# LouisPwr/CarpeDeam

Measured on AMD Instinct MI355X. Metric: corrected bases/sec on 50M×100bp synthetic reads (dhigh), 1/2/4/8 GPU, higher is better.
Workload: dtype u8 (2-bit packed bases; int32 scores; software x87 f80 likelihood sums)

## Files before the change

carpedeam_amd/csrc/aggvote.h:

```cpp
#pragma once
#include "runsort.h"

namespace aggv {

struct Ent { uint32_t id, diag, cs; };
constexpr uint32_t PENDING = 0xFFFFFFFFu;

__global__ __launch_bounds__(1024) void k_seg_flags(const uint32_t *__restrict__ recRep, uint64_t nRec, uint32_t *__restrict__ flag) {
    const uint64_t j = (uint64_t) blockIdx.x * blockDim.x + threadIdx.x;
    if (j <= nRec) flag[j] = (j < nRec && (j == 0 || recRep[j - 1] != recRep[j])) ? 1u : 0u;
}
__global__ __launch_bounds__(1024) void k_seg_fill(const uint32_t *__restrict__ recRep, uint64_t nRec, uint32_t *__restrict__ segOfRec, uint32_t *__restrict__ segRep,
                                                   unsigned long long *__restrict__ segFirstRec, uint32_t *__restrict__ entCnt) {
    const uint64_t j = (uint64_t) blockIdx.x * blockDim.x + threadIdx.x;
    if (j > nRec) return;
    const uint32_t ex = segOfRec[j];
    if (j == nRec) { segFirstRec[ex] = nRec; return; }
    const bool start = j == 0 || recRep[j - 1] != recRep[j];
    const uint32_t g = start ? ex : ex - 1;
    segOfRec[j] = g;
    if (start) { segRep[g] = recRep[j]; segFirstRec[g] = j; entCnt[g] = PENDING; }
}

struct AggArgs {
    const uint64_t *keys; const uint64_t *recVal; const unsigned long long *dst; uint64_t nRec;
    const uint32_t *segOfRec, *segRep; const unsigned long long *segFirstRec; uint64_t nSeg;
    unsigned long long *entOff; uint32_t *entCnt; unsigned long long *perRep;
    Ent *ent; unsigned long long *cursor; unsigned long long cap; unsigned int *overflow;
    int repShift, diagBits; uint32_t idBits;
    uint32_t maxD;
    const uint64_t *sorted;
    const unsigned long long *list; const unsigned int *count;
    bucket::BigList hard;
    unsigned int nextClass = 0;
    int wideWord = 0;
};
constexpr int AG_H = 1024, AG_D = 512, AG_IDX = 9, AG_ORD = 11;
constexpr unsigned long long AG_CHUNK = 2048;
inline unsigned long long aggChunkSlack(unsigned long long units, unsigned long long segments, int cuCount) {
    const unsigned long long g = (unsigned long long) cuCount * 64;
    return (3 * std::min(units + 1, g) + std::min(segments + 1, g)) * AG_CHUNK;
}
static_assert((1 << AG_IDX) >= AG_D && (1 << AG_ORD) > runsort::U_T, "aggregation geometry");
__device__ __forceinline__ uint32_t aggHash(uint64_t k) { return (uint32_t) ((k * 0x9E3779B97F4A7C15ull) >> 40); }

#ifndef CDM_AGG_MINW
#define CDM_AGG_MINW 4
#endif
template <int NT, int ITEMS, typename W = uint64_t>
__global__ __launch_bounds__(NT, CDM_AGG_MINW) void k_unit_agg(AggArgs a) {
    using namespace runsort;
    __shared__ __align__(8) unsigned char sTab[AG_H * 16];
    unsigned long long *tKey = reinterpret_cast<unsigned long long *>(sTab);
    unsigned int *tCnt = reinterpret_cast<unsigned int *>(sTab + AG_H * 8), *tLast = reinterpret_cast<unsigned int *>(sTab + AG_H * 12);
    unsigned int *oFirst = reinterpret_cast<unsigned int *>(sTab), *oEnt = oFirst + (U_T + 2), *oHit = oEnt + (U_T + 2);
    static_assert(3 * (U_T + 2) * 4 <= AG_H * 16, "the directory fits the table's memory");
    __shared__ unsigned long long dKey[AG_D];
    __shared__ unsigned int dCnt[AG_D], dLast[AG_D];
    __shared__ uint16_t sPerm[AG_D];
    __shared__ uint64_t sGStart[NT];
    __shared__ uint32_t sGOff[NT], sGSeg[NT];
    __shared__ unsigned int sDistinct, sOver, sMaxOrd;
    __shared__ unsigned long long sBase, sChunkAt, sChunkEnd;
    const int tid = threadIdx.x, lane = tid & 63, wave = tid >> 6;
    const unsigned int nUnits = *a.count;
    if (tid == 0) { sChunkAt = 0; sChunkEnd = 0; }
    const int lowBits = a.repShift - 1;
    const uint64_t lowMask = (1ull << lowBits) - 1ull;
    for (unsigned int item = blockIdx.x; item < nUnits; item += gridDim.x) {
        const uint64_t base = a.list[3 * (size_t) item];
        const int m = (int) (a.list[3 * (size_t) item + 1] - base);
        const uint64_t rec0 = a.list[3 * (size_t) item + 2];
        const uint32_t g0 = a.segOfRec[rec0];
        for (int i = tid; i < AG_H; i += NT) { tKey[i] = ~0ull; tCnt[i] = 0u; tLast[i] = 0u; }
        if (tid == 0) { sDistinct = 0; sOver = 0; sMaxOrd = 0; }
        __syncthreads();
        const unsigned long long endG = base + (uint64_t) m;
        for (uint64_t c0 = rec0; c0 < a.nRec; c0 += NT) {
            const uint64_t j = c0 + tid;
            const unsigned long long d = j < a.nRec ? a.dst[j] : ~0ull;
            const bool valid = d < endG;
            sGOff[tid] = valid ? (uint32_t) (d - base) : (uint32_t) m;
            sGStart[tid] = valid ? (a.recVal[j] >> RUN_CNT_BITS) : 0ull;
            sGSeg[tid] = valid ? a.segOfRec[j] - g0 : 0u;
            const int nr = __syncthreads_count(valid);
            if (nr == 0) break;
            const int e0 = (int) sGOff[0], e1 = (nr == NT) ? (int) min((unsigned long long) m, (j0Next(a.dst, a.nRec, c0 + NT) - base)) : m;
            if (tid == 0) sMaxOrd = max(sMaxOrd, sGSeg[nr - 1]);
            for (int eb = e0; eb < e1; eb += NT * ITEMS) {
                uint64_t key[ITEMS]; uint32_t ordv[ITEMS];
#pragma unroll
                for (int k = 0; k < ITEMS; k++) {
                    const int e = eb + k * NT + tid;
                    if (e < e1) {
                        int r = 0;
#pragma unroll
                        for (int st = NT / 2; st > 0; st >>= 1) if (r + st < nr && (int) sGOff[r + st] <= e) r += st;
                        key[k] = a.keys[sGStart[r] + (uint64_t) (e - (int) sGOff[r])];
                        ordv[k] = sGSeg[r];
                    }
                }
#pragma unroll
                for (int k = 0; k < ITEMS; k++) {
                    const int e = eb + k * NT + tid;
                    if (e < e1) {
                        const uint64_t hk = ((uint64_t) ordv[k] << lowBits) | ((key[k] >> 1) & lowMask);
                        const unsigned int last = ((unsigned int) e << 1) | (unsigned int) (key[k] & 1ull);
                        uint32_t h = aggHash(hk) & (AG_H - 1);
                        int probe = 0;
                        for (; probe < AG_H; probe++) {
                            unsigned long long old = __hip_atomic_load(&tKey[h], __ATOMIC_RELAXED, __HIP_MEMORY_SCOPE_WORKGROUP);
                            if (old == ~0ull) {
                                old = atomicCAS(&tKey[h], ~0ull, (unsigned long long) hk);
                                if (old == ~0ull) { atomicAdd(&sDistinct, 1u); old = hk; }
                            }
                            if (old == hk) { atomicAdd(&tCnt[h], 1u); atomicMax(&tLast[h], last); break; }
                            h = (h + 1) & (AG_H - 1);
                        }
                        if (probe == AG_H) sOver = 1u;
                    }
                }
            }
            const bool stop = __syncthreads_or(sDistinct > a.maxD || sOver != 0u);
            if (stop || nr < NT) break;
        }
        __syncthreads();
        if (sDistinct > a.maxD || sOver) {
            if (tid == 0) a.hard.add(base, base + (uint64_t) m);
            __syncthreads();
            continue;
        }
        unsigned int c = 0;
        for (int i = tid; i < AG_H; i += NT) c += tKey[i] != ~0ull;
        unsigned int D;
        unsigned int pos = cdm_block_excl_sum<unsigned int>(c, D);
        for (int i = tid; i < AG_H; i += NT) if (tKey[i] != ~0ull) { dKey[pos] = tKey[i]; dCnt[pos] = tCnt[i]; dLast[pos] = tLast[i]; pos++; }
        __syncthreads();
        if (wave == 0) {
            bucket::sortGroup<W>((int) D, lane,
                [&](int i) { return ((W) dKey[i] << AG_IDX) | (W) i; },
                [&](auto &v) {
                    constexpr int R = sizeof(v) / sizeof(v[0]);
#pragma unroll
                    for (int r = 0; r < R; r++) { const int p = lane * R + r; if (p < (int) D) sPerm[p] = (uint16_t) ((uint32_t) v[r] & ((1u << AG_IDX) - 1u)); }
                });
        }
        const unsigned int nOrd = sMaxOrd + 1u;
        for (unsigned int o = tid; o < nOrd; o += NT) { oFirst[o] = 0xFFFFFFFFu; oEnt[o] = 0u; oHit[o] = 0u; }
        if (tid == 0) {
            if (sChunkAt + D > sChunkEnd) { const unsigned long long want = max(AG_CHUNK, (unsigned long long) D); sChunkAt = atomicAdd(a.cursor, want); sChunkEnd = sChunkAt + want; }
            const unsigned long long b = sChunkAt;
            sChunkAt += D;
            if (b + D > a.cap) { atomicExch(a.overflow, 1u); sBase = ~0ull; } else sBase = b;
        }
        __syncthreads();
        const uint64_t idMask = (1ull << a.idBits) - 1ull, diagMask = (1ull << a.diagBits) - 1ull;
        for (unsigned int p = tid; p < D; p += NT) {
            const uint64_t hk = dKey[sPerm[p]], prev = p ? dKey[sPerm[p - 1]] : ~0ull;
            const uint32_t o = (uint32_t) (hk >> lowBits);
            atomicMin(&oFirst[o], p);
            atomicAdd(&oEnt[o], 1u);
            if (p == 0 || (hk >> a.diagBits) != (prev >> a.diagBits)) {
                const uint32_t id = (uint32_t) ((hk >> a.diagBits) & idMask);
                if (id != a.segRep[g0 + o]) atomicAdd(&oHit[o], 1u);
            }
        }
        __syncthreads();
        const unsigned long long b = sBase;
        if (b != ~0ull) {
            for (unsigned int p = tid; p < D; p += NT) {
                const int i = sPerm[p]; const uint64_t hk = dKey[i];
                Ent e; e.id = (uint32_t) ((hk >> a.diagBits) & idMask); e.diag = (uint32_t) (hk & diagMask); e.cs = (dCnt[i] << 1) | (dLast[i] & 1u);
                a.ent[b + p] = e;
            }
            for (unsigned int o = tid; o < nOrd; o += NT) {
                a.entOff[g0 + o] = b + oFirst[o]; a.entCnt[g0 + o] = oEnt[o];
                a.perRep[a.segRep[g0 + o]] = oHit[o];
            }
        }
        __syncthreads();
    }
}

__global__ __launch_bounds__(1024) void k_pending_list(const uint32_t *__restrict__ entCnt, uint64_t nSeg, uint32_t *__restrict__ list, unsigned int *__restrict__ cnt) {
    const uint64_t g = (uint64_t) blockIdx.x * blockDim.x + threadIdx.x;
    const bool p = g < nSeg && entCnt[g] == PENDING;
    const uint32_t q = cdm_block_append(cnt, p);
    if (p) list[q] = (uint32_t) g;
}
__global__ __launch_bounds__(256) void k_rle_segment(AggArgs a, const uint32_t *__restrict__ list, const unsigned int *__restrict__ nList) {
    const unsigned int n = *nList;
    const int lane = threadIdx.x & 63;
    const uint64_t idMask = (1ull << a.idBits) - 1ull, diagMask = (1ull << a.diagBits) - 1ull;
    const uint64_t below = (1ull << lane) - 1ull;
    unsigned long long chunkAt = 0, chunkEnd = 0;
    for (unsigned int it = blockIdx.x * (blockDim.x >> 6) + (threadIdx.x >> 6); it < n; it += gridDim.x * (blockDim.x >> 6)) {
        const uint32_t g = list[it];
        const uint64_t s = a.dst[a.segFirstRec[g]], e = a.dst[a.segFirstRec[g + 1]];
        const uint32_t rep = a.segRep[g];
        unsigned int runs = 0, hits = 0;
        for (uint64_t i = s + lane; i < e; i += 64) {
            const uint64_t k = a.sorted[i], p = i > s ? a.sorted[i - 1] : ~0ull;
            if (i == s || (k >> 1) != (p >> 1)) runs++;
            if (i == s || (k >> (a.diagBits + 1)) != (p >> (a.diagBits + 1))) hits += ((uint32_t) ((k >> (a.diagBits + 1)) & idMask) != rep);
        }
        const unsigned int D = (unsigned int) cdm_wave_sum((int) runs), H = (unsigned int) cdm_wave_sum((int) hits);
        unsigned long long b = 0;
        if (lane == 0) {
            if (chunkAt + D > chunkEnd) { const unsigned long long want = max(AG_CHUNK, (unsigned long long) D); chunkAt = atomicAdd(a.cursor, want); chunkEnd = chunkAt + want; }
            b = chunkAt; chunkAt += D;
            if (b + D > a.cap) { atomicExch(a.overflow, 1u); b = ~0ull; }
            else { a.entOff[g] = b; a.entCnt[g] = D; a.perRep[rep] = H; }
        }
        b = (unsigned long long) __shfl((long long) b, 0, 64);
        if (b == ~0ull) continue;
        unsigned long long run = 0;
        for (uint64_t t0 = s; t0 < e; t0 += 64) {
            const uint64_t i = t0 + lane;
            bool start = false; uint64_t k = 0;
            if (i < e) { k = a.sorted[i]; start = i == s || (k >> 1) != (a.sorted[i - 1] >> 1); }
            const uint64_t m = __ballot(start);
            if (start) {
                const uint64_t later = lane < 63 ? (m >> (lane + 1)) : 0ull;
                uint64_t hi;
                if (later) hi = i + (uint64_t) __ffsll((unsigned long long) later);
                else {
                    uint64_t lo = min(t0 + 63, e - 1); hi = e;
                    while (hi - lo > 1) { const uint64_t mid = lo + ((hi - lo) >> 1); if ((a.sorted[mid] >> 1) == (k >> 1)) lo = mid; else hi = mid; }
                }
                Ent en; en.id = (uint32_t) ((k >> (a.diagBits + 1)) & idMask); en.diag = (uint32_t) ((k >> 1) & diagMask);
                en.cs = ((uint32_t) (hi - i) << 1) | (uint32_t) (a.sorted[hi - 1] & 1ull);
                a.ent[b + run + (unsigned long long) __popcll(m & below)] = en;
            }
            run += (unsigned long long) __popcll(m);
        }
    }
}

struct VoteEntArgs {
    const Ent *ent; const unsigned long long *entOff; const uint32_t *entCnt; const uint32_t *segRep; uint64_t nSeg;
    const uint64_t *hitOff;
    const uint32_t *stale;
    int diagBias;
    const uint32_t *cont = nullptr;
};
constexpr int HEAD_WORDS = 2048;
__global__ void k_head_entries(const Ent *__restrict__ ent, const unsigned long long *__restrict__ entOff, const uint32_t *__restrict__ entCnt, uint64_t nSeg, uint32_t *__restrict__ out) {
    if (nSeg == 0) { out[0] = 0; out[1] = 0; out[2] = 1; out[HEAD_WORDS + 3] = 0; return; }
    const uint32_t id = ent[entOff[0]].id;
    uint32_t words = 0; bool whole = true;
    for (uint64_t g = 0; g < nSeg && whole && words <= (uint32_t) HEAD_WORDS; g++) {
        const Ent *e = ent + entOff[g]; const uint32_t c = entCnt[g];
        for (uint32_t j = 0; j < c; j++) {
            if (e[j].id != id) { whole = false; break; }
            if (words + 2 <= (uint32_t) HEAD_WORDS) { out[3 + words] = e[j].diag | ((e[j].cs & 1u) ? 0u : 1u << 31); out[4 + words] = e[j].cs >> 1; words += 2; }
            else { words = (uint32_t) HEAD_WORDS + 1; whole = false; break; }
        }
    }
    out[0] = words; out[1] = id; out[2] = whole ? 1u : 0u;
    const uint64_t gl = nSeg - 1;
    out[HEAD_WORDS + 3] = ent[entOff[gl] + entCnt[gl] - 1].id;
}
struct Walk {
    uint32_t prevDiag = 0, diagCnt = 0, maxDiag = 0, diagonal = 0, top = 0; int bestRev = 0; bool any = false;
    __device__ __forceinline__ void add(uint32_t d, uint32_t c, int rev) {
        diagCnt = (any && prevDiag == d) ? diagCnt + c : c;
        if (diagCnt >= maxDiag) { diagonal = d; maxDiag = diagCnt; bestRev = rev; }
        prevDiag = d; top += c; any = true;
    }
};
template <typename HitT>
__global__ __launch_bounds__(256) void k_vote_entries(VoteEntArgs a, HitT *__restrict__ out) {
    const uint64_t g = (uint64_t) blockIdx.x * blockDim.x + threadIdx.x;
    if (g >= a.nSeg) return;
    const uint32_t rep = a.segRep[g], cnt = a.entCnt[g];
    const Ent *e = a.ent + a.entOff[g];
    uint64_t pos = a.hitOff[rep] + 1;
    uint32_t p = 0;
    while (p < cnt) {
        const uint32_t id = e[p].id;
        if (id == rep) { do p++; while (p < cnt && e[p].id == id); continue; }
        Walk w;
        do { const Ent x = e[p]; w.add(x.diag, x.cs >> 1, (x.cs & 1u) ? 0 : 1); p++; } while (p < cnt && e[p].id == id);
        if (p == cnt) {
            bool done = false;
            for (uint64_t g2 = g + 1; g2 < a.nSeg && !done; g2++) {
                const Ent *f = a.ent + a.entOff[g2]; const uint32_t c2 = a.entCnt[g2];
                uint32_t j = 0;
                for (; j < c2 && f[j].id == id; j++) w.add(f[j].diag, f[j].cs >> 1, (f[j].cs & 1u) ? 0 : 1);
                done = j < c2;
            }
            bool intoStale = !done;
            if (!done && a.cont) {
                if (id == a.cont[1]) for (uint32_t j = 0; j + 1 < a.cont[0]; j += 2) w.add(a.cont[3 + j] & 0x7FFFFFFFu, a.cont[4 + j], (int) (a.cont[3 + j] >> 31));
                intoStale = a.cont[2] != 0u;
            }
            if (intoStale && id == a.stale[1]) {
                const uint32_t m = a.stale[0];
                for (uint32_t j = 0; j < m; j++) w.add(a.stale[2 + j] + (uint32_t) a.diagBias, 1u, 0);
            }
        }
        HitT h;
        h.target = id; h.score = w.bestRev ? -(int) w.top : (int) w.top; h.diagonal = (int) (short) ((int) w.diagonal - a.diagBias);
        out[pos++] = h;
    }
}

}
```

carpedeam_amd/csrc/kmermatch.hip:

```cpp
#include <memory>
#include <cstring>

#include "aggvote.h"
#include "kmer_plan.h"
#include "kmer_tuple.h"
#include "kmer_extract.h"
#include "kmer_group.h"
#include "kmer_vote.h"

namespace {

using rx::DoubleBuf;
using namespace kplan;
static_assert(RADIX_BITS == rx::BITS && SLOT_REM_BITS == rx::SLOT_REM, "kmer_plan.h restates the radix sort's geometry");
inline uint64_t deviceBytes() { size_t fr = 0, tot = 0; if (hipMemGetInfo(&fr, &tot) == hipSuccess) return tot; (void) hipGetLastError(); return 0; }
inline Db planDb(const cdm_seqdb *db, int k, bool device = false) { Db d; d.n = db->n; d.maxLen = db->maxLen; d.residues = db->residues; d.k = k; if (device) d.deviceBytes = deviceBytes(); return d; }
inline int slotSplit(int k, int &lowBits) {
    lowBits = slotLowBits(k);
    if (const char *e = cdmGetenv("CDM_SLOT_LOWBITS")) {
        char *end = nullptr; const long v = strtol(e, &end, 10);
        if (end == e || *end || v < 0 || v > 64 || !slotLowBitsServed(k, (int) v)) {
            cdm_set_error("cdm_kmermatch: CDM_SLOT_LOWBITS=%s: k = %d takes 0 <= 2k - %d - n <= %d global bits behind the head digit", e, k, RADIX_BITS, 2 * RADIX_BITS); return CDM_ERR_INVALID;
        }
        lowBits = (int) v;
    }
    return CDM_OK;
}

struct KmerJobBase {
    virtual ~KmerJobBase() {}
    virtual int phaseA() = 0;
    virtual int staleTail(unsigned long long J) = 0;
    virtual int phaseB(cdm_hits **out) = 0;
    virtual int gatherByRep() = 0;
    virtual int sortFrom(const uint64_t *devKeys, uint64_t nKeys, uint32_t *head, uint64_t info[2]) = 0;
    virtual int voteWith(const uint32_t *cont, const uint32_t *staleIn, cdm_hits **out) = 0;
    virtual int splitBegin() = 0;
    virtual int splitFinish(const void *keys, const void *vals, uint64_t m, const void *hkeys, const void *hvals, uint64_t h, bool below) = 0;
    bool split = false;
    std::vector<unsigned long long> sendOff;
    const void *sendKeys = nullptr, *sendVals = nullptr, *sendHashKeys = nullptr, *sendHashVals = nullptr; unsigned long long sendHash = 0; int valBytes = 0;
    cdm_ctx *ctx = nullptr; const cdm_seqdb *db = nullptr; cdm_kmer_params parCopy; const cdm_kmer_params *par = nullptr;
    int part = 0, nparts = 1;
    int block = 0, nBlocks = 0;
    unsigned long long live = 0, nKept = 0, regionTwo = 0;
    bool anyBelow = false;
    uint64_t *gathered = nullptr;
    uint32_t staleHost[64 + 3] = {0};
};
template <typename LY>
struct KmerJob : KmerJobBase {
    typedef typename LY::V V;
    hipStream_t s = nullptr; uint32_t n = 0; int k = 0;
    uint32_t idBits = 0, diagBits = 0; int diagBias = 0; const char *sortEnv = nullptr; bool lsdOnly = false;
    bool wide = false;
    bool passes = false;
    uint64_t r2Slots = 0;
    uint32_t ordLo = 0, ordHi = 0;
    DevBuf<uint64_t> splitK; DevBuf<V> splitV;
    DevBuf<unsigned long long> counters;
    DevBuf<unsigned int> cls;
    DevBuf<uint32_t> listShort, listLong, listSingle, listHuge;
    DevBuf<unsigned long long> slots; DevBuf<uint64_t> slotOff; DevBuf<uint32_t> rankOf;
    uint64_t kmerSlots = 0; unsigned long long nTuples = 0;
    DoubleBuf<uint64_t> keys; DoubleBuf<V> vals;
    DevBuf<uint64_t> k0, k1; DevBuf<V> v0, v1;
    V *vA = nullptr, *vB = nullptr;
    DevBuf<unsigned long long> segBuf;
    TupleGeom geom; int lowBits = 0;
    DevBuf<unsigned long long> headHist; bool headCounted = false;
    DevBuf<uint32_t> stRep, ovRep; DevBuf<uint64_t> stVal, ovVal; DevBuf<uint8_t> stCnt; DevBuf<unsigned long long> recFlag; uint64_t stagedWaves = 0, stagedOwn = 0; unsigned long long ovCap = 0, nOvRec = 0;
    DevBuf<uint32_t> bigRecRep, bigRecRep1; DevBuf<uint64_t> bigRecVal, bigRecVal1; unsigned long long nBigRec = 0;
    bool ownPipeline = false;
    bool headRange = false; uint32_t headLo = 0, headHi = 0xFFFFFFFFu;
    GroupArgs<LY> ga; DevBuf<unsigned long long> statStripes; unsigned long long *startIo = nullptr; DevBuf<uint32_t> staleBuf;
    DevBuf<uint64_t> runsOut, runsTmp;
    DevBuf<uint64_t> recvA, recvB; DevBuf<uint32_t> contBuf;
    const uint64_t *sorted2M = nullptr; unsigned long long nGroupM = 0;
    bool haveEntries = false; uint64_t nSegM = 0;
    DevBuf<uint32_t> agSegOfRec, agSegRep, agEntCnt, agPending; DevBuf<unsigned long long> agSegFirstRec, agEntOff, agPerRep, agCursor; DevBuf<aggv::Ent> agEnt; DevBuf<unsigned int> agFlags;
    float msSort1 = 0;
    KmerJob(cdm_ctx *c, const cdm_seqdb *d, const cdm_kmer_params *p) { ctx = c; db = d; parCopy = *p; par = &parCopy; }
int init() {
    s = ctx->stream;
    n = (uint32_t) db->n;
    k = par->kmer_size;
    if (k < 4 || k > 31) { cdm_set_error("cdm_kmermatch: k must be in 4..31 (got %d)", k); return CDM_ERR_INVALID; }
    idBits = bitsFor(n); diagBits = bitsFor(2ull * db->maxLen + 2);
    wide = 2 * idBits + diagBits + 1 > 63 || cdmGetenv("CDM_FORCE_WIDE_KEY") != nullptr;
    if (wide && (int) (aggv::AG_ORD + idBits + diagBits) > 64) {
        cdm_set_error("cdm_kmermatch: %u sequences x max length %u: ids and diagonals beyond %d bits are not implemented", n, db->maxLen, 64 - aggv::AG_ORD); return CDM_ERR_UNSUPPORTED;
    }
    if (wide && nparts > 1 && !passes) { cdm_set_error("cdm_kmermatch_part: %u sequences x max length %u need the wide group key, which the exchange of the k-mer-range split does not carry yet", n, db->maxLen); return CDM_ERR_UNSUPPORTED; }
    diagBias = (int) db->maxLen + 1;
    sortEnv = cdmGetenv("CDM_KMER_SORT");
    lsdOnly = sortEnv && !strcmp(sortEnv, "lsd");
    if (!counters.alloc(8)) { cdm_set_error("cdm_kmermatch: out of device memory"); return CDM_ERR_HIP; }
    hipMemsetAsync(counters.p, 0, 8 * 8, s);
    geom.kbits = 2 * k; geom.lb = (int) bitsFor((uint64_t) db->maxLen + 1); geom.lenArr = db->len;
    if constexpr (LY::bySlot) {
        if (!slotLayoutFits(planDb(db, k)) || split || (nparts != 1 && !headRange) || passes || lsdOnly) { cdm_set_error("cdm_kmermatch: internal error: the slot layout was chosen for a run it does not serve"); return CDM_ERR_INVALID; }
        geom.uniL = db->maxLen; geom.uniK = k; geom.uniS = slotsPerSeq(db->maxLen, k); divMagic(geom.uniS, geom.uniMul, geom.uniSh); geom.headShift = 2 * k - std::min(rx::BITS, 2 * k);
    }
    return CDM_OK;
}
int phaseA() override {
    if (int rc = init()) return rc;
    constexpr uint32_t SHORT_CAP = 256, LONG_CAP = 4096;

    if (!cls.alloc(8) || !listShort.alloc(n) || !listLong.alloc(n) || !listSingle.alloc(n) || !listHuge.alloc(n)) { cdm_set_error("cdm_kmermatch: out of device memory"); return CDM_ERR_HIP; }
    if (!LY::bySlot && (!slots.alloc((size_t) n + 1) || !slotOff.alloc((size_t) n + 1) || !rankOf.alloc(n))) { cdm_set_error("cdm_kmermatch: out of device memory"); return CDM_ERR_HIP; }
    hipMemsetAsync(cls.p, 0, 8 * 4, s);
    uint64_t capacity = 0;
    if constexpr (LY::bySlot) capacity = (uint64_t) n * geom.uniS;
    else {
        DevBuf<uint32_t> lk0, lk1, lv0, lv1; DevBuf<unsigned long long> ordOff;
        if (!lk0.alloc(n) || !lk1.alloc(n) || !lv0.alloc(n) || !lv1.alloc(n) || !ordOff.alloc((size_t) n + 1)) { cdm_set_error("cdm_kmermatch: out of device memory"); return CDM_ERR_HIP; }
        hipLaunchKernelGGL(k_len_keys, dim3((n + 255) / 256), dim3(256), 0, s, db->len, n, db->maxLen, lk0.p, lv0.p);
        const unsigned lenBits = bitsFor((uint64_t) db->maxLen + 2);
        cdmscan::ScanTemp st;
        DoubleBuf<uint32_t> lk(lk0.p, lk1.p), lv(lv0.p, lv1.p);
        if (int rc = rx::sortPairs<uint32_t, uint32_t>(s, ctx->cuCount, lk, lv, (uint64_t) n, 0, (int) lenBits)) return rc;
        hipLaunchKernelGGL(k_slot_counts, dim3((n + 256) / 256), dim3(256), 0, s, db->len, lv.current(), n, k, slots.p);
        if (split) {
            const unsigned blk = nBlocks ? (unsigned) block : (unsigned) part, of = nBlocks ? (unsigned) nBlocks : (unsigned) nparts;
            DevBuf<uint32_t> cuts; uint32_t hc[2] = {0, 0};
            if (!cuts.alloc(2)) { cdm_set_error("cdm_kmermatch: out of device memory"); return CDM_ERR_HIP; }
            cdmscan::ScanTemp stCut;
            if (int rc = cdmscan::exclusiveScan<unsigned long long>(s, stCut, slots.p, ordOff.p, (size_t) n + 1)) return rc;
            hipLaunchKernelGGL(k_block_cuts, dim3(1), dim3(1), 0, s, (const unsigned long long *) ordOff.p, n, blk, of, cuts.p);
            hipMemcpyAsync(hc, cuts.p, 8, hipMemcpyDeviceToHost, s);
            if (hipStreamSynchronize(s) != hipSuccess) { cdm_set_error("cdm_kmermatch: slot layout failed"); return CDM_ERR_HIP; }
            ordLo = hc[0]; ordHi = hc[1];
            hipLaunchKernelGGL(k_slot_mask, dim3((n + 255) / 256), dim3(256), 0, s, slots.p, n, ordLo, ordHi);
        }
        if (int rc = cdmscan::exclusiveScan<unsigned long long>(s, st, slots.p, ordOff.p, (size_t) n + 1)) return rc;
        hipLaunchKernelGGL(k_slot_scatter, dim3((n + 256) / 256), dim3(256), 0, s, lv.current(), ordOff.p, n, slotOff.p, rankOf.p);
        hipMemcpyAsync(&capacity, ordOff.p + n, 8, hipMemcpyDeviceToHost, s);
        if (hipStreamSynchronize(s) != hipSuccess) { cdm_set_error("cdm_kmermatch: slot layout failed"); return CDM_ERR_HIP; }
    }
    kmerSlots = geom.kmerSlots = capacity;
    r2Slots = split ? (uint64_t) (ordHi - ordLo) : (uint64_t) n;
    capacity += r2Slots;
    nTuples = capacity;

    const uint64_t valSlots = LY::bySlot ? r2Slots : capacity;
    if (!k0.alloc(capacity) || !k1.alloc(capacity) || !v0.alloc(valSlots) || !v1.alloc(valSlots)) {
        cdm_set_error("cdm_kmermatch: out of device memory for %llu k-mer tuples (%.1f GB)", (unsigned long long) capacity, (capacity * 16.0 + valSlots * 2.0 * sizeof(V)) / 1e9); return CDM_ERR_HIP;
    }
    vA = LY::bySlot ? v0.p - kmerSlots : v0.p; vB = LY::bySlot ? v1.p - kmerSlots : v1.p;
    ExtractArgs<LY> ea; ea.geom = geom; ea.uniS = geom.uniS;
    ea.woff = db->woff; ea.len = db->len; ea.codes = db->codes; ea.nmask = db->nmask; ea.hasN = db->hasN;
    ea.k = k; ea.kmersPerSeq = par->kmers_per_seq; ea.scale = par->kmers_per_seq_scale; ea.seed = par->hash_shift; ea.ignoreMultiKmer = par->ignore_multi_kmer;
    ea.keys = k0.p; ea.vals = vA; ea.slotOff = slotOff.p; ea.slowShort = listShort.p; ea.slowLong = listLong.p; ea.slowHuge = listHuge.p; ea.slowCnt = cls.p; ea.n = n;
    ea.hugeSp = nullptr; ea.hugeSel = nullptr; ea.hugeCap = 0;
    ea.list = nullptr; ea.nList = 0; ea.hashBase = kmerSlots; ea.rankOf = rankOf.p;
    if constexpr (LY::bySlot) {
        const char *e = cdmGetenv("CDM_SLOT_HIST");
        if (headRange || !(e && !strcmp(e, "kernel"))) {
            if (!headHist.alloc(HEAD_BINS)) { cdm_set_error("cdm_kmermatch: out of device memory"); return CDM_ERR_HIP; }
            hipMemsetAsync(headHist.p, 0, HEAD_BINS * 8, s);
            ea.headHist = headHist.p; ea.headShift = geom.headShift; headCounted = true;
        }
    }
    {
        const unsigned __int128 space = (unsigned __int128) 1 << (2 * k);
        ea.kLo = (uint64_t) (space * (unsigned) part / (unsigned) nparts);
        ea.kHi = (part == nparts - 1) ? ~0ull : (uint64_t) (space * (unsigned) (part + 1) / (unsigned) nparts);
        ea.lastPart = (part == nparts - 1) ? 1 : 0; ea.belowFlag = cls.p + 5;
        if (split) { ea.kLo = 0; ea.kHi = ~0ull; ea.lastPart = 1; ea.ordLo = ordLo; ea.ordHi = ordHi; }
        if (headRange) { ea.kLo = 0; ea.kHi = ~0ull; }
    }
    hipEventRecord(ctx->ev0, s);
    bool uniformKernel = false;
    if constexpr (LY::bySlot) {
        const char *e = cdmGetenv("CDM_EXTRACT");
        const uint32_t L = db->maxLen, W = (L + 15) / 16, nPos = L - (uint32_t) k + 1u;
        const size_t cap = (size_t) (float) ((float) (par->kmers_per_seq - 1) + (par->kmers_per_seq_scale * (float) L));
        if (!(e && !strcmp(e, "pair")) && k <= 30 && ea.kLo == 0 && ea.kHi == ~0ull && ea.ordHi == 0 && ea.lastPart && nPos <= cap && nPos <= (uint32_t) PAIR_POS &&
            db->nCount == 0 && !db->raw && (uint64_t) n * W < (1ull << 32)) {
            unsigned int bad = 1;
            hipLaunchKernelGGL(k_uniform_check, dim3((n + 255) / 256), dim3(256), 0, s, (const uint32_t *) db->len, (const uint32_t *) db->woff, (const uint8_t *) db->hasN, n, L, W, cls.p + 6);
            hipMemcpyAsync(&bad, cls.p + 6, 4, hipMemcpyDeviceToHost, s);
            if (hipStreamSynchronize(s) != hipSuccess) { cdm_set_error("cdm_kmermatch: looking at the sequence lengths failed"); return CDM_ERR_HIP; }
            uniformKernel = bad == 0;
        }
        if (uniformKernel) {
            const uint32_t batches = ((n + 1) / 2 + UNI_BATCH - 1) / UNI_BATCH;
            uint32_t blocks = std::min<uint32_t>((batches + FAST_WAVES - 1) / FAST_WAVES, ctx->cuCount * UNI_MINW);
            if (const char *eb = cdmGetenv("CDM_EXTRACT_BLOCKS")) blocks = std::max(1u, std::min<uint32_t>(blocks, (uint32_t) atoi(eb)));
            hipLaunchKernelGGL(k_extract_uniform<LY>, dim3(blocks), dim3(64 * FAST_WAVES), 0, s, ea, L, W);
        }
    }
    ea.single = listSingle.p; ea.listCount = nullptr;
    if (!uniformKernel) {
        hipLaunchKernelGGL(k_seq_hash<LY>, dim3((n + 255) / 256), dim3(256), 0, s, ea);
        if (k <= 30) {
            hipLaunchKernelGGL(k_extract_pair<LY>, dim3(std::min<uint32_t>(((n + 1) / 2 + FAST_WAVES - 1) / FAST_WAVES, ctx->cuCount * 16)), dim3(64 * FAST_WAVES), 0, s, ea);
            ea.list = listSingle.p; ea.listCount = cls.p + 2;
        }
        hipLaunchKernelGGL(k_extract_fast<LY>, dim3(std::min<uint32_t>((n + FAST_WAVES - 1) / FAST_WAVES, ctx->cuCount * 16)), dim3(64 * FAST_WAVES), 0, s, ea);
        ea.listCount = nullptr;
    }
    unsigned int hcls[4] = {0, 0, 0, 0};
    hipMemcpyAsync(hcls, cls.p, 16, hipMemcpyDeviceToHost, s);
    { hipError_t e = hipStreamSynchronize(s); if (e != hipSuccess) { cdm_set_error("cdm_kmermatch: extraction failed: %s", hipGetErrorString(e)); return CDM_ERR_HIP; } }
    auto general = [&](void (*kern)(ExtractArgs<LY>), const uint32_t *list, uint32_t cnt, uint32_t blocks, uint32_t nt) { ea.list = list; ea.nList = cnt; hipLaunchKernelGGL(kern, dim3(blocks), dim3(nt), 0, s, ea); };
    if (hcls[0]) general(k_extract<LY, SHORT_CAP, 64>, listShort.p, hcls[0], std::min<uint32_t>(hcls[0], ctx->cuCount * 32), 64);
    if (hcls[1]) general(k_extract<LY, LONG_CAP, 256>, listLong.p, hcls[1], std::min<uint32_t>(hcls[1], ctx->cuCount * 2), 256);
    DevBuf<SeqPos> hugeSp; DevBuf<uint8_t> hugeSel;
    if (hcls[3]) {
        uint32_t cap = LONG_CAP; while (cap < db->maxLen) cap <<= 1;
        const uint32_t blocks = std::min<uint32_t>(hcls[3], (uint32_t) ctx->cuCount * 4);
        if (!hugeSp.alloc((size_t) blocks * cap) || !hugeSel.alloc((size_t) blocks * cap)) { cdm_set_error("cdm_kmermatch: out of device memory"); return CDM_ERR_HIP; }
        ea.hugeSp = hugeSp.p; ea.hugeSel = hugeSel.p; ea.hugeCap = cap;
        general(k_extract<LY, 0, 256>, listHuge.p, hcls[3], blocks, 256);
    }
    hipEventRecord(ctx->ev1, s);
    unsigned int belowHost = 0;
    hipMemcpyAsync(&belowHost, cls.p + 5, 4, hipMemcpyDeviceToHost, s);
    { hipError_t e = hipStreamSynchronize(s); if (e != hipSuccess) { cdm_set_error("cdm_kmermatch: extraction (general path) failed: %s", hipGetErrorString(e)); return CDM_ERR_HIP; } }
    anyBelow = belowHost != 0;
    hipEventElapsedTime(&ctx->lastMs[3], ctx->ev0, ctx->ev1);
    if (cdmGetenv("CDM_BUCKET_STATS")) fprintf(stderr, "kmermatch extraction (%s): %u sequences through k_extract for a repeated k-mer or a bottom-m selection, %u + %u longer ones\n", uniformKernel ? "uniform kernel" : "pair + fast kernels", hcls[0], hcls[1], hcls[3]);
    if (split) return splitPartition();
    if constexpr (LY::bySlot) if (headRange) {
        unsigned long long hh[HEAD_BINS];
        if (hipMemcpy(hh, headHist.p, sizeof(hh), hipMemcpyDeviceToHost) != hipSuccess) { cdm_set_error("cdm_kmermatch: reading the head histogram failed"); return CDM_ERR_HIP; }
        std::vector<uint32_t> cut = equalShareCuts(hh, HEAD_BINS, nparts);
        cut.resize((size_t) nparts + 1, (uint32_t) HEAD_BINS);
        headLo = cut[part]; headHi = cut[part + 1];
        anyBelow = false; for (uint32_t d = 0; d < headLo; d++) anyBelow = anyBelow || hh[d] != 0;
    }
    return sortAndGroup();
}
int splitPartition() {
    DevBuf<unsigned long long> cnt, bounds;
    if (!cnt.alloc(2) || !bounds.alloc((size_t) CDM_KPART_SLICES + 2)) { cdm_set_error("cdm_kmermatch: out of device memory"); return CDM_ERR_HIP; }
    unsigned long long m = 0, h = 0;
    const int shift = 2 * k - 8;
    DoubleBuf<uint64_t> ordK(k0.p, k1.p); DoubleBuf<V> ordV(v0.p, v1.p);
    if (kmerSlots) {
        if (int rc = rx::sortPairs<uint64_t, V>(s, ctx->cuCount, ordK, ordV, (uint64_t) kmerSlots, shift, 2 * k + 1)) return rc;
        hipLaunchKernelGGL(k_live_count, dim3(1), dim3(1), 0, s, (const uint64_t *) ordK.current(), (uint64_t) kmerSlots, 2 * k, cnt.p);
        hipMemcpyAsync(&m, cnt.p, 8, hipMemcpyDeviceToHost, s);
    }
    uint64_t *rK = ordK.current(); V *rV = ordV.current();
    if (r2Slots) {
        if (int rc = rx::compactPairs<uint64_t, V>(s, k0.p + kmerSlots, v0.p + kmerSlots, (uint64_t) r2Slots, k1.p + kmerSlots, v1.p + kmerSlots, cnt.p + 1)) return rc;
        hipMemcpyAsync(&h, cnt.p + 1, 8, hipMemcpyDeviceToHost, s);
    }
    if (hipStreamSynchronize(s) != hipSuccess) { cdm_set_error("cdm_kmermatch: ordering the tuples by k-mer slice failed: %s", hipGetErrorString(hipGetLastError())); return CDM_ERR_HIP; }
    sendOff.assign((size_t) CDM_KPART_SLICES + 1, 0);
    if (m) {
        hipLaunchKernelGGL(k_slice_bounds, dim3(2), dim3(256), 0, s, (const uint64_t *) rK, (uint64_t) m, shift, (uint32_t) CDM_KPART_SLICES, bounds.p);
        hipMemcpyAsync(sendOff.data(), bounds.p, ((size_t) CDM_KPART_SLICES + 1) * 8, hipMemcpyDeviceToHost, s);
        if (hipStreamSynchronize(s) != hipSuccess) { cdm_set_error("cdm_kmermatch: ordering the tuples by k-mer slice failed: %s", hipGetErrorString(hipGetLastError())); return CDM_ERR_HIP; }
    }
    sendKeys = rK; sendVals = rV; valBytes = (int) sizeof(V);
    sendHashKeys = k1.p + kmerSlots; sendHashVals = v1.p + kmerSlots; sendHash = h;
    return CDM_OK;
}
int splitBegin() override {
    split = true;
    if (nparts != CDM_KPART_SLICES) { cdm_set_error("cdm_kmermatch: internal error: the split by reads orders its tuples by %d slices", CDM_KPART_SLICES); return CDM_ERR_INVALID; }
    return phaseA();
}
int takeOver(uint64_t m, uint64_t h, bool below) { vA = v0.p; vB = v1.p; kmerSlots = m; r2Slots = h; nTuples = m + h; geom.kmerSlots = m; anyBelow = below; return sortAndGroup(); }
void freeExtraction() { slots.free(); slotOff.free(); rankOf.free(); listShort.free(); listLong.free(); listSingle.free(); listHuge.free(); }
int splitFinish(const void *keysIn, const void *valsIn, uint64_t m, const void *hkeys, const void *hvals, uint64_t h, bool below) override {
    freeExtraction();
    splitK.free(); splitV.free(); k0.free(); k1.free(); v0.free(); v1.free();
    DevBuf<uint64_t> nk0, nk1; DevBuf<V> nv0, nv1;
    const uint64_t tot = m + h;
    if (!nk0.alloc(tot) || !nk1.alloc(tot) || !nv0.alloc(tot) || !nv1.alloc(tot)) { cdm_set_error("cdm_kmermatch: out of device memory for %llu received k-mer tuples", (unsigned long long) tot); return CDM_ERR_HIP; }
    if (m) { hipMemcpyAsync(nk0.p, keysIn, m * 8, hipMemcpyDeviceToDevice, s); hipMemcpyAsync(nv0.p, valsIn, m * sizeof(V), hipMemcpyDeviceToDevice, s); }
    if (h) { hipMemcpyAsync(nk0.p + m, hkeys, h * 8, hipMemcpyDeviceToDevice, s); hipMemcpyAsync(nv0.p + m, hvals, h * sizeof(V), hipMemcpyDeviceToDevice, s); }
    if (hipStreamSynchronize(s) != hipSuccess) { cdm_set_error("cdm_kmermatch: taking over the received tuples failed"); return CDM_ERR_HIP; }
    k0.p = nk0.release(); k1.p = nk1.release(); v0.p = nv0.release(); v1.p = nv1.release();
    return takeOver(m, h, below);
}
int keepOnlyOutgoing() {
    DevBuf<uint64_t> hk; DevBuf<V> hv;
    const unsigned long long m = sendOff.empty() ? 0 : sendOff.back();
    if (!hk.alloc(sendHash) || !hv.alloc(sendHash) || !splitK.alloc(m) || !splitV.alloc(m)) { cdm_set_error("cdm_kmermatch: out of device memory"); return CDM_ERR_HIP; }
    if (m) { hipMemcpyAsync(splitK.p, sendKeys, m * 8, hipMemcpyDeviceToDevice, s); hipMemcpyAsync(splitV.p, sendVals, m * sizeof(V), hipMemcpyDeviceToDevice, s); }
    if (sendHash) { hipMemcpyAsync(hk.p, sendHashKeys, sendHash * 8, hipMemcpyDeviceToDevice, s); hipMemcpyAsync(hv.p, sendHashVals, sendHash * sizeof(V), hipMemcpyDeviceToDevice, s); }
    if (hipStreamSynchronize(s) != hipSuccess) { cdm_set_error("cdm_kmermatch: keeping a block's tuples failed"); return CDM_ERR_HIP; }
    k0.free(); k1.free(); v0.free(); v1.free();
    sendKeys = splitK.p; sendVals = splitV.p;
    freeExtraction(); cls.free(); counters.free();
    sendHashKeys = keptHashK.p = hk.release(); sendHashVals = keptHashV.p = hv.release();
    return CDM_OK;
}
DevBuf<uint64_t> keptHashK; DevBuf<V> keptHashV;
int rangeFinishOwned(DevBuf<uint64_t> &keysBuf, DevBuf<V> &valsBuf, uint64_t m, uint64_t h, bool below) {
    passes = true; split = true;
    if (int rc = init()) return rc;
    const uint64_t tot = m + h;
    if (!k1.alloc(tot) || !v1.alloc(tot)) { cdm_set_error("cdm_kmermatch: out of device memory for a pass over %llu k-mer tuples", (unsigned long long) tot); return CDM_ERR_HIP; }
    k0.p = keysBuf.release(); v0.p = valsBuf.release();
    return takeOver(m, h, below);
}
int sortAndGroup() {
    keys = DoubleBuf<uint64_t>(k0.p, k1.p); vals = DoubleBuf<V>(vA, vB);
    lowBits = lsdOnly ? 0 : std::max(0, 2 * k + 1 - 27);
    if constexpr (LY::bySlot) if (int rc = slotSplit(k, lowBits)) return rc;
    hipEventRecord(ctx->ev0, s);
    if (int rc = sortRegionOne()) return rc;
    hipEventRecord(ctx->ev1, s);
    hipEventRecord(ctx->ev2, s);
    if (int rc = sortRegionTwo()) return rc;
    hipEventRecord(ctx->ev3, s);
    ga.geom = geom;
    ga.keys = keys.current(); ga.vals = vals.current(); ga.n = nTuples; ga.onlyExtendable = par->include_only_extendable; ga.covMode = par->cov_mode;
    ga.covThr = par->cov_thr; ga.idBits = idBits; ga.diagBits = diagBits; ga.diagBias = diagBias; ga.first = 0; ga.wide = wide ? 1 : 0;
    ga.firstRunIdx = (anyBelow || (split && kmerSlots == 0)) ? ~0ull : 0ull;
    if (!statStripes.alloc(STAT_STRIPES)) { cdm_set_error("cdm_kmermatch: out of device memory"); return CDM_ERR_HIP; }
    hipMemsetAsync(statStripes.p, 0, STAT_STRIPES * 8, s);
    ga.stat = statStripes.p;
    startIo = (unsigned long long *) keys.alternate();
    if (!LY::bySlot) live = 0;
    nKept = 0;
    if (!staleBuf.alloc(STALE_MAX + 3)) { cdm_set_error("cdm_kmermatch: out of device memory"); return CDM_ERR_HIP; }
    hipMemsetAsync(staleBuf.p, 0, (STALE_MAX + 3) * 4, s);
    if (kmerSlots && !LY::bySlot) {
        hipLaunchKernelGGL(k_live_count, dim3(1), dim3(1), 0, s, ga.keys, (uint64_t) kmerSlots, 2 * k, counters.p + 3);
        hipMemcpyAsync(&live, counters.p + 3, 8, hipMemcpyDeviceToHost, s);
        if (hipStreamSynchronize(s) != hipSuccess) { cdm_set_error("cdm_kmermatch: grouping failed"); return CDM_ERR_HIP; }
    }
    if (lowBits == 0) { if (scanGroups(ga, startIo) != CDM_OK) return groupingFailed(); }
    else if (int rc = groupBuckets()) return rc;
    return countKept();
}
int groupingFailed() { cdm_set_error("cdm_kmermatch: grouping failed: %s", hipGetErrorString(hipGetLastError())); return CDM_ERR_HIP; }
int sortRegionOne() {
    const int sortTop = lowBits ? 2 * k + 1 : 2 * k;
    if constexpr (LY::bySlot) {
        if (!segBuf.alloc(rx::BINS + 1)) { cdm_set_error("cdm_kmermatch: out of device memory"); return CDM_ERR_HIP; }
        uint64_t *res = nullptr; unsigned long long liveSlots = 0;
        if (int rc = rx::sortSlotKeys(s, ctx->cuCount, k0.p, k1.p, (uint64_t) kmerSlots, 2 * k, lowBits, headCounted ? headHist.p : nullptr, segBuf.p, liveSlots, res, &ctx->lastMs[13], &ctx->lastMs[14],
                                      headRange ? headLo : 0u, headRange ? std::min<uint32_t>(headHi, (uint32_t) rx::BINS) : (uint32_t) rx::BINS)) return rc;
        keys = DoubleBuf<uint64_t>(res, res == k0.p ? k1.p : k0.p); vals = res == k0.p ? DoubleBuf<V>(vA, vB) : DoubleBuf<V>(vB, vA);
        ctx->lastMs[15] = (float) (((double) kmerSlots * 8.0 + (double) liveSlots * 8.0 + (double) (ctx->lastMs[14] - 1.f) * (double) liveSlots * 16.0) / 1e9);
        live = liveSlots; geom.seg = segBuf.p;
        return CDM_OK;
    }
    uint64_t sorted = kmerSlots;
    const bool range = nparts > 1 && kmerSlots && !lsdOnly && !split;
    DevBuf<unsigned long long> cnt;
    if (range) {
        if (!cnt.alloc(1)) { cdm_set_error("cdm_kmermatch: out of device memory"); return CDM_ERR_HIP; }
        if (int rc = rx::compactPairs<uint64_t, V>(s, k0.p, vA, (uint64_t) kmerSlots, k1.p, vB, cnt.p)) return rc;
        unsigned long long m = 0;
        hipMemcpyAsync(&m, cnt.p, 8, hipMemcpyDeviceToHost, s);
        if (hipStreamSynchronize(s) != hipSuccess) { cdm_set_error("cdm_kmermatch: compaction failed"); return CDM_ERR_HIP; }
        keys = DoubleBuf<uint64_t>(k1.p, k0.p); vals = DoubleBuf<V>(vB, vA); sorted = m;
    }
    if (int rc = rx::sortPairs<uint64_t, V>(s, ctx->cuCount, keys, vals, sorted, lowBits, sortTop, &ctx->lastMs[13])) return rc;
    ctx->lastMs[14] = (float) ((sortTop - lowBits + rx::BITS - 1) / rx::BITS);
    ctx->lastMs[15] = (float) ((double) ctx->lastMs[14] * (double) sorted * 2.0 * (8.0 + sizeof(V)) / 1e9);
    if (range) hipMemsetAsync(keys.current() + sorted, 0xFF, (size_t) (kmerSlots - sorted) * 8, s);
    return CDM_OK;
}
int sortRegionTwo() {
    DoubleBuf<uint64_t> rk(k0.p + kmerSlots, k1.p + kmerSlots); DoubleBuf<V> rv(vA + kmerSlots, vB + kmerSlots);
    if (int rc = rx::sortPairs<uint64_t, V>(s, ctx->cuCount, rk, rv, (uint64_t) r2Slots, 0, 63)) return rc;
    uint64_t *kOut = keys.current() + kmerSlots; V *vOut = vals.current() + kmerSlots;
    if (rk.current() != kOut && r2Slots) { hipMemcpyAsync(kOut, rk.current(), (size_t) r2Slots * 8, hipMemcpyDeviceToDevice, s); hipMemcpyAsync(vOut, rv.current(), (size_t) r2Slots * sizeof(V), hipMemcpyDeviceToDevice, s); }
    return CDM_OK;
}
int scanGroups(GroupArgs<LY> g, unsigned long long *io) {
    const size_t cnt = (size_t) (g.n - g.first);
    if (cnt == 0) return CDM_OK;
    cdmscan::ScanTemp t;
    if (int rc = cdmscan::inclusiveMaxScanFn(s, t, StartFrom<LY>{StartIndex<LY>{g.keys, g.geom, (unsigned long long) g.first}}, io + g.first, cnt)) return rc;
    if (cnt > CDM_MAX_LAUNCH_THREADS - 256) { cdm_set_error("cdm_kmermatch: %zu tuples in one grouping launch (CDM_KMER_SORT=lsd takes fewer than 2^32)", cnt); return CDM_ERR_UNSUPPORTED; }
    hipLaunchKernelGGL(k_groups<LY>, CDM_GRID((cnt + 255) / 256, 256), dim3(256), 0, s, g, io);
    return hipStreamSynchronize(s) == hipSuccess ? CDM_OK : CDM_ERR_HIP;
}
template <typename W>
bool launchFused(int own, uint32_t maxBucket, DevBuf<unsigned long long> &bigList, DevBuf<unsigned int> &bigCnt, DevBuf<BlockHead> &heads) {
    BucketGroupArgs<LY, W> ba;
    static_cast<GroupParams &>(ba) = ga; ba.n = live;
    ba.keys = ga.keys; ba.vals = ga.vals; ba.geom = geom; ba.out = startIo; ba.lowBits = lowBits; ba.own = own; ba.maxBucket = maxBucket;
    ba.big.list = bigList.p; ba.big.cnt = bigCnt.p;
    const uint64_t perBlock = (uint64_t) own * bucket::BK_WAVES;
    stagedWaves = 0;
    if (LY::bySlot && (ownPipeline || headRange) && live && !cdmGetenv("CDM_RUN_RECORDS") && !cdmGetenv("CDM_RUN_CAP")) {
        const uint64_t waves = (live + (uint64_t) own - 1) / (uint64_t) own;
        ovCap = live / 256 + 4096;
        if (stRep.alloc(waves * REC_CAP) && stVal.alloc(waves * REC_CAP) && stCnt.alloc(waves + 1) && recFlag.alloc(2) && ovRep.alloc(ovCap) && ovVal.alloc(ovCap)) {
            hipMemsetAsync(stCnt.p, 0, waves + 1, s); hipMemsetAsync(recFlag.p, 0, 8, s);
            ba.recRep = stRep.p; ba.recVal = stVal.p; ba.recCnt = stCnt.p; stagedWaves = waves; stagedOwn = (uint64_t) own; nBigRec = 0;
            ba.ovRep = ovRep.p; ba.ovVal = ovVal.p; ba.ovCursor = recFlag.p; ba.ovCap = ovCap;
            if (const char *e = cdmGetenv("CDM_REC_LIMIT")) { const long v = atol(e); if (v >= 0 && v <= REC_CAP) ba.recLimit = (uint32_t) v; }
        } else { dropStages(); (void) hipGetLastError(); }
    }
    if constexpr (LY::bySlot) {
        const uint64_t blocks = (live + perBlock - 1) / perBlock;
        if (!heads.alloc(blocks)) { cdm_set_error("cdm_kmermatch: out of device memory"); return false; }
        if (blocks) hipLaunchKernelGGL(k_block_heads, CDM_GRID((blocks + 255) / 256, 256), dim3(256), 0, s, geom, (uint64_t) live, perBlock, blocks, heads.p);
        ba.blockHead = heads.p;
    }
    if (live) hipLaunchKernelGGL((k_bucket_groups<LY, W>), dim3((unsigned) ((live + perBlock - 1) / perBlock)), dim3(bucket::BK_NT), cdm_lds_pad("CDM_LDS_PAD_GROUPS"), s, ba);
    return true;
}
void dropStages() { stagedWaves = 0; stRep.free(); stVal.free(); stCnt.free(); ovRep.free(); ovVal.free(); }
int groupBuckets() {
    int own; uint32_t maxBucket; bucket::capacities(own, maxBucket);
    own = std::min(own, GkGeom<LY>::OWN); maxBucket = std::min<uint32_t>(maxBucket, (uint32_t) GkGeom<LY>::MAXB);
    DevBuf<unsigned long long> bigList; DevBuf<unsigned int> bigCnt;
    if (!bigList.alloc(bucket::bigListSlots(kmerSlots, maxBucket)) || !bigCnt.alloc(1)) { cdm_set_error("cdm_kmermatch: out of device memory"); return CDM_ERR_HIP; }
    hipMemsetAsync(bigCnt.p, 0, 4, s);
    if (kmerSlots) hipMemsetAsync(startIo + live, 0xFF, (size_t) (kmerSlots - live) * 8, s);
    DevBuf<BlockHead> heads;
    if (!(lowBits <= GROUP_WORD32_LOWBITS ? launchFused<uint32_t>(own, maxBucket, bigList, bigCnt, heads) : launchFused<uint64_t>(own, maxBucket, bigList, bigCnt, heads))) return CDM_ERR_HIP;
    unsigned int nBig = 0; unsigned long long recOver = 0;
    hipMemcpyAsync(&nBig, bigCnt.p, 4, hipMemcpyDeviceToHost, s);
    if (stagedWaves) hipMemcpyAsync(&recOver, recFlag.p, 8, hipMemcpyDeviceToHost, s);
    GroupArgs<LY> g2 = ga; g2.first = kmerSlots;
    int rc = scanGroups(g2, startIo);
    nOvRec = recOver;
    if (stagedWaves && recOver > ovCap) dropStages();
    if (rc == CDM_OK && nBig) rc = groupBigBuckets(bigList, nBig);
    return rc == CDM_OK ? CDM_OK : groupingFailed();
}
template <bool GATHER> void bigBucketPairs(unsigned int grid, const unsigned long long *ranges, unsigned int nBig, uint64_t *dk, V *dv) {
    if constexpr (LY::bySlot) hipLaunchKernelGGL(k_big_slot_pairs<GATHER>, dim3(grid), dim3(256), 0, s, ranges, nBig, const_cast<uint64_t *>(ga.keys), geom, dk, dv);
    else {
        hipLaunchKernelGGL((bucket::k_big_copy<uint64_t, GATHER>), dim3(grid), dim3(256), 0, s, ranges, nBig, const_cast<uint64_t *>(ga.keys), dk);
        hipLaunchKernelGGL((bucket::k_big_copy<V, GATHER>), dim3(grid), dim3(256), 0, s, ranges, nBig, const_cast<V *>(ga.vals), dv);
    }
}
int groupBigBuckets(DevBuf<unsigned long long> &bigList, unsigned int nBig) {
    DevBuf<unsigned long long> ranges; uint64_t total = 0; unsigned long long firstStart = ~0ull;
    int rc = bucket::loadBigList(s, bigList.p, nBig, ranges, total, &firstStart);
    if (cdmGetenv("CDM_BUCKET_STATS")) fprintf(stderr, "kmermatch sort 1: %llu slots, low bits %d: %u big buckets, %llu tuples\n", (unsigned long long) kmerSlots, lowBits, nBig, (unsigned long long) total);
    DevBuf<uint64_t> dk0, dk1; DevBuf<V> dv0, dv1; DevBuf<unsigned long long> ds;
    if (rc == CDM_OK && (!dk0.alloc(total) || !dk1.alloc(total) || !dv0.alloc(total) || !dv1.alloc(total) || !ds.alloc(total))) rc = CDM_ERR_HIP;
    if (rc != CDM_OK) return rc;
    const unsigned int grid = bucket::bigCopyGrid(nBig);
    bigBucketPairs<true>(grid, ranges.p, nBig, dk0.p, dv0.p);
    DoubleBuf<uint64_t> dk(dk0.p, dk1.p); DoubleBuf<V> dv(dv0.p, dv1.p);
    if (int rc2 = rx::sortPairs<uint64_t, V>(s, ctx->cuCount, dk, dv, (uint64_t) total, 0, 2 * k)) return rc2;
    bigBucketPairs<false>(grid, ranges.p, nBig, dk.current(), dv.current());
    GroupArgs<LY> gd = ga; gd.keys = dk.current(); gd.vals = dv.current(); gd.n = total; gd.first = 0;
    gd.geom.kmerSlots = ~0ull;
    gd.firstRunIdx = (firstStart == 0 && !anyBelow) ? 0ull : ~0ull;
    if (int rc2 = scanGroups(gd, ds.p)) return rc2;
    hipLaunchKernelGGL((bucket::k_big_copy<unsigned long long, false>), dim3(grid), dim3(256), 0, s, (const unsigned long long *) ranges.p, nBig, startIo, ds.p);
    if (hipStreamSynchronize(s) != hipSuccess) return CDM_ERR_HIP;
    if (stagedWaves) {
        DevBuf<unsigned long long> gapped;
        if (!gapped.alloc(total + nBig)) return CDM_ERR_HIP;
        hipLaunchKernelGGL(k_big_gap_copy, dim3(grid), dim3(256), 0, s, (const unsigned long long *) ranges.p, nBig, (const unsigned long long *) ds.p, gapped.p);
        runsort::RunArgs ra = runArgs((const uint64_t *) gapped.p, total + nBig, 0, 0);
        rc = runsort::makeRunRecords(s, ra, bigRecRep, bigRecRep1, bigRecVal, bigRecVal1, nBigRec);
        if (rc == CDM_OK && nBigRec) hipLaunchKernelGGL(k_big_rec_starts, CDM_GRID((nBigRec + 255) / 256, 256), dim3(256), 0, s, (const unsigned long long *) ranges.p, nBig, bigRecVal.p, (uint64_t) nBigRec);
        if (rc == CDM_OK && hipStreamSynchronize(s) != hipSuccess) rc = CDM_ERR_HIP;
        bigRecRep1.free(); bigRecVal1.free();
    }
    return rc;
}
int countKept() {
    hipLaunchKernelGGL(k_reduce_stats, dim3(1), dim3(256), 0, s, (const unsigned long long *) statStripes.p, counters.p + 4);
    hipMemcpyAsync(&nKept, counters.p + 4, 8, hipMemcpyDeviceToHost, s);
    { hipError_t e = hipStreamSynchronize(s); if (e != hipSuccess) { cdm_set_error("cdm_kmermatch: grouping failed: %s", hipGetErrorString(e)); return CDM_ERR_HIP; } }
    hipEventElapsedTime(&msSort1, ctx->ev0, ctx->ev1);
    regionTwo = 0;
    if (nparts > 1 && part == nparts - 1 && r2Slots) {
        hipLaunchKernelGGL(k_count_hash_tuples, dim3(1), dim3(1), 0, s, (const uint64_t *) ga.keys + kmerSlots, (uint64_t) r2Slots, counters.p + 6);
        hipMemcpyAsync(&regionTwo, counters.p + 6, 8, hipMemcpyDeviceToHost, s);
        if (hipStreamSynchronize(s) != hipSuccess) { cdm_set_error("cdm_kmermatch: grouping failed"); return CDM_ERR_HIP; }
    }
    return CDM_OK;
}
runsort::RunArgs runArgs(const uint64_t *gk, unsigned long long nIn, unsigned long long skipLo, unsigned long long skipHi) const {
    runsort::RunArgs ra; ra.keys = gk; ra.n = nIn; ra.skipLo = skipLo; ra.skipHi = skipHi; ra.repShift = (int) (idBits + diagBits + 1);
    ra.wide = wide ? 1 : 0; ra.idShift = (int) diagBits + 1; ra.idMask = (1ull << idBits) - 1ull;
    return ra;
}
int staleTail(unsigned long long J) override {
    memset(staleHost, 0, sizeof(staleHost));
    hipMemsetAsync(staleBuf.p, 0, (STALE_MAX + 3) * 4, s);
    const unsigned long long realTuples = live + regionTwo;
    if (nparts > 1 && J >= realTuples) { staleHost[STALE_MAX + 4] = 1; return hipStreamSynchronize(s) == hipSuccess ? CDM_OK : CDM_ERR_HIP; }
    StaleArgs<LY> sa;
    sa.keys = ga.keys; sa.vals = ga.vals; sa.geom = geom; sa.live = live; sa.kmerSlots = kmerSlots; sa.nTuples = nTuples; sa.J = J;
    sa.lowBits = lowBits; sa.sorted = (lowBits == 0); sa.out = staleBuf.p;
    hipLaunchKernelGGL(k_stale_tail<LY>, dim3(1), dim3(256), 0, s, sa);
    hipMemcpyAsync(staleHost, staleBuf.p, (STALE_MAX + 3) * 4, hipMemcpyDeviceToHost, s);
    if (hipStreamSynchronize(s) != hipSuccess) { cdm_set_error("cdm_kmermatch: grouping failed"); return CDM_ERR_HIP; }
    if (staleHost[0] >= (uint32_t) STALE_MAX) {
        cdm_set_error("cdm_kmermatch: the reference's last per-target scan could run over %d or more left-over tuples of one sequence; not reproduced on the device", STALE_MAX);
        return CDM_ERR_UNSUPPORTED;
    }
    staleHost[STALE_MAX + 4] = (J + staleHost[0] >= realTuples) ? 1u : 0u;
    return CDM_OK;
}
int phaseB(cdm_hits **out) override {
    if (int rc = sort2((const uint64_t *) startIo, nTuples, live, kmerSlots, keys.current(), (uint64_t *) startIo, true)) return rc;
    return vote(nullptr, true, out);
}
int sort2(const uint64_t *keysIn, unsigned long long nIn, unsigned long long skipLo, unsigned long long skipHi, uint64_t *bufA, uint64_t *bufB, bool ownBuffers) {

    if (ownBuffers) { v0.free(); v1.free(); }
    const int top2 = (int) ((wide ? idBits : 2 * idBits) + diagBits + 1);
    const char *sort2Env = cdmGetenv("CDM_KMER_SORT2");
    const bool sort2Check = sort2Env && !strcmp(sort2Env, "check");
    const bool sort2Runs = !lsdOnly && (!sort2Env || !strcmp(sort2Env, "runs") || sort2Check);
    if (wide && (!sort2Runs || sort2Check || !ownBuffers)) { cdm_set_error("cdm_kmermatch: the wide group key runs on the default pipeline only (run records + aggregated entries)"); return CDM_ERR_UNSUPPORTED; }
    if (sort2Env && strcmp(sort2Env, "runs") && strcmp(sort2Env, "radix") && !sort2Check) { cdm_set_error("cdm_kmermatch: CDM_KMER_SORT2 must be runs, radix or check"); return CDM_ERR_INVALID; }
    unsigned long long nGroup = 0;
    const uint64_t *sorted2 = nullptr;
    hipEventRecord(ctx->ev0, s);
    if (sort2Runs) {
        using namespace runsort;
        const uint64_t *gk = keysIn;
        uint64_t *sortedOut = bufA;
        if (sort2Check) {
            if (!runsOut.alloc(nIn)) { cdm_set_error("cdm_kmermatch: out of device memory (sort 2 check)"); return CDM_ERR_HIP; }
            sortedOut = runsOut.p;
        }
        const RunArgs ra = runArgs(gk, nIn, skipLo, skipHi);
        const bool fromStage = stagedWaves && ownBuffers && keysIn == (const uint64_t *) startIo;
        RepRecords R;
        if (int rc = recordsByRep(ra, fromStage, true, R, nGroup)) return rc;
        const unsigned long long nRec = R.nRec; const DoubleBuf<uint32_t> &rk = R.rep; const DoubleBuf<uint64_t> &rv = R.val; DevBuf<unsigned long long> &dst = R.dst;
        if (nRec) {
            if (hipStreamSynchronize(s) != hipSuccess) { cdm_set_error("cdm_kmermatch: sort 2 (records) failed: %s", hipGetErrorString(hipGetLastError())); return CDM_ERR_HIP; }
            const char *voteEnv = cdmGetenv("CDM_KMER_VOTE");
            const bool wordFits = aggv::AG_ORD + idBits + diagBits + aggv::AG_IDX <= 64 && !(wide && cdmGetenv("CDM_FORCE_WIDE_WORD"));
            const char *distVote = cdmGetenv("CDM_DIST_VOTE");
            bool aggregated = wide || ((ownBuffers || !(distVote && !strcmp(distVote, "tuples"))) && !sort2Check && !(voteEnv && !strcmp(voteEnv, "tuples")) && wordFits);
            if ((wide || fromStage) && ownBuffers && nGroup != nKept) { cdm_set_error("cdm_kmermatch: internal error: %llu group tuples counted, %llu in the run records", nKept, nGroup); return CDM_ERR_HIP; }
            if (aggregated) {
                const unsigned long long slack = aggv::aggChunkSlack(nGroup / runsort::U_T, nRec, ctx->cuCount);
                unsigned long long capEnt = nGroup / 6 + (4ull << 20) + slack;
                if (const char *e = cdmGetenv("CDM_AGG_CAP")) capEnt = strtoull(e, nullptr, 10);
                int rc = aggregate(sortedOut, nGroup, rk.current(), (const uint64_t *) rv.current(), dst.p, nRec, gk, top2, capEnt, !wordFits);
                while (rc == CDM_ERR_UNSUPPORTED && wide && capEnt < nGroup + 1 + slack) {
                    capEnt = std::min<unsigned long long>(nGroup + 1 + slack, std::max<unsigned long long>(capEnt * 3, 1024));
                    rc = aggregate(sortedOut, nGroup, rk.current(), (const uint64_t *) rv.current(), dst.p, nRec, gk, top2, capEnt, !wordFits);
                }
                if (rc == CDM_ERR_UNSUPPORTED && !wide) aggregated = false;
                else if (rc) return rc;
            }
            haveEntries = aggregated;
            if (!aggregated && segmentedSortKeys(s, ctx->cuCount, sortedOut, sortedOut, nGroup, (int) (idBits + diagBits + 1), (int) (diagBits + 1), top2, rk.current(), dst.p, nRec, gk,
                                  (const uint64_t *) rv.current()) != CDM_OK) {
                cdm_set_error("cdm_kmermatch: segmented sort 2 failed: %s", hipGetErrorString(hipGetLastError())); return CDM_ERR_HIP;
            }
        }
        sorted2 = sortedOut;
    }
    if (!sort2Runs || sort2Check) {
        const int shiftHi2 = lsdOnly ? 1 : std::max(1, top2 + 1 - 32);
        bool g2First = true;
        if (int rc = rx::sortKeys<uint64_t>(s, ctx->cuCount, const_cast<uint64_t *>(keysIn), bufA, (uint64_t) nIn, shiftHi2, top2 + 1, g2First)) return rc;
        DoubleBuf<uint64_t> g(g2First ? const_cast<uint64_t *>(keysIn) : bufA, g2First ? bufA : const_cast<uint64_t *>(keysIn));
        unsigned long long nGroupR = 0;
        if (nIn) {
            hipLaunchKernelGGL(k_live_count, dim3(1), dim3(1), 0, s, (const uint64_t *) g.current(), (uint64_t) nIn, top2, counters.p + 2);
            hipMemcpyAsync(&nGroupR, counters.p + 2, 8, hipMemcpyDeviceToHost, s);
            if (hipStreamSynchronize(s) != hipSuccess) { cdm_set_error("cdm_kmermatch: radix sort 2 failed"); return CDM_ERR_HIP; }
        }
        const uint64_t *sortedR = g.current();
        if (shiftHi2 > 1) {
            if (bucket::bucketSortKeys(s, g.current(), g.alternate(), nGroupR, shiftHi2, 1, top2) != CDM_OK) { cdm_set_error("cdm_kmermatch: bucket sort 2 failed: %s", hipGetErrorString(hipGetLastError())); return CDM_ERR_HIP; }
            sortedR = g.alternate();
        }
        if (sort2Check) {
            if (nGroupR != nGroup) { cdm_set_error("cdm_kmermatch: sort 2 check: %llu kept tuples by runs, %llu by radix", nGroup, nGroupR); return CDM_ERR_HIP; }
            hipMemsetAsync(counters.p + 5, 0xFF, 8, s);
            if (nGroup) hipLaunchKernelGGL(k_first_diff, dim3((unsigned) std::min<uint64_t>((nGroup + 255) / 256, 65535)), dim3(256), 0, s, sorted2, sortedR, (uint64_t) nGroup, counters.p + 5);
            unsigned long long firstDiff = ~0ull, pair[2] = {0, 0};
            hipMemcpyAsync(&firstDiff, counters.p + 5, 8, hipMemcpyDeviceToHost, s);
            if (hipStreamSynchronize(s) != hipSuccess) { cdm_set_error("cdm_kmermatch: sort 2 check failed"); return CDM_ERR_HIP; }
            if (firstDiff != ~0ull) {
                hipMemcpy(&pair[0], sorted2 + firstDiff, 8, hipMemcpyDeviceToHost); hipMemcpy(&pair[1], sortedR + firstDiff, 8, hipMemcpyDeviceToHost);
                cdm_set_error("cdm_kmermatch: sort 2 check: first difference at %llu of %llu: runs %016llx radix %016llx (idBits %u diagBits %u)", firstDiff, nGroup, pair[0], pair[1], idBits, diagBits);
                return CDM_ERR_HIP;
            }
        }
        nGroup = nGroupR; sorted2 = sortedR;
    }
    hipEventRecord(ctx->ev1, s);
    sorted2M = sorted2; nGroupM = nGroup;
    return CDM_OK;
}
struct RepRecords {
    cdmscan::ScanTemp st; DevBuf<uint32_t> r0, r1; DevBuf<uint64_t> v0, v1; DevBuf<unsigned long long> dst; unsigned long long nRec = 0;
    DoubleBuf<uint32_t> rep; DoubleBuf<uint64_t> val;
};
int recordsByRep(const runsort::RunArgs &ra, bool staged, bool dstIfNone, RepRecords &R, unsigned long long &total) {
    if (staged) { if (int rc = stagedRunRecords(ra, R.r0, R.r1, R.v0, R.v1, R.nRec)) return rc; }
    else if (int rc = runsort::makeRunRecords(s, ra, R.r0, R.r1, R.v0, R.v1, R.nRec)) return rc;
    if (R.nRec == 0 && !dstIfNone) return CDM_OK;
    if (!R.dst.alloc(R.nRec + 1)) { cdm_set_error("cdm_kmermatch: out of device memory (%llu run records)", R.nRec); return CDM_ERR_HIP; }
    if (R.nRec == 0) return CDM_OK;
    R.rep = DoubleBuf<uint32_t>(R.r0.p, R.r1.p); R.val = DoubleBuf<uint64_t>(R.v0.p, R.v1.p);
    if (int rc = rx::sortPairs<uint32_t, uint64_t>(s, ctx->cuCount, R.rep, R.val, (uint64_t) R.nRec, 0, (int) idBits)) return rc;
    hipMemsetAsync(R.val.current() + R.nRec, 0, 8, s);
    if (int rc = cdmscan::exclusiveScanFn<unsigned long long, runsort::RunLen>(s, R.st, runsort::RunLen{R.val.current()}, R.dst.p, (size_t) R.nRec + 1)) return rc;
    hipMemcpyAsync(&total, R.dst.p + R.nRec, 8, hipMemcpyDeviceToHost, s);
    return CDM_OK;
}
int stagedRunRecords(const runsort::RunArgs &whole, DevBuf<uint32_t> &rr0, DevBuf<uint32_t> &rr1, DevBuf<uint64_t> &rv0, DevBuf<uint64_t> &rv1, unsigned long long &nRec) {
    DevBuf<unsigned long long> off; cdmscan::ScanTemp st;
    if (!off.alloc(stagedWaves + 1)) { cdm_set_error("cdm_kmermatch: out of device memory (run records)"); return CDM_ERR_HIP; }
    if (int rc = cdmscan::exclusiveScanFn<unsigned long long, RecCount>(s, st, RecCount{stCnt.p}, off.p, (size_t) stagedWaves + 1)) return rc;
    unsigned long long n1 = 0, n2 = 0;
    hipMemcpyAsync(&n1, off.p + stagedWaves, 8, hipMemcpyDeviceToHost, s);
    DevBuf<uint32_t> q0, q1; DevBuf<uint64_t> w0, w1;
    runsort::RunArgs r2 = whole; r2.keys = whole.keys + kmerSlots; r2.n = whole.n - kmerSlots; r2.skipLo = r2.skipHi = 0; r2.base = kmerSlots;
    if (r2.n) { if (int rc = runsort::makeRunRecords(s, r2, q0, q1, w0, w1, n2)) return rc; }
    if (hipStreamSynchronize(s) != hipSuccess) { cdm_set_error("cdm_kmermatch: run records failed: %s", hipGetErrorString(hipGetLastError())); return CDM_ERR_HIP; }
    unsigned long long nb = nBigRec;
    if (nOvRec) {
        DevBuf<uint64_t> x0, x1; DevBuf<uint32_t> y0, y1;
        const unsigned long long tot = nBigRec + nOvRec;
        if (!x0.alloc(tot) || !x1.alloc(tot) || !y0.alloc(tot) || !y1.alloc(tot)) { cdm_set_error("cdm_kmermatch: out of device memory (run records)"); return CDM_ERR_HIP; }
        if (nBigRec) { hipMemcpyAsync(x0.p, bigRecVal.p, nBigRec * 8, hipMemcpyDeviceToDevice, s); hipMemcpyAsync(y0.p, bigRecRep.p, nBigRec * 4, hipMemcpyDeviceToDevice, s); }
        hipMemcpyAsync(x0.p + nBigRec, ovVal.p, nOvRec * 8, hipMemcpyDeviceToDevice, s); hipMemcpyAsync(y0.p + nBigRec, ovRep.p, nOvRec * 4, hipMemcpyDeviceToDevice, s);
        DoubleBuf<uint64_t> x(x0.p, x1.p); DoubleBuf<uint32_t> y(y0.p, y1.p);
        if (int rc = rx::sortPairs<uint64_t, uint32_t>(s, ctx->cuCount, x, y, (uint64_t) tot, runsort::RUN_CNT_BITS, 64)) return rc;
        bigRecVal.free(); bigRecRep.free();
        bigRecVal.p = x.current() == x0.p ? x0.release() : x1.release(); bigRecRep.p = y.current() == y0.p ? y0.release() : y1.release();
        nb = tot;
    }
    nRec = n1 + nb + n2;
    if (!rr0.alloc(nRec) || !rr1.alloc(nRec) || !rv0.alloc(nRec + 1) || !rv1.alloc(nRec + 1)) { cdm_set_error("cdm_kmermatch: out of device memory (%llu run records)", nRec); return CDM_ERR_HIP; }
    if (n1) hipLaunchKernelGGL(k_rec_compact, CDM_GRID((stagedWaves + REC_WAVES - 1) / REC_WAVES, 256), dim3(256), 0, s, (const uint32_t *) stRep.p, (const uint64_t *) stVal.p, (const unsigned long long *) off.p, (uint64_t) stagedWaves,
                               (uint64_t) stagedOwn, (const uint64_t *) bigRecVal.p, (uint64_t) nb, rr0.p, rv0.p);
    if (nb) hipLaunchKernelGGL(k_rec_place_big, CDM_GRID((nb + 255) / 256, 256), dim3(256), 0, s, (const uint32_t *) bigRecRep.p, (const uint64_t *) bigRecVal.p, (uint64_t) nb, (const uint64_t *) stVal.p, (const uint8_t *) stCnt.p,
                               (const unsigned long long *) off.p, (uint64_t) stagedOwn, rr0.p, rv0.p);
    if (n2) { hipMemcpyAsync(rr0.p + n1 + nb, q0.p, n2 * 4, hipMemcpyDeviceToDevice, s); hipMemcpyAsync(rv0.p + n1 + nb, w0.p, n2 * 8, hipMemcpyDeviceToDevice, s); }
    if (hipStreamSynchronize(s) != hipSuccess) { cdm_set_error("cdm_kmermatch: run records (packing) failed: %s", hipGetErrorString(hipGetLastError())); return CDM_ERR_HIP; }
    if (cdmGetenv("CDM_BUCKET_STATS")) fprintf(stderr, "run records: %llu staged by the grouping kernel, %llu beyond its waves' stages, %llu of its big buckets, %llu of the whole-sequence hash region\n", n1, nOvRec, nBigRec, n2);
    stRep.free(); stVal.free(); stCnt.free(); bigRecRep.free(); bigRecVal.free(); ovRep.free(); ovVal.free(); stagedWaves = 0; nBigRec = 0; nOvRec = 0;
    return CDM_OK;
}
int voteEntries(cdm_hits **out, const uint32_t *contDev = nullptr) {
    DevBuf<unsigned long long> perRepScan;
    if (!perRepScan.alloc((size_t) n + 1)) { cdm_set_error("cdm_kmermatch: out of device memory (vote)"); return CDM_ERR_HIP; }
    cdmscan::ScanTemp st4a;
    if (int rc = cdmscan::exclusiveScan<unsigned long long>(s, st4a, agPerRep.p, perRepScan.p, (size_t) n + 1)) return rc;
    if (int rc = placeHits(perRepScan.p, true, out, [&](cdm_hits *res) {
        aggv::VoteEntArgs va; va.ent = agEnt.p; va.entOff = agEntOff.p; va.entCnt = agEntCnt.p; va.segRep = agSegRep.p; va.nSeg = nSegM; va.hitOff = res->off; va.stale = staleBuf.p; va.diagBias = diagBias; va.cont = contDev;
        if (nSegM) hipLaunchKernelGGL(aggv::k_vote_entries<HitRec>, dim3((unsigned) ((nSegM + 255) / 256)), dim3(256), 0, s, va, res->rec);
    })) return rc;
    agEnt.free(); agEntOff.free(); agEntCnt.free(); agSegRep.free(); agSegOfRec.free(); agSegFirstRec.free(); agPerRep.free(); agPending.free();
    return CDM_OK;
}
template <typename Place>
int placeHits(const unsigned long long *perRepScan, bool sort1R2, cdm_hits **out, Place place) {
    cdm_hits *res = new cdm_hits(); res->n = n;
    if (cdmMalloc(&res->off, ((size_t) n + 1) * 8) != hipSuccess) { delete res; cdm_set_error("cdm_kmermatch: out of device memory"); return CDM_ERR_HIP; }
    hipLaunchKernelGGL(k_offsets, dim3((n + 256) / 256), dim3(256), 0, s, perRepScan, n, res->off);
    uint64_t total = 0;
    hipMemcpyAsync(&total, res->off + n, 8, hipMemcpyDeviceToHost, s);
    { hipError_t e = hipStreamSynchronize(s); if (e != hipSuccess) { cdm_hits_free(res); cdm_set_error("cdm_kmermatch: vote failed: %s", hipGetErrorString(e)); return CDM_ERR_HIP; } }
    res->count = total;
    if (cdmMalloc(&res->rec, (total + 1) * sizeof(HitRec)) != hipSuccess) { cdm_hits_free(res); cdm_set_error("cdm_kmermatch: out of device memory"); return CDM_ERR_HIP; }
    hipLaunchKernelGGL(k_self, dim3((n + 255) / 256), dim3(256), 0, s, res->off, n, res->rec);
    place(res);
    { hipError_t e = hipStreamSynchronize(s); if (e != hipSuccess) { cdm_hits_free(res); cdm_set_error("cdm_kmermatch: placing hits failed: %s", hipGetErrorString(e)); return CDM_ERR_HIP; } }
    float msSort2 = 0; hipEventElapsedTime(&msSort2, ctx->ev0, ctx->ev1);
    ctx->lastMs[2] = msSort1 + msSort2;
    ctx->lastMs[5] = msSort1;
    ctx->lastMs[6] = msSort2;
    if (sort1R2) hipEventElapsedTime(&ctx->lastMs[7], ctx->ev2, ctx->ev3);
    *out = res;
    return CDM_OK;
}
static void aggUnitHook(hipStream_t st, unsigned int grid, const unsigned long long *list, const unsigned int *count, bucket::BigList hard, void *user) {
    aggv::AggArgs *u = reinterpret_cast<aggv::AggArgs *>(user);
    aggv::AggArgs a = *u;
    a.list = list; a.count = count; a.hard = hard;
    const int cls = (int) (u->nextClass++ % runsort::U_CLASSES);
    const unsigned int pad = cdm_lds_pad("CDM_LDS_PAD_AGG");
    if (u->wideWord) {
        if (cls == 0) hipLaunchKernelGGL((aggv::k_unit_agg<256, runsort::U_CLASS_CAP[0] / 256, bucket::u128>), dim3(grid), dim3(256), pad, st, a);
        else if (cls == 1) hipLaunchKernelGGL((aggv::k_unit_agg<256, runsort::U_CLASS_CAP[1] / 256, bucket::u128>), dim3(grid), dim3(256), pad, st, a);
        else hipLaunchKernelGGL((aggv::k_unit_agg<256, runsort::U_CLASS_CAP[2] / 256, bucket::u128>), dim3(grid), dim3(256), pad, st, a);
        return;
    }
    if (cls == 0) hipLaunchKernelGGL((aggv::k_unit_agg<256, runsort::U_CLASS_CAP[0] / 256>), dim3(grid), dim3(256), pad, st, a);
    else if (cls == 1) hipLaunchKernelGGL((aggv::k_unit_agg<256, runsort::U_CLASS_CAP[1] / 256>), dim3(grid), dim3(256), pad, st, a);
    else hipLaunchKernelGGL((aggv::k_unit_agg<256, runsort::U_CLASS_CAP[2] / 256>), dim3(grid), dim3(256), pad, st, a);
}
int aggregate(uint64_t *sortedOut, unsigned long long nGroup, const uint32_t *recRep, const uint64_t *recVal, const unsigned long long *dst, unsigned long long nRec,
              const uint64_t *gk, int top2, unsigned long long capEnt, bool wideWord) {
    using namespace aggv;
    cdmscan::ScanTemp st;
    agEnt.free(); agSegOfRec.free(); agPerRep.free(); agCursor.free(); agFlags.free(); agSegRep.free(); agSegFirstRec.free(); agEntOff.free(); agEntCnt.free(); agPending.free();
    if (!agSegOfRec.alloc(nRec + 2) || !agPerRep.alloc((size_t) n + 1) || !agCursor.alloc(2) || !agFlags.alloc(4)) { cdm_set_error("cdm_kmermatch: out of device memory (aggregation)"); return CDM_ERR_HIP; }
    hipLaunchKernelGGL(k_seg_flags, CDM_GRID((nRec + 1024) / 1024, 1024), dim3(1024), 0, s, recRep, (uint64_t) nRec, agSegOfRec.p);
    if (int rc = cdmscan::exclusiveScan<uint32_t>(s, st, agSegOfRec.p, agSegOfRec.p, (size_t) nRec + 1)) return rc;
    uint32_t nSeg = 0;
    hipMemcpyAsync(&nSeg, agSegOfRec.p + nRec, 4, hipMemcpyDeviceToHost, s);
    if (hipStreamSynchronize(s) != hipSuccess) { cdm_set_error("cdm_kmermatch: aggregation (segments) failed: %s", hipGetErrorString(hipGetLastError())); return CDM_ERR_HIP; }
    if (!agSegRep.alloc(nSeg + 1) || !agSegFirstRec.alloc((size_t) nSeg + 2) || !agEntOff.alloc((size_t) nSeg + 1) || !agEntCnt.alloc((size_t) nSeg + 1) || !agPending.alloc((size_t) nSeg + 1) ||
        !agEnt.alloc(capEnt + 1)) {
        agEnt.free(); cdm_set_error("cdm_kmermatch: out of device memory (aggregation)"); return CDM_ERR_HIP;
    }
    hipLaunchKernelGGL(k_seg_fill, CDM_GRID((nRec + 1024) / 1024, 1024), dim3(1024), 0, s, recRep, (uint64_t) nRec, agSegOfRec.p, agSegRep.p, agSegFirstRec.p, agEntCnt.p);
    hipMemsetAsync(agPerRep.p, 0, ((size_t) n + 1) * 8, s);
    hipMemsetAsync(agCursor.p, 0, 16, s); hipMemsetAsync(agFlags.p, 0, 16, s);
    AggArgs a;
    a.keys = gk; a.recVal = recVal; a.dst = dst; a.nRec = nRec; a.segOfRec = agSegOfRec.p; a.segRep = agSegRep.p; a.segFirstRec = agSegFirstRec.p; a.nSeg = nSeg;
    a.entOff = agEntOff.p; a.entCnt = agEntCnt.p; a.perRep = agPerRep.p; a.ent = agEnt.p; a.cursor = agCursor.p; a.cap = capEnt; a.overflow = agFlags.p;
    a.maxD = AG_D;
    if (const char *e = cdmGetenv("CDM_AGG_D")) { const long v = atol(e); if (v >= 1 && v <= AG_D) a.maxD = (uint32_t) v; }
    a.repShift = (int) (idBits + diagBits + 1); a.diagBits = (int) diagBits; a.idBits = idBits; a.sorted = sortedOut; a.list = nullptr; a.count = nullptr; a.hard.list = nullptr; a.hard.cnt = nullptr;
    a.wideWord = wideWord ? 1 : 0;
    if (runsort::segmentedSortKeys(s, ctx->cuCount, sortedOut, sortedOut, nGroup, (int) (idBits + diagBits + 1), (int) (diagBits + 1), top2, recRep, dst, nRec, gk, recVal, aggUnitHook, &a, wide, agSegOfRec.p, (int) bitsFor((uint64_t) nSeg + 1), agSegFirstRec.p, (uint64_t) nSeg) != CDM_OK) {
        cdm_set_error("cdm_kmermatch: segmented sort 2 failed: %s", hipGetErrorString(hipGetLastError())); return CDM_ERR_HIP;
    }
    hipLaunchKernelGGL(k_pending_list, dim3((unsigned) (((uint64_t) nSeg + 1023) / 1024)), dim3(1024), 0, s, (const uint32_t *) agEntCnt.p, (uint64_t) nSeg, agPending.p, agFlags.p + 1);
    unsigned int fl[4] = {0, 0, 0, 0};
    hipMemcpyAsync(fl, agFlags.p, 16, hipMemcpyDeviceToHost, s);
    if (hipStreamSynchronize(s) != hipSuccess) { cdm_set_error("cdm_kmermatch: aggregation failed: %s", hipGetErrorString(hipGetLastError())); return CDM_ERR_HIP; }
    if (fl[1] && cdmGetenv("CDM_RLE_STATS")) {
        std::vector<uint32_t> pl(fl[1]); std::vector<unsigned long long> fr((size_t) nSeg + 1), dd((size_t) nRec + 1);
        hipMemcpy(pl.data(), agPending.p, (size_t) fl[1] * 4, hipMemcpyDeviceToHost); hipMemcpy(fr.data(), agSegFirstRec.p, ((size_t) nSeg + 1) * 8, hipMemcpyDeviceToHost);
        hipMemcpy(dd.data(), dst, ((size_t) nRec + 1) * 8, hipMemcpyDeviceToHost);
        unsigned long long tot = 0, mx = 0, over4k = 0, over64k = 0, inBig = 0;
        for (uint32_t g : pl) { const unsigned long long m = dd[fr[g + 1]] - dd[fr[g]]; tot += m; mx = std::max(mx, m); if (m > 4096) { over4k++; inBig += m; } if (m > 65536) over64k++; }
        fprintf(stderr, "rle segments: %u of %llu, %llu tuples (longest %llu; %llu beyond 4096 tuples holding %llu, %llu beyond 65536)\n", fl[1], (unsigned long long) nSeg, tot, mx, over4k, inBig, over64k);
    }
    if (fl[1] && !fl[0]) {
        hipLaunchKernelGGL(k_rle_segment, dim3(std::min<unsigned int>((fl[1] + 3) / 4, (unsigned int) ctx->cuCount * 16)), dim3(256), 0, s, a, (const uint32_t *) agPending.p, (const unsigned int *) (agFlags.p + 1));
        hipMemcpyAsync(fl, agFlags.p, 16, hipMemcpyDeviceToHost, s);
        if (hipStreamSynchronize(s) != hipSuccess) { cdm_set_error("cdm_kmermatch: aggregation (segments of the tuple sorters) failed: %s", hipGetErrorString(hipGetLastError())); return CDM_ERR_HIP; }
    }
    unsigned long long used = 0;
    hipMemcpy(&used, agCursor.p, 8, hipMemcpyDeviceToHost);
    if (cdmGetenv("CDM_BUCKET_STATS")) fprintf(stderr, "aggregate: %llu group tuples, %u segments, %llu entries (room for %llu), %u segments through the tuple sorters%s\n", nGroup, nSeg, used, capEnt, fl[1],
                                            fl[0] ? "; entry buffer overflow" : "");
    if (fl[0]) { agEnt.free(); return CDM_ERR_UNSUPPORTED; }
    nSegM = nSeg;
    return CDM_OK;
}
int vote(const uint32_t *contDev, bool ownBuffers, cdm_hits **out) {
    if (haveEntries) return voteEntries(out, contDev);
    const uint64_t *sorted2 = sorted2M; const unsigned long long nGroup = nGroupM;
    DevBuf<unsigned long long> perRep, perRepScan, vTileCnt, vTileOff;
    const uint64_t vTiles = (nGroup + CP_TILE - 1) / CP_TILE;
    if (!perRep.alloc((size_t) n + 1) || !perRepScan.alloc((size_t) n + 1) || !vTileCnt.alloc(vTiles + 1) || !vTileOff.alloc(vTiles + 1)) {
        cdm_set_error("cdm_kmermatch: out of device memory (vote)"); return CDM_ERR_HIP;
    }
    hipMemsetAsync(perRep.p, 0, ((size_t) n + 1) * 8, s);
    hipMemsetAsync(vTileCnt.p, 0, (vTiles + 1) * 8, s);
    VoteArgs va;
    if (ownBuffers && nGroup != nKept) { cdm_set_error("cdm_kmermatch: internal error: %llu group tuples counted, %llu sorted", nKept, nGroup); return CDM_ERR_HIP; }
    va.stale = staleBuf.p; va.cont = contDev;
    va.keys = sorted2; va.n = nGroup; va.idBits = idBits; va.diagBits = diagBits; va.diagBias = diagBias; va.perRep = perRep.p;
    if (nGroup) hipLaunchKernelGGL(k_seg_count, dim3((unsigned) vTiles), dim3(256), 0, s, va, vTileCnt.p);
    cdmscan::ScanTemp st4a, st4b;
    if (int rc = cdmscan::exclusiveScan<unsigned long long>(s, st4a, perRep.p, perRepScan.p, (size_t) n + 1)) return rc;
    if (int rc = cdmscan::exclusiveScan<unsigned long long>(s, st4b, vTileCnt.p, vTileOff.p, (size_t) vTiles + 1)) return rc;
    return placeHits(perRepScan.p, ownBuffers, out, [&](cdm_hits *res) {
        if (nGroup) hipLaunchKernelGGL(k_seg_place, dim3((unsigned) vTiles), dim3(256), cdm_lds_pad("CDM_LDS_PAD_VOTE"), s, va, vTileOff.p, perRepScan.p, res->off, res->rec);
    });
}
int gatherByRep() override {
    using namespace runsort;
    v0.free(); v1.free();
    RunArgs ra; ra.keys = (const uint64_t *) startIo; ra.n = nTuples; ra.skipLo = live; ra.skipHi = kmerSlots; ra.repShift = (int) (idBits + diagBits + 1);
    unsigned long long nOut = 0;
    RepRecords R;
    if (int rc = recordsByRep(ra, stagedWaves != 0, false, R, nOut)) return rc;
    gathered = keys.current();
    if (R.nRec == 0) return CDM_OK;
    hipLaunchKernelGGL(k_run_gather, CDM_GRID((R.nRec + 255) / 256, 256), dim3(256), 0, s, (const uint64_t *) startIo, (const uint64_t *) R.val.current(), (const unsigned long long *) R.dst.p, (uint64_t) R.nRec, gathered);
    if (hipStreamSynchronize(s) != hipSuccess) { cdm_set_error("cdm_kmermatch: gather by representative failed: %s", hipGetErrorString(hipGetLastError())); return CDM_ERR_HIP; }
    if (nOut != nKept) { cdm_set_error("cdm_kmermatch: internal error: %llu group tuples counted, %llu gathered", nKept, nOut); return CDM_ERR_HIP; }
    return CDM_OK;
}
int sortFrom(const uint64_t *devKeys, uint64_t nKeys, uint32_t *head, uint64_t info[2]) override {
    k0.free(); k1.free(); v0.free(); v1.free();
    if (!recvA.alloc(nKeys) || !recvB.alloc(nKeys) || !contBuf.alloc(CONT_CAP + 4)) { cdm_set_error("cdm_kmermatch: out of device memory for %llu received group tuples", (unsigned long long) nKeys); return CDM_ERR_HIP; }
    if (nKeys) hipMemcpyAsync(recvB.p, devKeys, nKeys * 8, hipMemcpyDeviceToDevice, s);
    if (int rc = sort2(recvB.p, nKeys, 0, 0, recvA.p, recvB.p, false)) return rc;
    if (haveEntries) {
        static_assert(aggv::HEAD_WORDS == CONT_CAP, "the words of a head");
        uint32_t lastId = 0;
        hipLaunchKernelGGL(aggv::k_head_entries, dim3(1), dim3(1), 0, s, (const aggv::Ent *) agEnt.p, (const unsigned long long *) agEntOff.p, (const uint32_t *) agEntCnt.p, (uint64_t) nSegM, contBuf.p);
        hipMemcpyAsync(head, contBuf.p, (CONT_CAP + 3) * 4, hipMemcpyDeviceToHost, s);
        hipMemcpyAsync(&lastId, contBuf.p + CONT_CAP + 3, 4, hipMemcpyDeviceToHost, s);
        if (hipStreamSynchronize(s) != hipSuccess) { cdm_set_error("cdm_kmermatch: second half (aggregation) failed: %s", hipGetErrorString(hipGetLastError())); return CDM_ERR_HIP; }
        info[0] = nGroupM; info[1] = lastId;
        return CDM_OK;
    }
    hipLaunchKernelGGL(k_head_segment, dim3(1), dim3(1), 0, s, sorted2M, (uint64_t) nGroupM, idBits, diagBits, contBuf.p);
    uint64_t last = 0;
    hipMemcpyAsync(head, contBuf.p, (CONT_CAP + 3) * 4, hipMemcpyDeviceToHost, s);
    if (nGroupM) hipMemcpyAsync(&last, sorted2M + nGroupM - 1, 8, hipMemcpyDeviceToHost, s);
    if (hipStreamSynchronize(s) != hipSuccess) { cdm_set_error("cdm_kmermatch: second half (sort) failed: %s", hipGetErrorString(hipGetLastError())); return CDM_ERR_HIP; }
    info[0] = nGroupM; info[1] = (last >> (diagBits + 1)) & ((1ull << idBits) - 1ull);
    return CDM_OK;
}
int voteWith(const uint32_t *cont, const uint32_t *staleIn, cdm_hits **out) override {
    if (hipMemcpyAsync(staleBuf.p, staleIn, (STALE_MAX + 3) * 4, hipMemcpyHostToDevice, s) != hipSuccess) { cdm_set_error("cdm_kmermatch: stale list upload failed"); return CDM_ERR_HIP; }
    if (cont) {
        if (cont[0] > (uint32_t) CONT_CAP) { cdm_set_error("cdm_kmermatch: the scan of this rank's last target runs over more than %d tuples of the next ranks; not reproduced", CONT_CAP); return CDM_ERR_UNSUPPORTED; }
        if (hipMemcpyAsync(contBuf.p, cont, (3 + (size_t) cont[0]) * 4, hipMemcpyHostToDevice, s) != hipSuccess) { cdm_set_error("cdm_kmermatch: continuation list upload failed"); return CDM_ERR_HIP; }
    }
    return vote(cont ? contBuf.p : nullptr, false, out);
}
};

template <typename LY>
int kmermatchPassesT(cdm_ctx *ctx, const cdm_seqdb *db, const cdm_kmer_params *par, int P, int B, cdm_hits **out, const KmerRanks *ranks = nullptr) {
    typedef typename LY::V V;
    hipStream_t s = ctx->stream;
    const int W = ranks ? ranks->world : 1, R = ranks ? ranks->rank : 0;
    if (W > 1) P = std::min(255, (std::max(P, 1) + W - 1) / W * W);
    if (P < 1 || P > 255 || B < 1) { cdm_set_error("cdm_kmermatch: %d passes over %d blocks", P, B); return CDM_ERR_INVALID; }
    const bool stats = cdmGetenv("CDM_BUCKET_STATS") != nullptr;
    struct NoHeadroom { float was; NoHeadroom() : was(cdmPoolHeadroomSwap(1.0f)) {} ~NoHeadroom() { cdmPoolHeadroomSwap(was); } } noHeadroom;
    constexpr int F = CDM_KPART_SLICES;
    std::vector<std::vector<unsigned long long>> cnt((size_t) B, std::vector<unsigned long long>((size_t) F + 1, 0));
    auto extractBlock = [&](KmerJob<LY> &ex, int b) -> int { ex.part = 0; ex.nparts = F; ex.block = b; ex.nBlocks = B; ex.passes = true; return ex.splitBegin(); };
    std::vector<unsigned long long> fine((size_t) F, 0);
    auto poolLine = [&](const char *what, int i) { if (stats) { uint64_t st[8]; cdm_pool_stats(st); fprintf(stderr, "kmermatch passes (%d x %d): %s %d: %.1f GB mapped, %.1f GB in use\n", P, B, what, i, st[6] / 1e9, st[7] / 1e9); } };
    poolLine("start", 0);
    std::vector<std::unique_ptr<KmerJob<LY>>> kept((size_t) B);
    bool keepAll = true; unsigned long long keptBytes = 0, keepBudget = 0;
    { size_t fr = 0, tot = 0; if (hipMemGetInfo(&fr, &tot) == hipSuccess) keepBudget = (unsigned long long) (0.40 * (double) tot); else (void) hipGetLastError(); }
    if (const char *e = cdmGetenv("CDM_KMER_KEEP")) keepBudget = strtoull(e, nullptr, 10);
    for (int b = 0; b < B; b++) {
        std::unique_ptr<KmerJob<LY>> ex(new KmerJob<LY>(ctx, db, par));
        if (int rc = extractBlock(*ex, b)) return rc;
        for (int f = 0; f < F; f++) { cnt[b][f] = ex->sendOff[f + 1] - ex->sendOff[f]; fine[f] += cnt[b][f]; }
        cnt[b][F] = ex->sendHash;
        if (keepAll) {
            const unsigned long long bytes = (ex->sendOff[F] + ex->sendHash) * (8ull + sizeof(V));
            if (keptBytes + bytes > keepBudget) { keepAll = false; for (auto &q : kept) q.reset(); }
            else { if (int rc = ex->keepOnlyOutgoing()) return rc; keptBytes += bytes; kept[b] = std::move(ex); }
        }
        poolLine("counted block", b);
    }
    const std::vector<uint32_t> cut = equalShareCuts(fine.data(), F, P);
    P = (int) cut.size() - 1;
    auto runRange = [&](int r, KmerJob<LY> &job) -> int {
        const int f0 = (int) cut[r], f1 = (int) cut[r + 1];
        unsigned long long m = 0, h = 0; bool below = false;
        std::vector<unsigned long long> mine((size_t) B, 0);
        for (int b = 0; b < B; b++) {
            for (int f = f0; f < f1; f++) mine[b] += cnt[b][f];
            m += mine[b]; if (r == P - 1) h += cnt[b][F];
            for (int f = 0; f < f0; f++) below = below || cnt[b][f] != 0;
        }
        DevBuf<uint64_t> rk; DevBuf<V> rv;
        if (!rk.alloc(m + h) || !rv.alloc(m + h)) { cdm_set_error("cdm_kmermatch: out of device memory for a pass over %llu k-mer tuples", m + h); return CDM_ERR_HIP; }
        unsigned long long at = 0, hat = m;
        for (int b = 0; b < B; b++) {
            if (mine[b] == 0 && !(r == P - 1 && cnt[b][F])) continue;
            std::unique_ptr<KmerJob<LY>> again;
            if (!keepAll) { again.reset(new KmerJob<LY>(ctx, db, par)); if (int rc = extractBlock(*again, b)) return rc; }
            KmerJob<LY> &ex = keepAll ? *kept[b] : *again;
            if ((unsigned long long) (ex.sendOff[f1] - ex.sendOff[f0]) != mine[b] || ex.sendHash != cnt[b][F]) { cdm_set_error("cdm_kmermatch: internal error: a block's tuple counts changed between two extractions"); return CDM_ERR_HIP; }
            if (mine[b]) {
                hipMemcpyAsync(rk.p + at, (const uint64_t *) ex.sendKeys + ex.sendOff[f0], mine[b] * 8, hipMemcpyDeviceToDevice, s);
                hipMemcpyAsync(rv.p + at, (const V *) ex.sendVals + ex.sendOff[f0], mine[b] * sizeof(V), hipMemcpyDeviceToDevice, s);
                at += mine[b];
            }
            if (r == P - 1 && cnt[b][F]) {
                hipMemcpyAsync(rk.p + hat, ex.sendHashKeys, cnt[b][F] * 8, hipMemcpyDeviceToDevice, s);
                hipMemcpyAsync(rv.p + hat, ex.sendHashVals, cnt[b][F] * sizeof(V), hipMemcpyDeviceToDevice, s);
                hat += cnt[b][F];
            }
            if (hipStreamSynchronize(s) != hipSuccess) { cdm_set_error("cdm_kmermatch: gathering a pass's tuples failed: %s", hipGetErrorString(hipGetLastError())); return CDM_ERR_HIP; }
        }
        job.part = r; job.nparts = P;
        return job.rangeFinishOwned(rk, rv, m, h, below);
    };
    DevBuf<uint64_t> G; unsigned long long gCap = 0, gCount = 0, J = 0;
    std::vector<unsigned long long> realOf((size_t) P, 0);
    DevBuf<unsigned long long> cntDev;
    if (!cntDev.alloc(1)) { cdm_set_error("cdm_kmermatch: out of device memory"); return CDM_ERR_HIP; }
    auto ownerOf = [&](int r) { return (int) ((long long) r * W / P); };
    std::vector<unsigned long long> keptOf((size_t) P, 0);
    for (int r = 0; r < P; r++) {
        if (ownerOf(r) != R) continue;
        KmerJob<LY> job(ctx, db, par);
        if (int rc = runRange(r, job)) return rc;
        realOf[r] = job.live + job.regionTwo; J += job.nKept; keptOf[r] = job.nKept;
        const unsigned long long nt = job.nTuples;
        if (stats) fprintf(stderr, "kmermatch pass %d of %d: %llu tuples, %llu kept\n", r + 1, P, nt, job.nKept);
        if (nt == 0) continue;
        if (gCount + nt > gCap) {
            const unsigned long long want = std::max(gCount + nt, gCap * 2);
            DevBuf<uint64_t> bigger;
            if (!bigger.alloc(want)) { cdm_set_error("cdm_kmermatch: out of device memory for %llu group keys", want); return CDM_ERR_HIP; }
            if (gCount) hipMemcpyAsync(bigger.p, G.p, gCount * 8, hipMemcpyDeviceToDevice, s);
            if (hipStreamSynchronize(s) != hipSuccess) { cdm_set_error("cdm_kmermatch: growing the group key array failed"); return CDM_ERR_HIP; }
            G.free(); G.p = bigger.release(); gCap = want;
        }
        DevBuf<uint8_t> d0, d1;
        if (!d0.alloc(nt) || !d1.alloc(nt)) { cdm_set_error("cdm_kmermatch: out of device memory"); return CDM_ERR_HIP; }
        if (int rc = rx::compactPairs<uint64_t, uint8_t>(s, (const uint64_t *) job.startIo, d0.p, (uint64_t) nt, G.p + gCount, d1.p, cntDev.p)) return rc;
        unsigned long long got = 0;
        hipMemcpyAsync(&got, cntDev.p, 8, hipMemcpyDeviceToHost, s);
        if (hipStreamSynchronize(s) != hipSuccess) { cdm_set_error("cdm_kmermatch: collecting a pass's group keys failed"); return CDM_ERR_HIP; }
        gCount += got;
    }
    if (W > 1) {
        std::vector<unsigned long long> mine(2 * (size_t) P + 1), all((2 * (size_t) P + 1) * W);
        for (int r = 0; r < P; r++) { mine[2 * r] = realOf[r]; mine[2 * r + 1] = keptOf[r]; }
        mine[2 * (size_t) P] = gCount;
        if (int rc = ranks->gatherHost(ranks->user, mine.data(), all.data(), mine.size() * 8)) return rc;
        J = 0;
        std::vector<uint64_t> recvOff((size_t) W + 1, 0);
        for (int p = 0; p < W; p++) {
            const unsigned long long *a = all.data() + (size_t) p * mine.size();
            for (int r = 0; r < P; r++) if (ownerOf(r) == p) { realOf[r] = a[2 * r]; J += a[2 * r + 1]; }
            recvOff[p + 1] = recvOff[p] + a[2 * (size_t) P] * 8;
        }
        const unsigned long long total = recvOff[W] / 8;
        DevBuf<uint64_t> whole;
        if (!whole.alloc(total)) { cdm_set_error("cdm_kmermatch: out of device memory for %llu group keys of all ranks", total); return CDM_ERR_HIP; }
        if (!G.p && !G.alloc(0)) { cdm_set_error("cdm_kmermatch: out of device memory"); return CDM_ERR_HIP; }
        if (int rc = ranks->gatherDev(ranks->user, G.p, gCount * 8, whole.p, recvOff.data(), s)) return rc;
        if (hipStreamSynchronize(s) != hipSuccess) { cdm_set_error("cdm_kmermatch: gathering the ranks' group keys failed: %s", hipGetErrorString(hipGetLastError())); return CDM_ERR_HIP; }
        G.free(); G.p = whole.release(); gCount = total; gCap = total;
    }
    uint32_t stale[CDM_STALE_MAX + 5]; memset(stale, 0, sizeof(stale));
    if (J) {
        int holder = -1; unsigned long long jLocal = 0, base = 0;
        for (int r = 0; r < P; r++) { if (J < base + realOf[r]) { holder = r; jLocal = J - base; break; } base += realOf[r]; }
        uint32_t got = 0; bool have = false; uint32_t target = 0;
        for (int r = holder; holder >= 0 && r < P; r++) {
            KmerJob<LY> job(ctx, db, par);
            if (int rc = runRange(r, job)) return rc;
            if (int rc = job.staleTail(r == holder ? jLocal : 0)) return rc;
            const uint32_t *l = job.staleHost;
            if (l[0]) {
                if (!have) { target = l[1]; have = true; } else if (l[1] != target) break;
                for (uint32_t j = 0; j < l[0] && got < (uint32_t) CDM_STALE_MAX; j++) stale[2 + got++] = l[2 + j];
            }
            if (!l[CDM_STALE_MAX + 4]) break;
        }
        if (got >= (uint32_t) CDM_STALE_MAX) { cdm_set_error("cdm_kmermatch: the reference's last per-target scan would run over %d or more left-over tuples; not reproduced", CDM_STALE_MAX); return CDM_ERR_UNSUPPORTED; }
        stale[0] = got; stale[1] = have ? target : 0;
    }
    for (auto &q : kept) q.reset();
    KmerJob<LY> fin(ctx, db, par);
    fin.passes = true;
    if (int rc = fin.init()) return rc;
    if (!fin.staleBuf.alloc(STALE_MAX + 3) || !fin.k0.alloc(gCount)) { cdm_set_error("cdm_kmermatch: out of device memory"); return CDM_ERR_HIP; }
    if (hipMemcpyAsync(fin.staleBuf.p, stale, (STALE_MAX + 3) * 4, hipMemcpyHostToDevice, s) != hipSuccess || hipStreamSynchronize(s) != hipSuccess) { cdm_set_error("cdm_kmermatch: stale list upload failed"); return CDM_ERR_HIP; }
    if (!G.p && !G.alloc(0)) { cdm_set_error("cdm_kmermatch: out of device memory"); return CDM_ERR_HIP; }
    fin.startIo = (unsigned long long *) G.p; fin.live = gCount; fin.kmerSlots = gCount; fin.nTuples = gCount; fin.nKept = J;
    fin.keys = DoubleBuf<uint64_t>(fin.k0.p, G.p);
    if (int rc = fin.sort2(G.p, gCount, gCount, gCount, fin.k0.p, G.p, true)) return rc;
    return fin.vote(nullptr, true, out);
}
template <typename LY>
int kmermatchT(cdm_ctx *ctx, const cdm_seqdb *db, const cdm_kmer_params *par, cdm_hits **out, const KmerRanks *ranks, const Db &d) {
    PassPlan pl = passPlan(d, sizeof(typename LY::V));
    if (const char *e = cdmGetenv("CDM_KMER_PASSES")) { pl.P = atoi(e); const char *c = strchr(e, ','); pl.B = c ? atoi(c + 1) : pl.P; }
    const int P = pl.P, B = pl.B;
    if (ranks && ranks->world > 1) return kmermatchPassesT<LY>(ctx, db, par, std::max(P, ranks->world), std::max(B, 1), out, ranks);
    if (P > 1 || B > 1) return kmermatchPassesT<LY>(ctx, db, par, std::max(P, 1), std::max(B, 1), out);
    KmerJob<LY> job(ctx, db, par);
    job.ownPipeline = true;
    if (int rc = job.phaseA()) return rc;
    if (job.nKept) if (int rc = job.staleTail(job.nKept)) return rc;
    return job.phaseB(out);
}

Switches layoutSwitches() {
    Switches sw;
    if (const char *e = cdmGetenv("CDM_KMER_LAYOUT")) sw.layout = !strcmp(e, "wide") ? LayoutSwitch::Wide : !strcmp(e, "packed") ? LayoutSwitch::Packed : !strcmp(e, "slot") ? LayoutSwitch::Slot : LayoutSwitch::Other;
    sw.forceHuge = cdmGetenv("CDM_FORCE_HUGE_LAYOUT"); sw.forceWideKey = cdmGetenv("CDM_FORCE_WIDE_KEY"); sw.kmerSort = cdmGetenv("CDM_KMER_SORT"); sw.kmerPasses = cdmGetenv("CDM_KMER_PASSES");
    return sw;
}
template <typename F> auto withLayout(Layout l, F f) -> decltype(f(LayoutHuge())) {
    return l == Layout::Slot ? f(LayoutSlot()) : l == Layout::Packed ? f(LayoutPacked()) : l == Layout::Wide ? f(LayoutWide()) : l == Layout::Long ? f(LayoutLong()) : f(LayoutHuge());
}

}

struct cdm_kpart { KmerJobBase *job = nullptr; uint64_t nSeq = 0; uint32_t repShift = 0; bool gatheredDone = false; };
int cdm_kmermatch_part_takes_slots(const cdm_seqdb *db, const cdm_kmer_params *par) {
    return chooseLayout(Entry::Part, planDb(db, par->kmer_size, true), layoutSwitches()) == Layout::Slot ? 1 : 0;
}
template <typename Start>
static int openPart(const char *entry, Entry e, cdm_ctx *ctx, const cdm_seqdb *db, const cdm_kmer_params *par, cdm_kpart **out, Start start) {
    if (cdmGetenv("CDM_KMER_SORT") || cdmGetenv("CDM_KMER_SORT2")) { cdm_set_error("%s: the A/B switches CDM_KMER_SORT / CDM_KMER_SORT2 apply to the single-device path only", entry); return CDM_ERR_INVALID; }
    CDM_HIP(hipSetDevice(ctx->device));
    const Db d = planDb(db, par->kmer_size, e == Entry::Part);
    const Layout l = chooseLayout(e, d, layoutSwitches());
    if (l == Layout::TooLong) { cdm_set_error("%s: sequences of %u letters or more are not implemented", entry, MAX_SEQ_LETTERS); return CDM_ERR_UNSUPPORTED; }
    cdm_kpart *h = new cdm_kpart();
    h->job = withLayout(l, [&](auto ly) -> KmerJobBase * { auto *j = new KmerJob<decltype(ly)>(ctx, db, par); j->headRange = decltype(ly)::bySlot; return j; });
    h->nSeq = db->n; h->repShift = repShiftOf(d);
    const int rc = start(*h->job);
    if (rc != CDM_OK) { cdm_kpart_free(h); return rc; }
    *out = h;
    return CDM_OK;
}
extern "C" int cdm_kmermatch_part(cdm_ctx *ctx, const cdm_seqdb *db, const cdm_kmer_params *par, int part, int nparts, cdm_kpart **out) {
    if (!ctx || !db || !par || !out || nparts < 1 || part < 0 || part >= nparts) { cdm_set_error("cdm_kmermatch_part: invalid argument"); return CDM_ERR_INVALID; }
    return openPart("cdm_kmermatch_part", Entry::Part, ctx, db, par, out, [&](KmerJobBase &j) { j.part = part; j.nparts = nparts; return j.phaseA(); });
}
extern "C" int cdm_kmermatch_split_begin(cdm_ctx *ctx, const cdm_seqdb *db, const cdm_kmer_params *par, int rank, int nranks, cdm_kpart **out) {
    if (!ctx || !db || !par || !out || nranks < 1 || rank < 0 || rank >= nranks) { cdm_set_error("cdm_kmermatch_split_begin: invalid argument"); return CDM_ERR_INVALID; }
    return openPart("cdm_kmermatch_split_begin", Entry::SplitBegin, ctx, db, par, out, [&](KmerJobBase &j) { j.part = 0; j.nparts = CDM_KPART_SLICES; j.block = rank; j.nBlocks = nranks; return j.splitBegin(); });
}
extern "C" int cdm_kpart_outgoing(const cdm_kpart *h, uint64_t *offsets, const void **keys, const void **vals, int *valBytes, const void **hashKeys, const void **hashVals, uint64_t *nHash) {
    if (!h || !h->job->split || !offsets || !keys || !vals || !valBytes || !hashKeys || !hashVals || !nHash) { cdm_set_error("cdm_kpart_outgoing: invalid argument"); return CDM_ERR_INVALID; }
    for (int p = 0; p <= CDM_KPART_SLICES; p++) offsets[p] = h->job->sendOff[p];
    *keys = h->job->sendKeys; *vals = h->job->sendVals; *valBytes = h->job->valBytes;
    *hashKeys = h->job->sendHashKeys; *hashVals = h->job->sendHashVals; *nHash = h->job->sendHash;
    return CDM_OK;
}
int cdm_kmermatch_needs_wide_key(const cdm_seqdb *db) {
    return needsWideKey(planDb(db, 0), cdmGetenv("CDM_FORCE_WIDE_KEY") != nullptr) ? 1 : 0;
}
extern "C" int cdm_kpart_set_range(cdm_kpart *h, int rank, int nranks) {
    if (!h || !h->job->split || nranks < 1 || rank < 0 || rank >= nranks) { cdm_set_error("cdm_kpart_set_range: invalid argument"); return CDM_ERR_INVALID; }
    h->job->block = rank; h->job->nBlocks = nranks;
    return CDM_OK;
}
extern "C" int cdm_kmermatch_split_finish(cdm_ctx *ctx, cdm_kpart *h, const void *keys, const void *vals, uint64_t m, const void *hashKeys, const void *hashVals, uint64_t nHash, int below) {
    if (!ctx || !h || !h->job->split || (m && (!keys || !vals)) || (nHash && (!hashKeys || !hashVals))) { cdm_set_error("cdm_kmermatch_split_finish: invalid argument"); return CDM_ERR_INVALID; }
    h->job->part = h->job->block; h->job->nparts = h->job->nBlocks;
    if (nHash && h->job->part != h->job->nparts - 1) { cdm_set_error("cdm_kmermatch_split_finish: the whole-sequence hash tuples belong to the last rank"); return CDM_ERR_INVALID; }
    CDM_HIP(hipSetDevice(ctx->device));
    return h->job->splitFinish(keys, vals, m, hashKeys, hashVals, nHash, below != 0);
}
extern "C" void cdm_kpart_free(cdm_kpart *h) { if (!h) return; delete h->job; delete h; }
extern "C" int cdm_kpart_info(const cdm_kpart *h, uint64_t info[4]) {
    info[0] = h->job->live + h->job->regionTwo; info[1] = h->job->nKept; info[2] = h->job->anyBelow ? 1 : 0; info[3] = h->nSeq;
    return CDM_OK;
}
extern "C" int cdm_kpart_stale(cdm_ctx *ctx, cdm_kpart *h, uint64_t J, uint32_t out[67]) {
    CDM_HIP(hipSetDevice(ctx->device));
    const int rc = h->job->staleTail(J);
    if (rc != CDM_OK) return rc;
    memcpy(out, h->job->staleHost, 67 * sizeof(uint32_t));
    return CDM_OK;
}
extern "C" int cdm_kpart_gather_at(cdm_ctx *ctx, cdm_kpart *h, int nb, const uint64_t *bounds, uint64_t *offsets, const void **devKeys) {
    if (nb < 1 || !bounds || !offsets || !devKeys) { cdm_set_error("cdm_kpart_gather_at: invalid argument"); return CDM_ERR_INVALID; }
    CDM_HIP(hipSetDevice(ctx->device));
    if (!h->gatheredDone) { const int rc = h->job->gatherByRep(); if (rc != CDM_OK) return rc; h->gatheredDone = true; }
    DevBuf<uint64_t> dBound; DevBuf<unsigned long long> dOut;
    if (!dBound.alloc(nb) || !dOut.alloc(nb)) { cdm_set_error("cdm_kpart_gather_at: out of device memory"); return CDM_ERR_HIP; }
    CDM_HIP(hipMemcpyAsync(dBound.p, bounds, (size_t) nb * 8, hipMemcpyHostToDevice, ctx->stream));
    hipLaunchKernelGGL(k_rep_bounds, dim3((nb + 63) / 64), dim3(64), 0, ctx->stream, (const uint64_t *) h->job->gathered, (uint64_t) h->job->nKept, (int) h->repShift, (const uint64_t *) dBound.p, nb, dOut.p);
    std::vector<unsigned long long> o((size_t) nb);
    CDM_HIP(hipMemcpyAsync(o.data(), dOut.p, (size_t) nb * 8, hipMemcpyDeviceToHost, ctx->stream));
    CDM_HIP(hipStreamSynchronize(ctx->stream));
    for (int t = 0; t < nb; t++) offsets[t] = o[t];
    *devKeys = h->job->gathered;
    return CDM_OK;
}
extern "C" int cdm_kpart_gather(cdm_ctx *ctx, cdm_kpart *h, int nranks, uint64_t *offsets, const void **devKeys) {
    if (nranks < 1 || !offsets || !devKeys) { cdm_set_error("cdm_kpart_gather: invalid argument"); return CDM_ERR_INVALID; }
    std::vector<uint64_t> bound((size_t) nranks + 1);
    for (int r = 0; r <= nranks; r++) bound[r] = (uint64_t) ((unsigned __int128) h->nSeq * (unsigned) r / (unsigned) nranks);
    if (int rc = cdm_kpart_gather_at(ctx, h, nranks + 1, bound.data(), offsets, devKeys)) return rc;
    offsets[nranks] = h->job->nKept;
    return CDM_OK;
}
extern "C" int cdm_kpart_sort(cdm_ctx *ctx, cdm_kpart *h, const void *devKeys, uint64_t nKeys, uint32_t *head, uint64_t info[2]) {
    if (!head || !info || (nKeys && !devKeys)) { cdm_set_error("cdm_kpart_sort: invalid argument"); return CDM_ERR_INVALID; }
    CDM_HIP(hipSetDevice(ctx->device));
    return h->job->sortFrom((const uint64_t *) devKeys, nKeys, head, info);
}
extern "C" int cdm_kpart_vote(cdm_ctx *ctx, cdm_kpart *h, const uint32_t *cont, const uint32_t *stale, cdm_hits **out) {
    if (!out || !stale) { cdm_set_error("cdm_kpart_vote: invalid argument"); return CDM_ERR_INVALID; }
    CDM_HIP(hipSetDevice(ctx->device));
    return h->job->voteWith(cont, stale, out);
}
extern "C" int cdm_kpart_cont_cap(void) { return CONT_CAP; }
extern "C" int cdm_kmer_slot_split(int k, int *low_bits) {
    if (!low_bits) { cdm_set_error("cdm_kmer_slot_split: invalid argument"); return CDM_ERR_INVALID; }
    Db d; d.n = 1; d.maxLen = 64; d.residues = 64; d.k = k;
    if (!slotLayoutFits(d)) { cdm_set_error("cdm_kmer_slot_split: the slot layout takes 14 <= k <= 20 (got %d)", k); return CDM_ERR_INVALID; }
    return slotSplit(k, *low_bits);
}
extern "C" int cdm_dev_copy(cdm_ctx *ctx, void *dst, const void *src, uint64_t bytes) {
    CDM_HIP(hipSetDevice(ctx->device));
    if (bytes) CDM_HIP(hipMemcpyAsync(dst, src, bytes, hipMemcpyDeviceToDevice, ctx->stream));
    CDM_HIP(hipStreamSynchronize(ctx->stream));
    return CDM_OK;
}

int cdm_kmermatch_impl(cdm_ctx *ctx, const cdm_seqdb *db, const cdm_kmer_params *par, cdm_hits **out) { return cdm_kmermatch_ranks_impl(ctx, db, par, nullptr, out); }
int cdm_kmermatch_ranks_impl(cdm_ctx *ctx, const cdm_seqdb *db, const cdm_kmer_params *par, const KmerRanks *ranks, cdm_hits **out) {
    const Db d = planDb(db, par->kmer_size, true);
    const Layout l = chooseLayout(Entry::Single, d, layoutSwitches(), ranks != nullptr);
    switch (l) {
        case Layout::PackedUnfit: cdm_set_error("cdm_kmermatch: CDM_KMER_LAYOUT=packed needs 2k + 1 + 2 x length bits <= 63 (k %d, max length %u)", d.k, db->maxLen); return CDM_ERR_INVALID;
        case Layout::BadSwitch: cdm_set_error("cdm_kmermatch: CDM_KMER_LAYOUT must be wide, packed or slot"); return CDM_ERR_INVALID;
        case Layout::SlotUnfit: cdm_set_error("cdm_kmermatch: CDM_KMER_LAYOUT=slot needs sequences of one length (at least k letters), fewer than 2^32 k-mer slots and 14 <= k <= 20"); return CDM_ERR_INVALID;
        case Layout::TooLong: cdm_set_error("cdm_kmermatch: sequences of %u letters or more are not implemented", MAX_SEQ_LETTERS); return CDM_ERR_UNSUPPORTED;
        default: break;
    }
    return withLayout(l, [&](auto ly) { return kmermatchT<decltype(ly)>(ctx, db, par, out, ranks, d); });
}
```

carpedeam_amd/csrc/runsort.h:

```cpp
#pragma once
#include "bucket.h"
#include "devutil.h"

namespace runsort {

#ifndef CDM_RUN_ITEMS
#define CDM_RUN_ITEMS 16
#endif
constexpr int RUN_ITEMS = CDM_RUN_ITEMS, RUN_NT = 256, RUN_TILE = RUN_NT * RUN_ITEMS;
static_assert(RUN_ITEMS == 8 || RUN_ITEMS == 16, "the boundary bits of a thread are one byte or one 16-bit word");
template <int N> struct RunBitsOf { typedef uint16_t T; };
template <> struct RunBitsOf<8> { typedef uint8_t T; };
typedef RunBitsOf<RUN_ITEMS>::T RunBits;
constexpr int RUN_CNT_BITS = 13;

constexpr uint64_t GK_START = 1ull << 62, GK_DROPPED = 1ull << 63;
__host__ __device__ __forceinline__ bool gkKept(uint64_t k) { return (k >> 63) == 0ull; }
struct RunArgs {
    const uint64_t *keys;
    uint64_t n;
    uint64_t skipLo, skipHi;
    uint64_t base = 0;
    int repShift;
    int wide = 0, idShift = 0; uint64_t idMask = 0;
};
__device__ __forceinline__ int runPad(int i) { return i + (i >> 4); }
constexpr int RUN_LDS = RUN_TILE + RUN_TILE / 16 + 1;

constexpr uint32_t RUN_NONE = 0xFFFFFFFFu;
__device__ __forceinline__ void runRepsWide(const RunArgs &a, uint64_t base, bool skip, uint32_t *sRep) {
    __shared__ unsigned long long sKept[RUN_TILE / 64];
    __shared__ uint32_t sWaveLast[RUN_NT / 64], sCarry;
    __shared__ int sNeed;
    const int lane = threadIdx.x & 63, wave = threadIdx.x >> 6;
    if (threadIdx.x == 0) { sNeed = 0; sCarry = RUN_NONE; }
#pragma unroll
    for (int j = 0; j < RUN_ITEMS; j++) {
        const int li = threadIdx.x + RUN_NT * j; const uint64_t i = base + (uint64_t) li;
        const uint64_t k = (!skip && i < a.n && !(i >= a.skipLo && i < a.skipHi)) ? a.keys[i] : ~0ull;
        const bool start = k != ~0ull && (k & GK_START) != 0ull;
        sRep[runPad(li)] = start ? (uint32_t) ((k >> a.idShift) & a.idMask) : RUN_NONE;
        const unsigned long long kb = __ballot(gkKept(k));
        if (lane == 0) sKept[(RUN_NT * j + 64 * wave) >> 6] = kb;
    }
    __syncthreads();
    uint32_t mine = RUN_NONE;
#pragma unroll
    for (int j = 0; j < RUN_ITEMS; j++) { const uint32_t r = sRep[runPad(threadIdx.x * RUN_ITEMS + j)]; if (r != RUN_NONE) mine = r; }
    uint32_t incl = mine;
#pragma unroll
    for (int d = 1; d < 64; d <<= 1) { const uint32_t o = (uint32_t) __shfl_up((int) incl, d, 64); if (lane >= d && incl == RUN_NONE) incl = o; }
    if (lane == 63) sWaveLast[wave] = incl;
    uint32_t carry = (uint32_t) __shfl_up((int) incl, 1, 64);
    if (lane == 0) carry = RUN_NONE;
    __syncthreads();
    for (int w = wave - 1; w >= 0 && carry == RUN_NONE; w--) carry = sWaveLast[w];
    uint32_t cur = carry; bool need = false;
    const unsigned int keptBits = (unsigned int) ((sKept[(threadIdx.x * RUN_ITEMS) >> 6] >> ((threadIdx.x * RUN_ITEMS) & 63)) & ((1u << RUN_ITEMS) - 1u));
    uint32_t out[RUN_ITEMS];
#pragma unroll
    for (int j = 0; j < RUN_ITEMS; j++) {
        const uint32_t r = sRep[runPad(threadIdx.x * RUN_ITEMS + j)];
        if (r != RUN_NONE) cur = r;
        const bool kept = (keptBits >> j) & 1u;
        out[j] = kept ? cur : RUN_NONE;
        need |= kept && cur == RUN_NONE;
    }
    if (need) sNeed = 1;
    __syncthreads();
    if (sNeed) {
        if (wave == 0) {
            uint64_t hi = base;
            uint32_t found = RUN_NONE;
            while (hi > 0) {
                const uint64_t i = hi - 1 - (uint64_t) lane;
                const uint64_t k = (hi > (uint64_t) lane) ? a.keys[i] : ~0ull;
                const unsigned long long sm = __ballot(k != ~0ull && (k & GK_START) != 0ull);
                if (sm) { const int l = __ffsll(sm) - 1; found = (uint32_t) ((bucket::readLane64(k, l) >> a.idShift) & a.idMask); break; }
                hi = hi > 64 ? hi - 64 : 0;
            }
            if (lane == 0) sCarry = found;
        }
        __syncthreads();
        const uint32_t c = sCarry;
#pragma unroll
        for (int j = 0; j < RUN_ITEMS; j++) if (((keptBits >> j) & 1u) && out[j] == RUN_NONE) out[j] = c;
    }
    __syncthreads();
#pragma unroll
    for (int j = 0; j < RUN_ITEMS; j++) sRep[runPad(threadIdx.x * RUN_ITEMS + j)] = out[j];
}
__device__ __forceinline__ void runFlags(const RunArgs &a, uint64_t base, uint32_t *sRep, unsigned int &startBits, unsigned int &boundBits) {
    const bool skip = base >= a.skipLo && base + RUN_TILE <= a.skipHi;
    if (a.wide) runRepsWide(a, base, skip, sRep);
    else {
#pragma unroll
    for (int j = 0; j < RUN_ITEMS; j++) {
        const int li = threadIdx.x + RUN_NT * j; const uint64_t i = base + (uint64_t) li;
        const uint64_t k = (!skip && i < a.n && !(i >= a.skipLo && i < a.skipHi)) ? a.keys[i] : ~0ull;
        sRep[runPad(li)] = k != ~0ull ? (uint32_t) (k >> a.repShift) : RUN_NONE;
    }
    }
    __syncthreads();
    startBits = 0; boundBits = 0;
    uint32_t prev = (threadIdx.x == 0) ? RUN_NONE : sRep[runPad(threadIdx.x * RUN_ITEMS - 1)];
#pragma unroll
    for (int j = 0; j < RUN_ITEMS; j++) {
        const uint32_t r = sRep[runPad(threadIdx.x * RUN_ITEMS + j)];
        const bool kept = r != RUN_NONE;
        const bool start = kept && r != prev;
        if (start) startBits |= 1u << j;
        if (start || !kept) boundBits |= 1u << j;
        prev = r;
    }
}
__global__ __launch_bounds__(RUN_NT) void k_run_count(RunArgs a, unsigned long long *__restrict__ tileCnt) {
    __shared__ uint32_t sKeys[RUN_LDS];
    unsigned int sb, bb;
    runFlags(a, (uint64_t) blockIdx.x * RUN_TILE, sKeys, sb, bb);
    const unsigned int tot = cdm_block_sum<unsigned int>((unsigned int) __popc(sb));
    if (threadIdx.x == 0) tileCnt[blockIdx.x] = tot;
}
__global__ __launch_bounds__(RUN_NT) void k_run_write(RunArgs a, const unsigned long long *__restrict__ tileOff, uint32_t *__restrict__ recRep, uint64_t *__restrict__ recVal) {
    __shared__ uint32_t sKeys[RUN_LDS];
    __shared__ __align__(8) RunBits sBound[RUN_NT + 32 / sizeof(RunBits)];
    const uint64_t base = (uint64_t) blockIdx.x * RUN_TILE;
    unsigned int sb, bb;
    runFlags(a, base, sKeys, sb, bb);
    sBound[threadIdx.x] = (RunBits) bb;
    if (threadIdx.x < 32 / sizeof(RunBits)) sBound[RUN_NT + threadIdx.x] = 0;
    unsigned int tot;
    unsigned long long rank = tileOff[blockIdx.x] + cdm_block_excl_sum<unsigned int>((unsigned int) __popc(sb), tot);
    const unsigned long long *words = reinterpret_cast<const unsigned long long *>(sBound);
#pragma unroll 1
    while (sb) {
        const int j = __ffs(sb) - 1;
        sb &= sb - 1;
        const int li = threadIdx.x * RUN_ITEMS + j;
        int e = RUN_TILE;
        for (int w = (li + 1) >> 6; w < RUN_TILE / 64; w++) {
            unsigned long long m = words[w];
            if (w == ((li + 1) >> 6)) m &= ~0ull << ((li + 1) & 63);
            if (m) { e = w * 64 + __ffsll(m) - 1; break; }
        }
        recRep[rank] = sKeys[runPad(li)];
        recVal[rank] = ((a.base + base + (uint64_t) li) << RUN_CNT_BITS) | (uint64_t) (e - li);
        rank++;
    }
}
constexpr unsigned long long RS_AGG = 1ull << 62, RS_PREFIX = 2ull << 62, RS_MASK = (1ull << 62) - 1ull;
struct RunScan { unsigned long long *status; unsigned int *ticket; unsigned long long *total; unsigned int *overflow; unsigned long long cap; unsigned long long tiles; };
__global__ __launch_bounds__(RUN_NT) void k_run_records(RunArgs a, RunScan sc, uint32_t *__restrict__ recRep, uint64_t *__restrict__ recVal) {
    __shared__ uint32_t sKeys[RUN_LDS];
    __shared__ __align__(8) RunBits sBound[RUN_NT + 32 / sizeof(RunBits)];
    __shared__ unsigned int sTile;
    __shared__ unsigned long long sPrefix;
    if (threadIdx.x == 0) sTile = atomicAdd(sc.ticket, 1u);
    __syncthreads();
    const unsigned long long tile = sTile;
    const uint64_t base = (uint64_t) tile * RUN_TILE;
    unsigned int sb, bb;
    runFlags(a, base, sKeys, sb, bb);
    sBound[threadIdx.x] = (RunBits) bb;
    if (threadIdx.x < 32 / sizeof(RunBits)) sBound[RUN_NT + threadIdx.x] = 0;
    unsigned int tot;
    const unsigned int ex = cdm_block_excl_sum<unsigned int>((unsigned int) __popc(sb), tot);
    if (threadIdx.x < 64) {
        const int lane = threadIdx.x;
        unsigned long long excl = 0;
        if (tile == 0) { if (lane == 0) __hip_atomic_store(&sc.status[0], RS_PREFIX | (unsigned long long) tot, __ATOMIC_RELAXED, __HIP_MEMORY_SCOPE_AGENT); }
        else {
            if (lane == 0) __hip_atomic_store(&sc.status[tile], RS_AGG | (unsigned long long) tot, __ATOMIC_RELAXED, __HIP_MEMORY_SCOPE_AGENT);
            long long t0 = (long long) tile - 1;
            while (true) {
                const long long t = t0 - lane;
                unsigned long long v = RS_PREFIX;
                if (t >= 0) do { v = __hip_atomic_load(&sc.status[t], __ATOMIC_RELAXED, __HIP_MEMORY_SCOPE_AGENT); } while ((v >> 62) == 0ull);
                const unsigned long long pm = __ballot((v >> 62) == 2ull);
                const int first = pm ? __ffsll(pm) - 1 : 63;
                const unsigned long long part = cdm_wave_incl_sum<unsigned long long>(lane <= first ? (v & RS_MASK) : 0ull);
                excl += (unsigned long long) __shfl((long long) part, 63, 64);
                if (pm) break;
                t0 -= 64;
            }
            if (lane == 0) __hip_atomic_store(&sc.status[tile], RS_PREFIX | (excl + tot), __ATOMIC_RELAXED, __HIP_MEMORY_SCOPE_AGENT);
        }
        if (lane == 0) {
            sPrefix = excl;
            if (tile + 1 == sc.tiles) *sc.total = excl + tot;
            if (excl + tot > sc.cap) *sc.overflow = 1u;
        }
    }
    __syncthreads();
    unsigned long long rank = sPrefix + ex;
    if (sPrefix + tot > sc.cap) return;
    const unsigned long long *words = reinterpret_cast<const unsigned long long *>(sBound);
#pragma unroll 1
    while (sb) {
        const int j = __ffs(sb) - 1;
        sb &= sb - 1;
        const int li = threadIdx.x * RUN_ITEMS + j;
        int e = RUN_TILE;
        for (int w = (li + 1) >> 6; w < RUN_TILE / 64; w++) {
            unsigned long long m = words[w];
            if (w == ((li + 1) >> 6)) m &= ~0ull << ((li + 1) & 63);
            if (m) { e = w * 64 + __ffsll(m) - 1; break; }
        }
        recRep[rank] = sKeys[runPad(li)];
        recVal[rank] = ((a.base + base + (uint64_t) li) << RUN_CNT_BITS) | (uint64_t) (e - li);
        rank++;
    }
}
struct RunLen { const uint64_t *recVal; __device__ __forceinline__ unsigned long long operator()(size_t j) const { return recVal[j] & ((1ull << RUN_CNT_BITS) - 1ull); } };

template <typename Put>
__device__ __forceinline__ unsigned int waveGatherRecords(const uint64_t *__restrict__ keys, const uint64_t *__restrict__ recVal, const unsigned long long *__restrict__ dst,
                                                          uint64_t nRec, uint64_t j0, unsigned long long end, int lane, uint32_t *sOff, uint64_t *sStart, const Put &put) {
    const uint64_t j = j0 + lane;
    const bool valid = j < nRec && dst[j] < end;
    const uint64_t rv = valid ? recVal[j] : 0ull;
    const unsigned int cnt = (unsigned int) (rv & ((1ull << RUN_CNT_BITS) - 1ull));
    const unsigned int incl = cdm_wave_incl_sum<unsigned int>(cnt);
    sOff[lane] = incl - cnt; sStart[lane] = rv >> RUN_CNT_BITS;
    const unsigned int total = (unsigned int) __shfl((int) incl, 63, 64);
    bucket::waveLdsSync();
    for (unsigned int e = lane; e < total; e += 64) {
        int r = 0;
#pragma unroll
        for (int s = 32; s > 0; s >>= 1) if (sOff[r + s] <= e) r += s;
        put(e, keys[sStart[r] + (e - sOff[r])]);
    }
    bucket::waveLdsSync();
    return total;
}
__global__ __launch_bounds__(256) void k_run_gather(const uint64_t *__restrict__ keys, const uint64_t *__restrict__ recVal, const unsigned long long *__restrict__ dst,
                                                    uint64_t nRec, uint64_t *__restrict__ out) {
    __shared__ uint32_t sOffAll[4][64];
    __shared__ uint64_t sStartAll[4][64];
    const int lane = threadIdx.x & 63, wave = threadIdx.x >> 6;
    const uint64_t j0 = ((uint64_t) blockIdx.x * 4 + wave) * 64;
    if (j0 >= nRec) return;
    const unsigned long long d0 = dst[j0];
    waveGatherRecords(keys, recVal, dst, nRec, j0, ~0ull, lane, sOffAll[wave], sStartAll[wave], [&](unsigned int e, uint64_t t) { out[d0 + e] = t; });
}
__global__ __launch_bounds__(256) void k_gather_ranges(const unsigned long long *__restrict__ list, const unsigned int *__restrict__ count, const uint64_t *__restrict__ keys,
                                                       const uint64_t *__restrict__ recVal, const unsigned long long *__restrict__ dst, uint64_t nRec, uint64_t *__restrict__ out) {
    __shared__ uint32_t sOffAll[4][64];
    __shared__ uint64_t sStartAll[4][64];
    const int lane = threadIdx.x & 63, wave = threadIdx.x >> 6;
    const unsigned int n = *count;
    for (unsigned int item = blockIdx.x; item < n; item += gridDim.x) {
        const unsigned long long s = list[2 * (size_t) item], e = list[2 * (size_t) item + 1];
        uint64_t lo = 0, hi = nRec;
        while (lo < hi) { const uint64_t mid = lo + ((hi - lo) >> 1); if (dst[mid] < s) lo = mid + 1; else hi = mid; }
        for (uint64_t j0 = lo + 64ull * wave; j0 < nRec; j0 += 256) {
            const unsigned long long d0 = dst[j0];
            if (d0 >= e) break;
            waveGatherRecords(keys, recVal, dst, nRec, j0, e, lane, sOffAll[wave], sStartAll[wave], [&](unsigned int x, uint64_t t) { out[d0 + x] = t; });
        }
    }
}

constexpr int U_T = 1024;
constexpr int SEG_CLASSES = 4;
struct SegListArgs {
    const uint32_t *recRep; const unsigned long long *dst; uint64_t nRec;
    uint32_t maxWave;
    const unsigned long long *uEnd; uint64_t units;
    uint32_t cap[SEG_CLASSES - 1];
    unsigned long long *list[SEG_CLASSES]; unsigned int *cnt;
    const unsigned long long *segFirstRec = nullptr; uint64_t nSeg = 0;
};
__global__ __launch_bounds__(1024) void k_seg_list(SegListArgs a) {
    const uint64_t j = (uint64_t) blockIdx.x * blockDim.x + threadIdx.x;
    int cls = -1; unsigned long long s = 0, e = 0;
    if (j < a.nRec) {
        const uint32_t rep = a.recRep[j];
        if (j == 0 || a.recRep[j - 1] != rep) {
            uint64_t lo = j, step = 1;
            while (lo + step < a.nRec && a.recRep[lo + step] == rep) { lo += step; step <<= 1; }
            uint64_t hi = min(lo + step, a.nRec);
            while (hi - lo > 1) { const uint64_t mid = lo + ((hi - lo) >> 1); if (a.recRep[mid] == rep) lo = mid; else hi = mid; }
            s = a.dst[j]; e = a.dst[hi];
            const unsigned long long n = e - s;
            const bool inUnit = a.uEnd && s / U_T < a.units && e <= a.uEnd[s / U_T];
            if (n > a.maxWave && !inUnit) cls = n <= a.cap[0] ? 0 : n <= a.cap[1] ? 1 : n <= a.cap[2] ? 2 : 3;
        }
    }
    if (!__syncthreads_or(cls >= 0)) return;
#pragma unroll
    for (int c = 0; c < SEG_CLASSES; c++) {
        const uint32_t q = cdm_block_append(a.cnt + c, cls == c);
        if (cls == c) { a.list[c][2 * (size_t) q] = s; a.list[c][2 * (size_t) q + 1] = e; }
    }
}

__global__ __launch_bounds__(1024) void k_seg_list_segments(SegListArgs a) {
    const uint64_t g = (uint64_t) blockIdx.x * blockDim.x + threadIdx.x;
    int cls = -1; unsigned long long s = 0, e = 0;
    if (g < a.nSeg) {
        s = a.dst[a.segFirstRec[g]]; e = a.dst[a.segFirstRec[g + 1]];
        const unsigned long long n = e - s;
        const bool inUnit = a.uEnd && s / U_T < a.units && e <= a.uEnd[s / U_T];
        if (n > a.maxWave && !inUnit) cls = n <= a.cap[0] ? 0 : n <= a.cap[1] ? 1 : n <= a.cap[2] ? 2 : 3;
    }
    if (!__syncthreads_or(cls >= 0)) return;
#pragma unroll
    for (int c = 0; c < SEG_CLASSES; c++) {
        const uint32_t q = cdm_block_append(a.cnt + c, cls == c);
        if (cls == c) { a.list[c][2 * (size_t) q] = s; a.list[c][2 * (size_t) q + 1] = e; }
    }
}

#ifndef CDM_U_NT
#define CDM_U_NT 512
#endif
#ifndef CDM_U_NT0
#define CDM_U_NT0 256
#define CDM_U_NT1 256
#endif
constexpr int U_MAXSEG = 2048, U_CAP = U_T + U_MAXSEG, U_NB = 256, U_IDXB = 12, U_ORDB = 11;
constexpr int U_CLASSES = 3;
constexpr int U_CLASS_CAP[U_CLASSES] = {1536, 2048, U_CAP};
constexpr int U_CLASS_NT[U_CLASSES] = {CDM_U_NT0, CDM_U_NT1, CDM_U_NT};
static_assert(U_CAP <= (1 << U_IDXB) && U_T <= (1 << U_ORDB), "unit sorter geometry");

struct UnitBoundArgs {
    const uint32_t *recRep; const unsigned long long *dst; uint64_t nRec;
    uint32_t maxSeg; uint64_t units;
    unsigned long long *uStart, *uEnd, *uRec;
    const uint32_t *segOfRec = nullptr; const unsigned long long *segFirstRec = nullptr;
};
__global__ __launch_bounds__(1024) void k_unit_bounds(UnitBoundArgs a) {
    const uint64_t r = (uint64_t) blockIdx.x * blockDim.x + threadIdx.x;
    if (r >= a.nRec) return;
    const unsigned long long d0 = a.dst[r], d1 = a.dst[r + 1];
    const uint64_t uLo = d0 / U_T + 1, uHi = (r == a.nRec - 1) ? a.units : d1 / U_T;
    if (r == 0) { a.uStart[0] = 0; a.uRec[0] = 0; }
    if (uLo > uHi) return;
    uint64_t hi, first;
    if (a.segFirstRec) { const uint32_t g = a.segOfRec[r]; first = a.segFirstRec[g]; hi = a.segFirstRec[g + 1]; }
    else {
        const uint32_t rep = a.recRep[r];
        uint64_t lo = r, step = 1;
        while (lo + step < a.nRec && a.recRep[lo + step] == rep) { lo += step; step <<= 1; }
        hi = min(lo + step, a.nRec);
        while (hi - lo > 1) { const uint64_t mid = lo + ((hi - lo) >> 1); if (a.recRep[mid] == rep) lo = mid; else hi = mid; }
        first = r; uint64_t out = ~0ull, st = 1;
        while (first >= st) { if (a.recRep[first - st] == rep) { first -= st; st <<= 1; } else { out = first - st; break; } }
        while (first - out > 1) { const uint64_t mid = out + ((first - out) >> 1); if (a.recRep[mid] == rep) first = mid; else out = mid; }
    }
    const unsigned long long e = a.dst[hi];
    const unsigned long long sSeg = a.dst[first];
    for (uint64_t u = uLo; u <= uHi; u++) {
        if (u <= a.units) { a.uStart[u] = e; a.uRec[u] = hi; }
        const bool mine = sSeg >= (u - 1) * (unsigned long long) U_T;
        if (u >= 1 && u - 1 < a.units) a.uEnd[u - 1] = (mine && e - sSeg > a.maxSeg) ? sSeg : e;
    }
}
struct UnitClassArgs {
    const unsigned long long *uStart, *uEnd, *uRec; uint64_t units, n;
    uint32_t cap[U_CLASSES];
    unsigned long long *list[U_CLASSES]; unsigned int *cnt;
};
__global__ __launch_bounds__(1024) void k_unit_classes(UnitClassArgs a) {
    const uint64_t u = (uint64_t) blockIdx.x * blockDim.x + threadIdx.x;
    int cls = -1; unsigned long long s = 0, e = 0, r0 = 0;
    if (u < a.units) {
        s = a.uStart[u]; e = a.uEnd[u]; r0 = a.uRec[u];
        const unsigned long long m = e > s ? e - s : 0;
        if (m) cls = m <= a.cap[0] ? 0 : m <= a.cap[1] ? 1 : 2;
    }
#pragma unroll
    for (int c = 0; c < U_CLASSES; c++) {
        const uint32_t q = cdm_block_append(a.cnt + c, cls == c);
        if (cls == c) { a.list[c][3 * (size_t) q] = s; a.list[c][3 * (size_t) q + 1] = e; a.list[c][3 * (size_t) q + 2] = r0; }
    }
}

struct UnitArgs {
    const uint64_t *keys; const uint64_t *recVal; const unsigned long long *dst; uint64_t nRec;
    uint64_t *out; uint64_t n;
    int repShift;
    int hiShift;
    uint32_t maxSub;
    const unsigned long long *list; const unsigned int *count;
    bucket::BigList hard;
};
__device__ __forceinline__ unsigned long long j0Next(const unsigned long long *__restrict__ dst, uint64_t nRec, uint64_t j) { return dst[min(j, nRec)]; }
#ifndef CDM_U_MINW
#define CDM_U_MINW 5
#endif
template <int CAP, int U_NT>
__global__ __launch_bounds__(U_NT, CDM_U_MINW) void k_unit_sort(UnitArgs a) {
    constexpr int ROUNDS = (CAP + U_NT - 1) / U_NT, U_WAVES = U_NT / 64;
    static_assert(U_NB <= U_NT && U_NB % U_WAVES == 0 && CAP % U_NT == 0, "unit sorter geometry");
    __shared__ uint64_t sKeys[CAP];
    constexpr int SHARE_BYTES = (CAP * 2 > U_NT * 12) ? CAP * 2 : U_NT * 12;
    __shared__ __align__(8) unsigned char sShare[SHARE_BYTES];
    uint16_t *sPerm = reinterpret_cast<uint16_t *>(sShare);
    uint64_t *sGStart = reinterpret_cast<uint64_t *>(sShare);
    uint32_t *sGOff = reinterpret_cast<uint32_t *>(sShare + U_NT * 8);
    __shared__ unsigned long long sBits[ROUNDS * U_NT / 64];
    __shared__ unsigned int sPre[ROUNDS * U_NT / 64];
    __shared__ unsigned int sCnt[U_NB];
    __shared__ unsigned int sOff[U_NB + 1];
    __shared__ uint32_t sRep[U_T + 2];
    const int tid = threadIdx.x, lane = tid & 63, wave = tid >> 6;
    const unsigned int nUnits = *a.count;
    for (unsigned int item = blockIdx.x; item < nUnits; item += gridDim.x) {
        const uint64_t base = a.list[3 * (size_t) item];
        const int m = (int) (a.list[3 * (size_t) item + 1] - base);
        const uint64_t rec0 = a.list[3 * (size_t) item + 2];
        {
            if (tid < U_NB) sCnt[tid] = 0;
            const unsigned long long endG = base + (uint64_t) m;
            for (uint64_t c0 = rec0; c0 < a.nRec; c0 += U_NT) {
                const uint64_t j = c0 + tid;
                const unsigned long long d = j < a.nRec ? a.dst[j] : ~0ull;
                const bool valid = d < endG;
                sGOff[tid] = valid ? (uint32_t) (d - base) : (uint32_t) m;
                sGStart[tid] = valid ? (a.recVal[j] >> RUN_CNT_BITS) : 0ull;
                const int nr = __syncthreads_count(valid);
                if (nr == 0) break;
                const int e0 = (int) sGOff[0], e1 = (nr == U_NT) ? (int) min((unsigned long long) m, (j0Next(a.dst, a.nRec, c0 + U_NT) - base)) : m;
                for (int e = e0 + tid; e < e1; e += U_NT) {
                    int r = 0;
#pragma unroll
                    for (int st = U_NT / 2; st > 0; st >>= 1) if (r + st < nr && (int) sGOff[r + st] <= e) r += st;
                    sKeys[e] = a.keys[sGStart[r] + (uint64_t) (e - (int) sGOff[r])];
                }
                __syncthreads();
                if (nr < U_NT) break;
            }
            __syncthreads();
#pragma unroll
            for (int r = 0; r < ROUNDS; r++) {
                const int i = r * U_NT + tid;
                const uint64_t k = i < m ? sKeys[i] : ~0ull, p = (i && i < m) ? sKeys[i - 1] : 0ull;
                const unsigned long long bm = __ballot(i < m && (i == 0 || (k >> a.repShift) != (p >> a.repShift)));
                if (lane == 0) sBits[i >> 6] = bm;
            }
            __syncthreads();
        }
        if (wave == 0) {
            unsigned int run = 0;
#pragma unroll
            for (int w0 = 0; w0 < ROUNDS * U_NT / 64; w0 += 64) {
                const unsigned int c = (w0 + lane < ROUNDS * U_NT / 64) ? (unsigned int) __popcll(sBits[w0 + lane]) : 0u;
                const unsigned int incl = cdm_wave_incl_sum<unsigned int>(c);
                if (w0 + lane < ROUNDS * U_NT / 64) sPre[w0 + lane] = run + incl - c;
                run += __shfl(incl, 63, 64);
            }
        }
        __syncthreads();
        const int idBits = a.repShift - a.hiShift;
        const unsigned int nSeg = sPre[(m - 1) >> 6] + (unsigned int) __popcll(sBits[(m - 1) >> 6] & ((2ull << ((m - 1) & 63)) - 1ull));
        const uint64_t range = ((uint64_t) nSeg << idBits) - 1ull;
        const int bl = range ? 64 - __clzll((long long) range) : 0, sh = max(0, bl - 8) + a.hiShift;
        const uint64_t lowRep = (1ull << a.repShift) - 1ull;
        for (int i = tid; i < m; i += U_NT) {
            const unsigned long long w = sBits[i >> 6];
            const unsigned int o = sPre[i >> 6] + (unsigned int) __popcll(w & ((2ull << (i & 63)) - 1ull)) - 1u;
            const uint64_t k = sKeys[i];
            if ((w >> (i & 63)) & 1ull) sRep[o] = (uint32_t) (k >> a.repShift);
            const uint64_t t = ((uint64_t) o << a.repShift) | (k & lowRep);
            sKeys[i] = t;
            atomicAdd(&sCnt[(unsigned int) (t >> sh)], 1u);
        }
        __syncthreads();
        const unsigned int c = tid < U_NB ? sCnt[tid] : 0u;
        unsigned int tot;
        const unsigned int ex = cdm_block_excl_sum<unsigned int>(c, tot);
        if (tid < U_NB) sOff[tid] = ex;
        if (tid == 0) sOff[U_NB] = tot;
        const bool hard = __syncthreads_or(c > a.maxSub);
        if (hard) { if (tid == 0) a.hard.add(base, base + (uint64_t) m); continue; }
        if (tid < U_NB) sCnt[tid] = ex;
        __syncthreads();
        for (int i = tid; i < m; i += U_NT) sPerm[atomicAdd(&sCnt[(unsigned int) (sKeys[i] >> sh)], 1u)] = (uint16_t) i;
        __syncthreads();
        constexpr int PER = U_NB / U_WAVES;
        auto sortRange = [&](int g0, int gm) {
            bucket::sortGroup<uint64_t>(gm, lane,
                [&](int i) { const int e = sPerm[g0 + i]; return ((sKeys[e] >> 1) << U_IDXB) | (uint64_t) e; },
                [&](auto &v) {
                    constexpr int R = sizeof(v) / sizeof(v[0]);
#pragma unroll
                    for (int r = 0; r < R; r++) {
                        const int p = lane * R + r;
                        if (p < gm) { const uint64_t t = sKeys[(int) (v[r] & ((1u << U_IDXB) - 1u))]; a.out[base + (uint64_t) (g0 + p)] = ((uint64_t) sRep[t >> a.repShift] << a.repShift) | (t & lowRep); }
                    }
                });
        };
        int b = wave * PER;
        const int bLast = b + PER;
        const int w0 = (int) sOff[b], wm = (int) sOff[bLast] - w0;
        if (wm <= bucket::BK_MAXB) { if (wm > 0) sortRange(w0, wm); }
        else while (b < bLast) {
            const int g0 = (int) sOff[b];
            int bE = b + 1;
            while (bE < bLast && (int) sOff[bE + 1] - g0 <= bucket::BK_GROUP) bE++;
            const int gm = (int) sOff[bE] - g0;
            if (gm > 0) sortRange(g0, gm);
            b = bE;
        }
        __syncthreads();
    }
}

__global__ __launch_bounds__(256) void k_gather_ranges_dense(const unsigned long long *__restrict__ ranges, unsigned int cnt, const uint64_t *__restrict__ keys,
                                                             const uint64_t *__restrict__ recVal, const unsigned long long *__restrict__ dst, uint64_t nRec,
                                                             const uint32_t *__restrict__ segOfRec, uint64_t keyMask, uint64_t *__restrict__ dense, uint32_t *__restrict__ ord) {
    __shared__ uint32_t sOffAll[4][64];
    __shared__ uint64_t sStartAll[4][64];
    const int lane = threadIdx.x & 63, wave = threadIdx.x >> 6;
    uint32_t *sOff = sOffAll[wave]; uint64_t *sStart = sStartAll[wave];
    for (unsigned int item = blockIdx.x; item < cnt; item += gridDim.x) {
        const unsigned long long s = ranges[3 * (size_t) item], e = ranges[3 * (size_t) item + 1], o = ranges[3 * (size_t) item + 2];
        uint64_t lo = 0, hi = nRec;
        while (lo < hi) { const uint64_t mid = lo + ((hi - lo) >> 1); if (dst[mid] < s) lo = mid + 1; else hi = mid; }
        for (uint64_t j0 = lo + 64ull * wave; j0 < nRec; j0 += 256) {
            const unsigned long long d0 = dst[j0];
            if (d0 >= e) break;
            const uint64_t j = j0 + lane;
            const bool valid = j < nRec && dst[j] < e;
            const uint64_t rv = valid ? recVal[j] : 0ull;
            const unsigned int len = (unsigned int) (rv & ((1ull << RUN_CNT_BITS) - 1ull));
            const unsigned int incl = cdm_wave_incl_sum<unsigned int>(len);
            sOff[lane] = incl - len; sStart[lane] = rv >> RUN_CNT_BITS;
            const unsigned int total = (unsigned int) __shfl((int) incl, 63, 64);
            bucket::waveLdsSync();
            for (unsigned int x = lane; x < total; x += 64) {
                int r = 0;
#pragma unroll
                for (int st = 32; st > 0; st >>= 1) if (sOff[r + st] <= x) r += st;
                const unsigned long long at = o + (d0 - s) + x;
                dense[at] = keys[sStart[r] + (x - sOff[r])] & keyMask;
                ord[at] = segOfRec[j0 + (uint64_t) r];
            }
            bucket::waveLdsSync();
        }
    }
}
typedef void (*UnitHook)(hipStream_t s, unsigned int grid, const unsigned long long *list, const unsigned int *count, bucket::BigList hard, void *user);
inline int segmentedSortKeys(hipStream_t s, int cuCount, uint64_t *in, uint64_t *out, uint64_t n, int shiftHi, int hiShift, int top,
                             const uint32_t *recRep, const unsigned long long *dst, uint64_t nRec, const uint64_t *srcKeys, const uint64_t *recVal,
                             UnitHook unitHook = nullptr, void *hookUser = nullptr, bool wide = false, const uint32_t *segOfRec = nullptr, int segBits = 0,
                             const unsigned long long *segFirstRec = nullptr, uint64_t nSeg = 0) {
    using namespace bucket;
    if (n == 0) return CDM_OK;
    if (wide && (!unitHook || !segOfRec)) { cdm_set_error("segmented sort: keys without the representative need the aggregating unit kernel and its segment table"); return CDM_ERR_UNSUPPORTED; }
    uint32_t maxSeg = U_MAXSEG, blockCap = wide ? 0 : 4096;
    if (const char *e = cdmGetenv("CDM_UNIT_CAP")) { const long m = atol(e); if (m >= 1 && m <= U_MAXSEG) maxSeg = (uint32_t) m; }
    if (const char *e = cdmGetenv("CDM_BLOCK_CAP")) { const long m = atol(e); if (m >= 0 && m <= 4096) blockCap = (uint32_t) m; }
    uint32_t maxSub = BK_MAXB;
    if (const char *e = cdmGetenv("CDM_UNIT_SUB")) { const long m = atol(e); if (m >= 1 && m <= BK_MAXB) maxSub = (uint32_t) m; }
    if (shiftHi - 1 + BLK_IDX > 64) blockCap = 0;
    if (!unitHook && U_ORDB + shiftHi - 1 + U_IDXB > 64) maxSeg = 0;
    const uint64_t units = (n + U_T - 1) / U_T;
    const size_t listCap = (size_t) (n / ((uint64_t) maxSeg + 1) + 2);
    DevBuf<unsigned long long> lists[SEG_CLASSES], hardList, uStart, uEnd, uRec, uList[U_CLASSES]; DevBuf<unsigned int> cnt;
    constexpr int NCNT = SEG_CLASSES + 1 + U_CLASSES;
    if (!cnt.alloc(NCNT) || !hardList.alloc(2 * (size_t) (units + 1)) || !uStart.alloc(units + 2) || !uEnd.alloc(units + 1) || !uRec.alloc(units + 2)) return CDM_ERR_HIP;
    for (int c = 0; c < U_CLASSES; c++) if (!uList[c].alloc(3 * (size_t) (units + 1))) return CDM_ERR_HIP;
    for (int c = 2; c < SEG_CLASSES; c++) if (!lists[c].alloc(2 * (listCap + (c == 3 ? (size_t) units + 1 : 0)))) return CDM_ERR_HIP;
    hipMemsetAsync(cnt.p, 0, NCNT * 4, s);
    if (maxSeg) {
        hipMemsetAsync(uStart.p, 0, (units + 2) * 8, s); hipMemsetAsync(uEnd.p, 0, (units + 1) * 8, s); hipMemsetAsync(uRec.p, 0, (units + 2) * 8, s);
        UnitBoundArgs ub; ub.recRep = recRep; ub.dst = dst; ub.nRec = nRec; ub.maxSeg = maxSeg; ub.units = units; ub.uStart = uStart.p; ub.uEnd = uEnd.p; ub.uRec = uRec.p;
        if (segOfRec && segFirstRec) { ub.segOfRec = segOfRec; ub.segFirstRec = segFirstRec; }
        hipLaunchKernelGGL(k_unit_bounds, CDM_GRID((nRec + 1023) / 1024, 1024), dim3(1024), 0, s, ub);
        UnitClassArgs uc; uc.uStart = uStart.p; uc.uEnd = uEnd.p; uc.uRec = uRec.p; uc.units = units; uc.n = n;
        for (int c = 0; c < U_CLASSES; c++) { uc.cap[c] = (uint32_t) U_CLASS_CAP[c]; uc.list[c] = uList[c].p; }
        uc.cnt = cnt.p + SEG_CLASSES + 1;
        hipLaunchKernelGGL(k_unit_classes, dim3((unsigned) ((units + 1023) / 1024)), dim3(1024), 0, s, uc);
        UnitArgs ua; ua.keys = srcKeys; ua.recVal = recVal; ua.dst = dst; ua.nRec = nRec; ua.out = out; ua.n = n; ua.repShift = shiftHi; ua.hiShift = hiShift; ua.maxSub = maxSub; ua.hard.list = hardList.p; ua.hard.cnt = cnt.p + SEG_CLASSES;
        const unsigned int pad = cdm_lds_pad("CDM_LDS_PAD_UNIT");
        const unsigned int grid = (unsigned int) std::min<uint64_t>(units, (uint64_t) cuCount * 64);
        if (unitHook) {
            for (int c = 0; c < U_CLASSES; c++) unitHook(s, grid, uList[c].p, cnt.p + SEG_CLASSES + 1 + c, ua.hard, hookUser);
        } else {
        ua.list = uList[0].p; ua.count = cnt.p + SEG_CLASSES + 1; hipLaunchKernelGGL((k_unit_sort<U_CLASS_CAP[0], U_CLASS_NT[0]>), dim3(grid), dim3(U_CLASS_NT[0]), pad, s, ua);
        ua.list = uList[1].p; ua.count = cnt.p + SEG_CLASSES + 2; hipLaunchKernelGGL((k_unit_sort<U_CLASS_CAP[1], U_CLASS_NT[1]>), dim3(grid), dim3(U_CLASS_NT[1]), pad, s, ua);
        ua.list = uList[2].p; ua.count = cnt.p + SEG_CLASSES + 3; hipLaunchKernelGGL((k_unit_sort<U_CLASS_CAP[2], U_CLASS_NT[2]>), dim3(grid), dim3(U_CLASS_NT[2]), pad, s, ua);
        }
    }
    SegListArgs la; la.recRep = recRep; la.dst = dst; la.nRec = nRec; la.maxWave = maxSeg; la.uEnd = maxSeg ? uEnd.p : nullptr; la.units = units;
    la.cap[0] = 0; la.cap[1] = 0; la.cap[2] = blockCap;
    for (int c = 0; c < SEG_CLASSES; c++) la.list[c] = lists[c].p;
    la.cnt = cnt.p;
    if (segFirstRec && nSeg) { la.segFirstRec = segFirstRec; la.nSeg = nSeg; hipLaunchKernelGGL(k_seg_list_segments, CDM_GRID((nSeg + 1023) / 1024, 1024), dim3(1024), 0, s, la); }
    else hipLaunchKernelGGL(k_seg_list, CDM_GRID((nRec + 1023) / 1024, 1024), dim3(1024), 0, s, la);
    const unsigned int gatherGrid = (unsigned int) std::min<uint64_t>((uint64_t) cuCount * 8, listCap + units + 1);
    BlockSortArgs ba; ba.in = in; ba.out = out; ba.shiftHi = shiftHi; ba.ign = 1;
    ba.list = lists[2].p; ba.count = cnt.p + 2;
    if (blockCap) hipLaunchKernelGGL(k_gather_ranges, dim3(gatherGrid), dim3(256), 0, s, (const unsigned long long *) lists[2].p, (const unsigned int *) (cnt.p + 2), srcKeys, recVal, dst, nRec, in);
    if (blockCap) hipLaunchKernelGGL(k_block_sort<8>, dim3((unsigned int) std::min<uint64_t>((uint64_t) cuCount * 8, listCap)), dim3(512), 0, s, ba);
    unsigned int hc[NCNT] = {0};
    if (hipMemcpyAsync(hc, cnt.p, NCNT * 4, hipMemcpyDeviceToHost, s) != hipSuccess || hipStreamSynchronize(s) != hipSuccess) return CDM_ERR_HIP;
    if (cdmGetenv("CDM_BUCKET_STATS")) fprintf(stderr, "segmentedSortKeys%s: n %llu, %llu records, %llu units (%u / %u / %u by size class): segments > %u: %u (<= %u, block sort), %u longer (global radix sort); %u hard units (global radix sort)\n",
                                            unitHook ? " (units aggregated)" : "", (unsigned long long) n, (unsigned long long) nRec, (unsigned long long) units, hc[SEG_CLASSES + 1], hc[SEG_CLASSES + 2], hc[SEG_CLASSES + 3], maxSeg, hc[2], blockCap, hc[3], hc[SEG_CLASSES]);
    const unsigned int nBig = hc[3] + hc[SEG_CLASSES];
    if (nBig == 0) return CDM_OK;
    if (hc[SEG_CLASSES]) hipMemcpyAsync(lists[3].p + 2 * (size_t) hc[3], hardList.p, 2 * (size_t) hc[SEG_CLASSES] * 8, hipMemcpyDeviceToDevice, s);
    if (!wide) {
        DevBuf<unsigned int> nb;
        if (!nb.alloc(1)) return CDM_ERR_HIP;
        hipMemcpyAsync(nb.p, &nBig, 4, hipMemcpyHostToDevice, s);
        hipLaunchKernelGGL(k_gather_ranges, dim3(gatherGrid), dim3(256), 0, s, (const unsigned long long *) lists[3].p, (const unsigned int *) nb.p, srcKeys, recVal, dst, nRec, in);
        if (hipStreamSynchronize(s) != hipSuccess) return CDM_ERR_HIP;
    }
    DevBuf<unsigned long long> ranges; uint64_t total = 0;
    if (int rc = loadBigList(s, lists[3].p, nBig, ranges, total)) return rc;
    DevBuf<uint64_t> d0, d1;
    if (!d0.alloc(total) || !d1.alloc(total)) return CDM_ERR_HIP;
    const unsigned int g = bigCopyGrid(nBig);
    bool inFirst = true;
    if (wide) {
        DevBuf<uint32_t> o0, o1;
        if (!o0.alloc(total) || !o1.alloc(total)) return CDM_ERR_HIP;
        hipLaunchKernelGGL(k_gather_ranges_dense, dim3(gatherGrid), dim3(256), 0, s, (const unsigned long long *) ranges.p, nBig, srcKeys, recVal, dst, nRec, segOfRec, (1ull << shiftHi) - 1ull, d0.p, o0.p);
        if (int rc = rx::sortPairs<uint64_t, uint32_t>(s, cuCount, d0.p, d1.p, o0.p, o1.p, total, 1, shiftHi, inFirst)) return rc;
        uint64_t *kA = inFirst ? d0.p : d1.p, *kB = inFirst ? d1.p : d0.p; uint32_t *oA = inFirst ? o0.p : o1.p, *oB = inFirst ? o1.p : o0.p;
        bool second = true;
        if (int rc = rx::sortPairs<uint32_t, uint64_t>(s, cuCount, oA, oB, kA, kB, total, 0, std::max(1, segBits), second)) return rc;
        hipLaunchKernelGGL((k_big_copy<uint64_t, false>), dim3(g), dim3(256), 0, s, (const unsigned long long *) ranges.p, nBig, out, second ? kA : kB);
    } else {
    hipLaunchKernelGGL((k_big_copy<uint64_t, true>), dim3(g), dim3(256), 0, s, (const unsigned long long *) ranges.p, nBig, const_cast<uint64_t *>(in), d0.p);
    if (int rc = rx::sortKeys<uint64_t>(s, cuCount, d0.p, d1.p, total, 1, top, inFirst)) return rc;
    hipLaunchKernelGGL((k_big_copy<uint64_t, false>), dim3(g), dim3(256), 0, s, (const unsigned long long *) ranges.p, nBig, out, inFirst ? d0.p : d1.p);
    }
    if (hipStreamSynchronize(s) != hipSuccess) return CDM_ERR_HIP;
    return CDM_OK;
}

inline int makeRunRecords(hipStream_t s, const RunArgs &ra, DevBuf<uint32_t> &rr0, DevBuf<uint32_t> &rr1, DevBuf<uint64_t> &rv0, DevBuf<uint64_t> &rv1, unsigned long long &nRec) {
    const uint64_t tiles = (ra.n + RUN_TILE - 1) / RUN_TILE;
    nRec = 0;
    if (tiles == 0) return CDM_OK;
    const char *mode = cdmGetenv("CDM_RUN_RECORDS");
    unsigned long long cap = ra.n / 8 + 4096;
    if (const char *e = cdmGetenv("CDM_RUN_CAP")) cap = strtoull(e, nullptr, 10);
    if (!(mode && !strcmp(mode, "twopass"))) {
        DevBuf<unsigned long long> status, total; DevBuf<unsigned int> flags;
        if (!status.alloc(tiles) || !total.alloc(1) || !flags.alloc(2) || !rr0.alloc(cap) || !rr1.alloc(cap) || !rv0.alloc(cap + 1) || !rv1.alloc(cap + 1)) { cdm_set_error("run records: out of device memory"); return CDM_ERR_HIP; }
        hipMemsetAsync(status.p, 0, tiles * 8, s); hipMemsetAsync(total.p, 0, 8, s); hipMemsetAsync(flags.p, 0, 8, s);
        RunScan sc; sc.status = status.p; sc.ticket = flags.p; sc.overflow = flags.p + 1; sc.total = total.p; sc.cap = cap; sc.tiles = tiles;
        hipLaunchKernelGGL(k_run_records, dim3((unsigned) tiles), dim3(RUN_NT), 0, s, ra, sc, rr0.p, rv0.p);
        unsigned int fl[2] = {0, 0};
        hipMemcpyAsync(&nRec, total.p, 8, hipMemcpyDeviceToHost, s); hipMemcpyAsync(fl, flags.p, 8, hipMemcpyDeviceToHost, s);
        if (hipStreamSynchronize(s) != hipSuccess) { cdm_set_error("run records failed: %s", hipGetErrorString(hipGetLastError())); return CDM_ERR_HIP; }
        if (!fl[1]) return CDM_OK;
        rr0.free(); rr1.free(); rv0.free(); rv1.free();
    }
    DevBuf<unsigned long long> tileCnt, tileOff; cdmscan::ScanTemp st;
    if (!tileCnt.alloc(tiles + 1) || !tileOff.alloc(tiles + 1)) { cdm_set_error("run records: out of device memory"); return CDM_ERR_HIP; }
    hipMemsetAsync(tileCnt.p + tiles, 0, 8, s);
    hipLaunchKernelGGL(k_run_count, dim3((unsigned) tiles), dim3(RUN_NT), 0, s, ra, tileCnt.p);
    if (int rc = cdmscan::exclusiveScan<unsigned long long>(s, st, tileCnt.p, tileOff.p, (size_t) tiles + 1)) return rc;
    hipMemcpyAsync(&nRec, tileOff.p + tiles, 8, hipMemcpyDeviceToHost, s);
    if (hipStreamSynchronize(s) != hipSuccess) { cdm_set_error("run records failed: %s", hipGetErrorString(hipGetLastError())); return CDM_ERR_HIP; }
    if (!rr0.alloc(nRec) || !rr1.alloc(nRec) || !rv0.alloc(nRec + 1) || !rv1.alloc(nRec + 1)) { cdm_set_error("run records: out of device memory (%llu records)", nRec); return CDM_ERR_HIP; }
    if (nRec) hipLaunchKernelGGL(k_run_write, dim3((unsigned) tiles), dim3(RUN_NT), 0, s, ra, (const unsigned long long *) tileOff.p, rr0.p, rv0.p);
    return CDM_OK;
}

}
```

Before: 18.86 billion.

## Add small wave-sized aggregation units with front class and overflow handoff

Parametrizes the unit aggregation kernel by table size, thread count, records per thread and ordinal limit, and adds a front "wave" class of smaller unit ranges (256/512) processed by single-wave blocks with smaller shared tables. Units that overflow the small tables are appended to the regular size-class lists instead of going to the global hard sort. It also prefetches the next unit's descriptors, caches segment representatives in shared memory and reuses one shared buffer for the staging and directory arrays. The aim is higher occupancy and less per-unit overhead for small units, at the cost of more kernel variants and re-processing of the units that get handed on.

Result: faster. 19.58 billion, median of 6 (+3.8%).

```diff
diff --git a/carpedeam_amd/csrc/aggvote.h b/carpedeam_amd/csrc/aggvote.h
--- a/carpedeam_amd/csrc/aggvote.h
+++ b/carpedeam_amd/csrc/aggvote.h
@@ -32,61 +32,93 @@
     const uint64_t *sorted;
     const unsigned long long *list; const unsigned int *count;
     bucket::BigList hard;
-    unsigned int nextClass = 0;
+    const uint32_t *recRep = nullptr;
+    runsort::UnitClassLists next = {{nullptr, nullptr, nullptr}, nullptr, {0, 0, 0}, nullptr};
     int wideWord = 0;
+    int cuCount = 0, waveGeom = -1;
 };
 constexpr int AG_H = 1024, AG_D = 512, AG_IDX = 9, AG_ORD = 11;
 constexpr unsigned long long AG_CHUNK = 2048;
-inline unsigned long long aggChunkSlack(unsigned long long units, unsigned long long segments, int cuCount) {
-    const unsigned long long g = (unsigned long long) cuCount * 64;
-    return (3 * std::min(units + 1, g) + std::min(segments + 1, g)) * AG_CHUNK;
-}
-static_assert((1 << AG_IDX) >= AG_D && (1 << AG_ORD) > runsort::U_T, "aggregation geometry");
+inline unsigned int aggGridPerCu(bool waveUnits) { return waveUnits ? 32u : 64u; }
+inline unsigned long long aggChunkSlack(unsigned long long units, unsigned long long segments, int cuCount, bool waveUnits) {
+    const unsigned long long g = (unsigned long long) cuCount * 64, gu = (unsigned long long) cuCount * aggGridPerCu(waveUnits);
+    return ((waveUnits ? 4 : 3) * std::min(units + 1, gu) + std::min(segments + 1, g)) * AG_CHUNK;
+}
 __device__ __forceinline__ uint32_t aggHash(uint64_t k) { return (uint32_t) ((k * 0x9E3779B97F4A7C15ull) >> 40); }
 
 #ifndef CDM_AGG_MINW
 #define CDM_AGG_MINW 4
 #endif
-template <int NT, int ITEMS, typename W = uint64_t>
-__global__ __launch_bounds__(NT, CDM_AGG_MINW) void k_unit_agg(AggArgs a) {
+template <int NT, int ITEMS, int H, int DL, int RPT, int NO, int MINW, typename W = uint64_t>
+__global__ __launch_bounds__(NT, MINW) void k_unit_agg(AggArgs a) {
     using namespace runsort;
-    __shared__ __align__(8) unsigned char sTab[AG_H * 16];
+    constexpr int R = NT * RPT;
+    constexpr int MAXR = DL <= 64 ? 1 : DL <= 128 ? 2 : DL <= 256 ? 4 : 8;
+    static_assert((1 << AG_IDX) >= DL && (1 << AG_ORD) > NO && DL <= H, "aggregation geometry: the sort word holds (ordinal, id, diagonal, index)");
+    static_assert((R & (R - 1)) == 0 && (H & (H - 1)) == 0 && NT % 64 == 0, "aggregation geometry: powers of two");
+    __shared__ __align__(8) unsigned char sTab[H * 16];
     unsigned long long *tKey = reinterpret_cast<unsigned long long *>(sTab);
-    unsigned int *tCnt = reinterpret_cast<unsigned int *>(sTab + AG_H * 8), *tLast = reinterpret_cast<unsigned int *>(sTab + AG_H * 12);
-    unsigned int *oFirst = reinterpret_cast<unsigned int *>(sTab), *oEnt = oFirst + (U_T + 2), *oHit = oEnt + (U_T + 2);
-    static_assert(3 * (U_T + 2) * 4 <= AG_H * 16, "the directory fits the table's memory");
-    __shared__ unsigned long long dKey[AG_D];
-    __shared__ unsigned int dCnt[AG_D], dLast[AG_D];
-    __shared__ uint16_t sPerm[AG_D];
-    __shared__ uint64_t sGStart[NT];
-    __shared__ uint32_t sGOff[NT], sGSeg[NT];
-    __shared__ unsigned int sDistinct, sOver, sMaxOrd;
-    __shared__ unsigned long long sBase, sChunkAt, sChunkEnd;
+    unsigned int *tCnt = reinterpret_cast<unsigned int *>(sTab + H * 8), *tLast = reinterpret_cast<unsigned int *>(sTab + H * 12);
+    unsigned int *oFirst = reinterpret_cast<unsigned int *>(sTab), *oEnt = oFirst + (NO + 2), *oHit = oEnt + (NO + 2);
+    static_assert(3 * (NO + 2) * 4 <= H * 16, "the directory fits the table's memory");
+    constexpr int SHARE = (R * 16 > DL * 18) ? R * 16 : DL * 18;
+    __shared__ __align__(8) unsigned char sShare[SHARE];
+    uint64_t *sGStart = reinterpret_cast<uint64_t *>(sShare);
+    uint32_t *sGOff = reinterpret_cast<uint32_t *>(sShare + R * 8), *sGSeg = reinterpret_cast<uint32_t *>(sShare + R * 12);
+    unsigned long long *dKey = reinterpret_cast<unsigned long long *>(sShare);
+    unsigned int *dCnt = reinterpret_cast<unsigned int *>(sShare + DL * 8), *dLast = reinterpret_cast<unsigned int *>(sShare + DL * 12);
+    uint16_t *sPerm = reinterpret_cast<uint16_t *>(sShare + DL * 16);
+    __shared__ uint32_t sRep[NO + 1];
+    __shared__ unsigned int sDistinct, sOver, sMaxOrd, sNr[2];
+    __shared__ unsigned long long sBase, sChunkAt, sChunkEnd, sNext;
     const int tid = threadIdx.x, lane = tid & 63, wave = tid >> 6;
     const unsigned int nUnits = *a.count;
     if (tid == 0) { sChunkAt = 0; sChunkEnd = 0; }
     const int lowBits = a.repShift - 1;
     const uint64_t lowMask = (1ull << lowBits) - 1ull;
-    for (unsigned int item = blockIdx.x; item < nUnits; item += gridDim.x) {
-        const uint64_t base = a.list[3 * (size_t) item];
-        const int m = (int) (a.list[3 * (size_t) item + 1] - base);
-        const uint64_t rec0 = a.list[3 * (size_t) item + 2];
-        const uint32_t g0 = a.segOfRec[rec0];
-        for (int i = tid; i < AG_H; i += NT) { tKey[i] = ~0ull; tCnt[i] = 0u; tLast[i] = 0u; }
-        if (tid == 0) { sDistinct = 0; sOver = 0; sMaxOrd = 0; }
+    const uint32_t maxD = min(a.maxD, (uint32_t) DL);
+    unsigned int item = blockIdx.x;
+    uint64_t nBase = 0, nEnd = 0, nRec0 = 0; uint32_t nG0 = 0;
+    if (item < nUnits) { nBase = a.list[3 * (size_t) item]; nEnd = a.list[3 * (size_t) item + 1]; nRec0 = a.list[3 * (size_t) item + 2]; nG0 = a.segOfRec[nRec0]; }
+    for (; item < nUnits; item += gridDim.x) {
+        const uint64_t base = nBase;
+        const int m = (int) (nEnd - base);
+        const uint64_t rec0 = nRec0;
+        const uint32_t g0 = nG0;
+        const bool more = item + gridDim.x < nUnits;
+        if (more) { const size_t nx = (size_t) item + gridDim.x; nBase = a.list[3 * nx]; nEnd = a.list[3 * nx + 1]; nRec0 = a.list[3 * nx + 2]; }
+        for (int i = tid; i < H; i += NT) { tKey[i] = ~0ull; tCnt[i] = 0u; tLast[i] = 0u; }
+        if (tid == 0) { sDistinct = 0; sOver = 0; sMaxOrd = 0; sNr[0] = 0; sNr[1] = 0; }
         __syncthreads();
         const unsigned long long endG = base + (uint64_t) m;
-        for (uint64_t c0 = rec0; c0 < a.nRec; c0 += NT) {
-            const uint64_t j = c0 + tid;
-            const unsigned long long d = j < a.nRec ? a.dst[j] : ~0ull;
-            const bool valid = d < endG;
-            sGOff[tid] = valid ? (uint32_t) (d - base) : (uint32_t) m;
-            sGStart[tid] = valid ? (a.recVal[j] >> RUN_CNT_BITS) : 0ull;
-            sGSeg[tid] = valid ? a.segOfRec[j] - g0 : 0u;
-            const int nr = __syncthreads_count(valid);
+        int par = 0;
+        for (uint64_t c0 = rec0; c0 < a.nRec; c0 += R, par ^= 1) {
+            unsigned int nv = 0;
+#pragma unroll
+            for (int k = 0; k < RPT; k++) {
+                const int i = tid * RPT + k;
+                const uint64_t j = c0 + i;
+                const bool in = j < a.nRec;
+                const unsigned long long d = in ? a.dst[j] : ~0ull;
+                const uint64_t rv = in ? a.recVal[j] : 0ull;
+                const uint32_t sg = in ? a.segOfRec[j] : 0u, rp = in ? a.recRep[j] : 0u;
+                const bool valid = d < endG;
+                sGOff[i] = valid ? (uint32_t) (d - base) : (uint32_t) m;
+                sGStart[i] = valid ? (rv >> RUN_CNT_BITS) : 0ull;
+                sGSeg[i] = valid ? sg - g0 : 0u;
+                if (valid && sg - g0 < (uint32_t) NO) sRep[sg - g0] = rp;
+                nv += (unsigned int) __popcll(__ballot(valid));
+            }
+            if (tid == NT - 1) sNext = j0Next(a.dst, a.nRec, c0 + R);
+            if (lane == 0 && nv) atomicAdd(&sNr[par], nv);
+            __syncthreads();
+            const int nr = (int) sNr[par];
             if (nr == 0) break;
-            const int e0 = (int) sGOff[0], e1 = (nr == NT) ? (int) min((unsigned long long) m, (j0Next(a.dst, a.nRec, c0 + NT) - base)) : m;
-            if (tid == 0) sMaxOrd = max(sMaxOrd, sGSeg[nr - 1]);
+            if (tid == 0) sNr[par ^ 1] = 0u;
+            const uint32_t lastOrd = sGSeg[nr - 1];
+            if (lastOrd >= (uint32_t) NO) { if (tid == 0) sOver = 1u; break; }
+            const int e0 = (int) sGOff[0], e1 = (nr == R) ? (int) min((unsigned long long) m, sNext - base) : m;
+            if (tid == 0) sMaxOrd = max(sMaxOrd, lastOrd);
             for (int eb = e0; eb < e1; eb += NT * ITEMS) {
                 uint64_t key[ITEMS]; uint32_t ordv[ITEMS];
 #pragma unroll
@@ -95,7 +127,7 @@
                     if (e < e1) {
                         int r = 0;
 #pragma unroll
-                        for (int st = NT / 2; st > 0; st >>= 1) if (r + st < nr && (int) sGOff[r + st] <= e) r += st;
+                        for (int st = R / 2; st > 0; st >>= 1) if (r + st < nr && (int) sGOff[r + st] <= e) r += st;
                         key[k] = a.keys[sGStart[r] + (uint64_t) (e - (int) sGOff[r])];
                         ordv[k] = sGSeg[r];
                     }
@@ -106,43 +138,52 @@
                     if (e < e1) {
                         const uint64_t hk = ((uint64_t) ordv[k] << lowBits) | ((key[k] >> 1) & lowMask);
                         const unsigned int last = ((unsigned int) e << 1) | (unsigned int) (key[k] & 1ull);
-                        uint32_t h = aggHash(hk) & (AG_H - 1);
+                        uint32_t h = aggHash(hk) & (H - 1);
                         int probe = 0;
-                        for (; probe < AG_H; probe++) {
+                        for (; probe < H; probe++) {
                             unsigned long long old = __hip_atomic_load(&tKey[h], __ATOMIC_RELAXED, __HIP_MEMORY_SCOPE_WORKGROUP);
                             if (old == ~0ull) {
                                 old = atomicCAS(&tKey[h], ~0ull, (unsigned long long) hk);
                                 if (old == ~0ull) { atomicAdd(&sDistinct, 1u); old = hk; }
                             }
                             if (old == hk) { atomicAdd(&tCnt[h], 1u); atomicMax(&tLast[h], last); break; }
-                            h = (h + 1) & (AG_H - 1);
+                            h = (h + 1) & (H - 1);
                         }
-                        if (probe == AG_H) sOver = 1u;
+                        if (probe == H) sOver = 1u;
                     }
                 }
             }
-            const bool stop = __syncthreads_or(sDistinct > a.maxD || sOver != 0u);
-            if (stop || nr < NT) break;
-        }
-        __syncthreads();
-        if (sDistinct > a.maxD || sOver) {
-            if (tid == 0) a.hard.add(base, base + (uint64_t) m);
+            const bool stop = __syncthreads_or(sDistinct > maxD || sOver != 0u);
+            if (stop || nr < R) break;
+        }
+        __syncthreads();
+        if (more) nG0 = a.segOfRec[nRec0];
+        if (sDistinct > maxD || sOver) {
+            if (tid == 0) {
+                if (a.next.cnt) {
+                    int c = 0;
+                    while (c < U_CLASSES - 1 && (uint32_t) m > a.next.cap[c]) c++;
+                    const unsigned int q = atomicAdd(a.next.cnt + c, 1u);
+                    a.next.list[c][3 * (size_t) q] = base; a.next.list[c][3 * (size_t) q + 1] = base + (uint64_t) m; a.next.list[c][3 * (size_t) q + 2] = rec0;
+                    atomicAdd(a.next.handed, 1u);
+                } else a.hard.add(base, base + (uint64_t) m);
+            }
             __syncthreads();
             continue;
         }
         unsigned int c = 0;
-        for (int i = tid; i < AG_H; i += NT) c += tKey[i] != ~0ull;
+        for (int i = tid; i < H; i += NT) c += tKey[i] != ~0ull;
         unsigned int D;
         unsigned int pos = cdm_block_excl_sum<unsigned int>(c, D);
-        for (int i = tid; i < AG_H; i += NT) if (tKey[i] != ~0ull) { dKey[pos] = tKey[i]; dCnt[pos] = tCnt[i]; dLast[pos] = tLast[i]; pos++; }
+        for (int i = tid; i < H; i += NT) if (tKey[i] != ~0ull) { dKey[pos] = tKey[i]; dCnt[pos] = tCnt[i]; dLast[pos] = tLast[i]; pos++; }
         __syncthreads();
         if (wave == 0) {
-            bucket::sortGroup<W>((int) D, lane,
+            bucket::sortGroup<W, MAXR>((int) D, lane,
                 [&](int i) { return ((W) dKey[i] << AG_IDX) | (W) i; },
                 [&](auto &v) {
-                    constexpr int R = sizeof(v) / sizeof(v[0]);
-#pragma unroll
-                    for (int r = 0; r < R; r++) { const int p = lane * R + r; if (p < (int) D) sPerm[p] = (uint16_t) ((uint32_t) v[r] & ((1u << AG_IDX) - 1u)); }
+                    constexpr int RR = sizeof(v) / sizeof(v[0]);
+#pragma unroll
+                    for (int r = 0; r < RR; r++) { const int p = lane * RR + r; if (p < (int) D) sPerm[p] = (uint16_t) ((uint32_t) v[r] & ((1u << AG_IDX) - 1u)); }
                 });
         }
         const unsigned int nOrd = sMaxOrd + 1u;
@@ -162,7 +203,7 @@
             atomicAdd(&oEnt[o], 1u);
             if (p == 0 || (hk >> a.diagBits) != (prev >> a.diagBits)) {
                 const uint32_t id = (uint32_t) ((hk >> a.diagBits) & idMask);
-                if (id != a.segRep[g0 + o]) atomicAdd(&oHit[o], 1u);
+                if (id != sRep[o]) atomicAdd(&oHit[o], 1u);
             }
         }
         __syncthreads();
@@ -175,7 +216,7 @@
             }
             for (unsigned int o = tid; o < nOrd; o += NT) {
                 a.entOff[g0 + o] = b + oFirst[o]; a.entCnt[g0 + o] = oEnt[o];
-                a.perRep[a.segRep[g0 + o]] = oHit[o];
+                a.perRep[sRep[o]] = oHit[o];
             }
         }
         __syncthreads();
diff --git a/carpedeam_amd/csrc/kmermatch.hip b/carpedeam_amd/csrc/kmermatch.hip
--- a/carpedeam_amd/csrc/kmermatch.hip
+++ b/carpedeam_amd/csrc/kmermatch.hip
@@ -536,7 +536,7 @@
             bool aggregated = wide || ((ownBuffers || !(distVote && !strcmp(distVote, "tuples"))) && !sort2Check && !(voteEnv && !strcmp(voteEnv, "tuples")) && wordFits);
             if ((wide || fromStage) && ownBuffers && nGroup != nKept) { cdm_set_error("cdm_kmermatch: internal error: %llu group tuples counted, %llu in the run records", nKept, nGroup); return CDM_ERR_HIP; }
             if (aggregated) {
-                const unsigned long long slack = aggv::aggChunkSlack(nGroup / runsort::U_T, nRec, ctx->cuCount);
+                const unsigned long long slack = aggv::aggChunkSlack(nGroup / runsort::U_T, nRec, ctx->cuCount, aggWaveGeom() >= 0);
                 unsigned long long capEnt = nGroup / 6 + (4ull << 20) + slack;
                 if (const char *e = cdmGetenv("CDM_AGG_CAP")) capEnt = strtoull(e, nullptr, 10);
                 int rc = aggregate(sortedOut, nGroup, rk.current(), (const uint64_t *) rv.current(), dst.p, nRec, gk, top2, capEnt, !wordFits);
@@ -675,21 +675,51 @@
     *out = res;
     return CDM_OK;
 }
-static void aggUnitHook(hipStream_t st, unsigned int grid, const unsigned long long *list, const unsigned int *count, bucket::BigList hard, void *user) {
-    aggv::AggArgs *u = reinterpret_cast<aggv::AggArgs *>(user);
+struct AggWaveGeom { int range, nt, h, dl, no, minw, items; uint32_t cap; };
+static constexpr AggWaveGeom AGG_WAVE[] = {{256, 64, 256, 128, 32, 6, 2, 2304}, {256, 64, 256, 128, 32, 5, 4, 2304}, {256, 64, 512, 256, 32, 3, 4, 2304},
+                                           {512, 128, 512, 256, 64, 6, 2, 2560}, {512, 64, 512, 256, 64, 3, 4, 2560}, {256, 128, 256, 128, 32, 6, 2, 2304}};
+static constexpr int AGG_WAVE_GEOMS = (int) (sizeof(AGG_WAVE) / sizeof(AGG_WAVE[0])), AGG_WAVE_DEFAULT = 1;
+template <int G, typename W> static void launchWaveAgg(hipStream_t st, unsigned int grid, unsigned int pad, const aggv::AggArgs &a) {
+    constexpr AggWaveGeom g = AGG_WAVE[G];
+    hipLaunchKernelGGL((aggv::k_unit_agg<g.nt, g.items, g.h, g.dl, 2, g.no, g.minw, W>), dim3(grid), dim3(g.nt), pad, st, a);
+}
+template <typename W> static void launchWaveAggGeom(int geom, hipStream_t st, unsigned int grid, unsigned int pad, const aggv::AggArgs &a) {
+    switch (geom) {
+        case 0: launchWaveAgg<0, W>(st, grid, pad, a); break;
+        case 1: launchWaveAgg<1, W>(st, grid, pad, a); break;
+        case 2: launchWaveAgg<2, W>(st, grid, pad, a); break;
+        case 3: launchWaveAgg<3, W>(st, grid, pad, a); break;
+        case 4: launchWaveAgg<4, W>(st, grid, pad, a); break;
+        default: launchWaveAgg<5, W>(st, grid, pad, a); break;
+    }
+}
+template <int CLS, typename W> static void launchBlockAgg(hipStream_t st, unsigned int grid, unsigned int pad, const aggv::AggArgs &a) {
+    constexpr int ITEMS = runsort::U_CLASS_CAP[CLS] / 256 > 8 ? runsort::U_CLASS_CAP[CLS] / 512 : runsort::U_CLASS_CAP[CLS] / 256;
+    hipLaunchKernelGGL((aggv::k_unit_agg<256, ITEMS, aggv::AG_H, aggv::AG_D, 2, runsort::U_T, CDM_AGG_MINW, W>), dim3(grid), dim3(256), pad, st, a);
+}
+static void aggUnitHook(hipStream_t st, unsigned int grid, int cls, const unsigned long long *list, const unsigned int *count, const runsort::UnitClassLists &next, bucket::BigList hard, void *user) {
+    const aggv::AggArgs *u = reinterpret_cast<const aggv::AggArgs *>(user);
     aggv::AggArgs a = *u;
     a.list = list; a.count = count; a.hard = hard;
-    const int cls = (int) (u->nextClass++ % runsort::U_CLASSES);
     const unsigned int pad = cdm_lds_pad("CDM_LDS_PAD_AGG");
+    grid = std::min(grid, (unsigned int) u->cuCount * aggv::aggGridPerCu(u->waveGeom >= 0));
+    if (cls < 0) {
+        a.next = next;
+        if (u->wideWord) launchWaveAggGeom<bucket::u128>(u->waveGeom, st, grid, pad, a); else launchWaveAggGeom<uint64_t>(u->waveGeom, st, grid, pad, a);
+        return;
+    }
     if (u->wideWord) {
-        if (cls == 0) hipLaunchKernelGGL((aggv::k_unit_agg<256, runsort::U_CLASS_CAP[0] / 256, bucket::u128>), dim3(grid), dim3(256), pad, st, a);
-        else if (cls == 1) hipLaunchKernelGGL((aggv::k_unit_agg<256, runsort::U_CLASS_CAP[1] / 256, bucket::u128>), dim3(grid), dim3(256), pad, st, a);
-        else hipLaunchKernelGGL((aggv::k_unit_agg<256, runsort::U_CLASS_CAP[2] / 256, bucket::u128>), dim3(grid), dim3(256), pad, st, a);
+        if (cls == 0) launchBlockAgg<0, bucket::u128>(st, grid, pad, a); else if (cls == 1) launchBlockAgg<1, bucket::u128>(st, grid, pad, a); else launchBlockAgg<2, bucket::u128>(st, grid, pad, a);
         return;
     }
-    if (cls == 0) hipLaunchKernelGGL((aggv::k_unit_agg<256, runsort::U_CLASS_CAP[0] / 256>), dim3(grid), dim3(256), pad, st, a);
-    else if (cls == 1) hipLaunchKernelGGL((aggv::k_unit_agg<256, runsort::U_CLASS_CAP[1] / 256>), dim3(grid), dim3(256), pad, st, a);
-    else hipLaunchKernelGGL((aggv::k_unit_agg<256, runsort::U_CLASS_CAP[2] / 256>), dim3(grid), dim3(256), pad, st, a);
+    if (cls == 0) launchBlockAgg<0, uint64_t>(st, grid, pad, a); else if (cls == 1) launchBlockAgg<1, uint64_t>(st, grid, pad, a); else launchBlockAgg<2, uint64_t>(st, grid, pad, a);
+}
+static int aggWaveGeom() {
+    const char *m = cdmGetenv("CDM_AGG");
+    if (m && !strcmp(m, "block")) return -1;
+    int g = AGG_WAVE_DEFAULT;
+    if (const char *e = cdmGetenv("CDM_AGG_GEOM")) { const int v = atoi(e); if (v >= 0 && v < AGG_WAVE_GEOMS) g = v; }
+    return g;
 }
 int aggregate(uint64_t *sortedOut, unsigned long long nGroup, const uint32_t *recRep, const uint64_t *recVal, const unsigned long long *dst, unsigned long long nRec,
               const uint64_t *gk, int top2, unsigned long long capEnt, bool wideWord) {
@@ -712,11 +742,16 @@
     AggArgs a;
     a.keys = gk; a.recVal = recVal; a.dst = dst; a.nRec = nRec; a.segOfRec = agSegOfRec.p; a.segRep = agSegRep.p; a.segFirstRec = agSegFirstRec.p; a.nSeg = nSeg;
     a.entOff = agEntOff.p; a.entCnt = agEntCnt.p; a.perRep = agPerRep.p; a.ent = agEnt.p; a.cursor = agCursor.p; a.cap = capEnt; a.overflow = agFlags.p;
-    a.maxD = AG_D;
+    a.maxD = AG_D; a.recRep = recRep; a.cuCount = ctx->cuCount; a.waveGeom = aggWaveGeom();
+    int unitRange = runsort::U_T; uint32_t frontCap = 0;
+    if (a.waveGeom >= 0) {
+        unitRange = AGG_WAVE[a.waveGeom].range; frontCap = AGG_WAVE[a.waveGeom].cap;
+        if (const char *e = cdmGetenv("CDM_AGG_WAVE_CAP")) { const long v = atol(e); if (v >= 1 && v < (long) frontCap) frontCap = (uint32_t) v; }
+    }
     if (const char *e = cdmGetenv("CDM_AGG_D")) { const long v = atol(e); if (v >= 1 && v <= AG_D) a.maxD = (uint32_t) v; }
     a.repShift = (int) (idBits + diagBits + 1); a.diagBits = (int) diagBits; a.idBits = idBits; a.sorted = sortedOut; a.list = nullptr; a.count = nullptr; a.hard.list = nullptr; a.hard.cnt = nullptr;
     a.wideWord = wideWord ? 1 : 0;
-    if (runsort::segmentedSortKeys(s, ctx->cuCount, sortedOut, sortedOut, nGroup, (int) (idBits + diagBits + 1), (int) (diagBits + 1), top2, recRep, dst, nRec, gk, recVal, aggUnitHook, &a, wide, agSegOfRec.p, (int) bitsFor((uint64_t) nSeg + 1), agSegFirstRec.p, (uint64_t) nSeg) != CDM_OK) {
+    if (runsort::segmentedSortKeys(s, ctx->cuCount, sortedOut, sortedOut, nGroup, (int) (idBits + diagBits + 1), (int) (diagBits + 1), top2, recRep, dst, nRec, gk, recVal, aggUnitHook, &a, wide, agSegOfRec.p, (int) bitsFor((uint64_t) nSeg + 1), agSegFirstRec.p, (uint64_t) nSeg, unitRange, frontCap) != CDM_OK) {
         cdm_set_error("cdm_kmermatch: segmented sort 2 failed: %s", hipGetErrorString(hipGetLastError())); return CDM_ERR_HIP;
     }
     hipLaunchKernelGGL(k_pending_list, dim3((unsigned) (((uint64_t) nSeg + 1023) / 1024)), dim3(1024), 0, s, (const uint32_t *) agEntCnt.p, (uint64_t) nSeg, agPending.p, agFlags.p + 1);
@@ -738,6 +773,17 @@
     }
     unsigned long long used = 0;
     hipMemcpy(&used, agCursor.p, 8, hipMemcpyDeviceToHost);
+    if (cdmGetenv("CDM_BUCKET_STATS") && !fl[0]) {
+        std::vector<uint32_t> ec(nSeg);
+        hipMemcpy(ec.data(), agEntCnt.p, (size_t) nSeg * 4, hipMemcpyDeviceToHost);
+        unsigned long long written = 0;
+        for (uint32_t c : ec) written += c;
+        fprintf(stderr, "aggregate: %llu entries written (%s)\n", written, a.waveGeom >= 0 ? "wave-sized units in front" : "block form");
+        if (a.waveGeom >= 0) {
+            const AggWaveGeom &g = AGG_WAVE[a.waveGeom];
+            fprintf(stderr, "aggregate: wave-sized instance %d: unit range %d, %d threads, table of %d slots, distinct limit %d, %d records a round, %u tuples\n", a.waveGeom, g.range, g.nt, g.h, g.dl, 2 * g.nt, frontCap);
+        }
+    }
     if (cdmGetenv("CDM_BUCKET_STATS")) fprintf(stderr, "aggregate: %llu group tuples, %u segments, %llu entries (room for %llu), %u segments through the tuple sorters%s\n", nGroup, nSeg, used, capEnt, fl[1],
                                             fl[0] ? "; entry buffer overflow" : "");
     if (fl[0]) { agEnt.free(); return CDM_ERR_UNSUPPORTED; }
diff --git a/carpedeam_amd/csrc/runsort.h b/carpedeam_amd/csrc/runsort.h
--- a/carpedeam_amd/csrc/runsort.h
+++ b/carpedeam_amd/csrc/runsort.h
@@ -262,11 +262,13 @@
 }
 
 constexpr int U_T = 1024;
+static_assert(U_T == 1 << 10, "SegListArgs::uShift");
 constexpr int SEG_CLASSES = 4;
 struct SegListArgs {
     const uint32_t *recRep; const unsigned long long *dst; uint64_t nRec;
     uint32_t maxWave;
     const unsigned long long *uEnd; uint64_t units;
+    int uShift = 10;
     uint32_t cap[SEG_CLASSES - 1];
     unsigned long long *list[SEG_CLASSES]; unsigned int *cnt;
     const unsigned long long *segFirstRec = nullptr; uint64_t nSeg = 0;
@@ -283,7 +285,7 @@
             while (hi - lo > 1) { const uint64_t mid = lo + ((hi - lo) >> 1); if (a.recRep[mid] == rep) lo = mid; else hi = mid; }
             s = a.dst[j]; e = a.dst[hi];
             const unsigned long long n = e - s;
-            const bool inUnit = a.uEnd && s / U_T < a.units && e <= a.uEnd[s / U_T];
+            const bool inUnit = a.uEnd && (s >> a.uShift) < a.units && e <= a.uEnd[s >> a.uShift];
             if (n > a.maxWave && !inUnit) cls = n <= a.cap[0] ? 0 : n <= a.cap[1] ? 1 : n <= a.cap[2] ? 2 : 3;
         }
     }
@@ -301,7 +303,7 @@
     if (g < a.nSeg) {
         s = a.dst[a.segFirstRec[g]]; e = a.dst[a.segFirstRec[g + 1]];
         const unsigned long long n = e - s;
-        const bool inUnit = a.uEnd && s / U_T < a.units && e <= a.uEnd[s / U_T];
+        const bool inUnit = a.uEnd && (s >> a.uShift) < a.units && e <= a.uEnd[s >> a.uShift];
         if (n > a.maxWave && !inUnit) cls = n <= a.cap[0] ? 0 : n <= a.cap[1] ? 1 : n <= a.cap[2] ? 2 : 3;
     }
     if (!__syncthreads_or(cls >= 0)) return;
@@ -331,11 +333,12 @@
     unsigned long long *uStart, *uEnd, *uRec;
     const uint32_t *segOfRec = nullptr; const unsigned long long *segFirstRec = nullptr;
 };
+template <int UT>
 __global__ __launch_bounds__(1024) void k_unit_bounds(UnitBoundArgs a) {
     const uint64_t r = (uint64_t) blockIdx.x * blockDim.x + threadIdx.x;
     if (r >= a.nRec) return;
     const unsigned long long d0 = a.dst[r], d1 = a.dst[r + 1];
-    const uint64_t uLo = d0 / U_T + 1, uHi = (r == a.nRec - 1) ? a.units : d1 / U_T;
+    const uint64_t uLo = d0 / UT + 1, uHi = (r == a.nRec - 1) ? a.units : d1 / UT;
     if (r == 0) { a.uStart[0] = 0; a.uRec[0] = 0; }
     if (uLo > uHi) return;
     uint64_t hi, first;
@@ -354,14 +357,15 @@
     const unsigned long long sSeg = a.dst[first];
     for (uint64_t u = uLo; u <= uHi; u++) {
         if (u <= a.units) { a.uStart[u] = e; a.uRec[u] = hi; }
-        const bool mine = sSeg >= (u - 1) * (unsigned long long) U_T;
+        const bool mine = sSeg >= (u - 1) * (unsigned long long) UT;
         if (u >= 1 && u - 1 < a.units) a.uEnd[u - 1] = (mine && e - sSeg > a.maxSeg) ? sSeg : e;
     }
 }
 struct UnitClassArgs {
     const unsigned long long *uStart, *uEnd, *uRec; uint64_t units, n;
-    uint32_t cap[U_CLASSES];
-    unsigned long long *list[U_CLASSES]; unsigned int *cnt;
+    uint32_t cap[U_CLASSES + 1];
+    unsigned long long *list[U_CLASSES + 1]; unsigned int *cnt;
+    int nCls = U_CLASSES;
 };
 __global__ __launch_bounds__(1024) void k_unit_classes(UnitClassArgs a) {
     const uint64_t u = (uint64_t) blockIdx.x * blockDim.x + threadIdx.x;
@@ -369,10 +373,11 @@
     if (u < a.units) {
         s = a.uStart[u]; e = a.uEnd[u]; r0 = a.uRec[u];
         const unsigned long long m = e > s ? e - s : 0;
-        if (m) cls = m <= a.cap[0] ? 0 : m <= a.cap[1] ? 1 : 2;
-    }
-#pragma unroll
-    for (int c = 0; c < U_CLASSES; c++) {
+        if (m) { cls = 0; while (cls < a.nCls - 1 && m > a.cap[cls]) cls++; }
+    }
+#pragma unroll
+    for (int c = 0; c < U_CLASSES + 1; c++) {
+        if (c >= a.nCls) break;
         const uint32_t q = cdm_block_append(a.cnt + c, cls == c);
         if (cls == c) { a.list[c][3 * (size_t) q] = s; a.list[c][3 * (size_t) q + 1] = e; a.list[c][3 * (size_t) q + 2] = r0; }
     }
@@ -543,12 +548,15 @@
         }
     }
 }
-typedef void (*UnitHook)(hipStream_t s, unsigned int grid, const unsigned long long *list, const unsigned int *count, bucket::BigList hard, void *user);
+struct UnitClassLists { unsigned long long *list[U_CLASSES]; unsigned int *cnt; uint32_t cap[U_CLASSES]; unsigned int *handed; };
+typedef void (*UnitHook)(hipStream_t s, unsigned int grid, int cls, const unsigned long long *list, const unsigned int *count, const UnitClassLists &next, bucket::BigList hard, void *user);
 inline int segmentedSortKeys(hipStream_t s, int cuCount, uint64_t *in, uint64_t *out, uint64_t n, int shiftHi, int hiShift, int top,
                              const uint32_t *recRep, const unsigned long long *dst, uint64_t nRec, const uint64_t *srcKeys, const uint64_t *recVal,
                              UnitHook unitHook = nullptr, void *hookUser = nullptr, bool wide = false, const uint32_t *segOfRec = nullptr, int segBits = 0,
-                             const unsigned long long *segFirstRec = nullptr, uint64_t nSeg = 0) {
+                             const unsigned long long *segFirstRec = nullptr, uint64_t nSeg = 0, int unitRange = U_T, uint32_t frontCap = 0) {
     using namespace bucket;
+    if ((unitRange != 256 && unitRange != 512 && unitRange != U_T) || ((unitRange != U_T || frontCap) && !unitHook)) { cdm_set_error("segmented sort: a unit range of its own needs the aggregating unit kernel"); return CDM_ERR_UNSUPPORTED; }
+    const int nFront = frontCap ? 1 : 0;
     if (n == 0) return CDM_OK;
     if (wide && (!unitHook || !segOfRec)) { cdm_set_error("segmented sort: keys without the representative need the aggregating unit kernel and its segment table"); return CDM_ERR_UNSUPPORTED; }
     uint32_t maxSeg = U_MAXSEG, blockCap = wide ? 0 : 4096;
@@ -558,35 +566,46 @@
     if (const char *e = cdmGetenv("CDM_UNIT_SUB")) { const long m = atol(e); if (m >= 1 && m <= BK_MAXB) maxSub = (uint32_t) m; }
     if (shiftHi - 1 + BLK_IDX > 64) blockCap = 0;
     if (!unitHook && U_ORDB + shiftHi - 1 + U_IDXB > 64) maxSeg = 0;
-    const uint64_t units = (n + U_T - 1) / U_T;
+    const uint64_t units = (n + unitRange - 1) / unitRange;
     const size_t listCap = (size_t) (n / ((uint64_t) maxSeg + 1) + 2);
-    DevBuf<unsigned long long> lists[SEG_CLASSES], hardList, uStart, uEnd, uRec, uList[U_CLASSES]; DevBuf<unsigned int> cnt;
-    constexpr int NCNT = SEG_CLASSES + 1 + U_CLASSES;
+    DevBuf<unsigned long long> lists[SEG_CLASSES], hardList, uStart, uEnd, uRec, uList[U_CLASSES + 1]; DevBuf<unsigned int> cnt;
+    constexpr int NCNT = SEG_CLASSES + 1 + U_CLASSES + 2 + U_CLASSES + 1;
     if (!cnt.alloc(NCNT) || !hardList.alloc(2 * (size_t) (units + 1)) || !uStart.alloc(units + 2) || !uEnd.alloc(units + 1) || !uRec.alloc(units + 2)) return CDM_ERR_HIP;
-    for (int c = 0; c < U_CLASSES; c++) if (!uList[c].alloc(3 * (size_t) (units + 1))) return CDM_ERR_HIP;
+    for (int c = 0; c < U_CLASSES + nFront; c++) if (!uList[c].alloc(3 * (size_t) (units + 1))) return CDM_ERR_HIP;
     for (int c = 2; c < SEG_CLASSES; c++) if (!lists[c].alloc(2 * (listCap + (c == 3 ? (size_t) units + 1 : 0)))) return CDM_ERR_HIP;
     hipMemsetAsync(cnt.p, 0, NCNT * 4, s);
     if (maxSeg) {
         hipMemsetAsync(uStart.p, 0, (units + 2) * 8, s); hipMemsetAsync(uEnd.p, 0, (units + 1) * 8, s); hipMemsetAsync(uRec.p, 0, (units + 2) * 8, s);
         UnitBoundArgs ub; ub.recRep = recRep; ub.dst = dst; ub.nRec = nRec; ub.maxSeg = maxSeg; ub.units = units; ub.uStart = uStart.p; ub.uEnd = uEnd.p; ub.uRec = uRec.p;
         if (segOfRec && segFirstRec) { ub.segOfRec = segOfRec; ub.segFirstRec = segFirstRec; }
-        hipLaunchKernelGGL(k_unit_bounds, CDM_GRID((nRec + 1023) / 1024, 1024), dim3(1024), 0, s, ub);
+        if (unitRange == 256) hipLaunchKernelGGL(k_unit_bounds<256>, CDM_GRID((nRec + 1023) / 1024, 1024), dim3(1024), 0, s, ub);
+        else if (unitRange == 512) hipLaunchKernelGGL(k_unit_bounds<512>, CDM_GRID((nRec + 1023) / 1024, 1024), dim3(1024), 0, s, ub);
+        else hipLaunchKernelGGL(k_unit_bounds<U_T>, CDM_GRID((nRec + 1023) / 1024, 1024), dim3(1024), 0, s, ub);
         UnitClassArgs uc; uc.uStart = uStart.p; uc.uEnd = uEnd.p; uc.uRec = uRec.p; uc.units = units; uc.n = n;
-        for (int c = 0; c < U_CLASSES; c++) { uc.cap[c] = (uint32_t) U_CLASS_CAP[c]; uc.list[c] = uList[c].p; }
-        uc.cnt = cnt.p + SEG_CLASSES + 1;
+        unsigned int *const uCnt = cnt.p + SEG_CLASSES + 1;
+        unsigned int *const clsCnt = uCnt + U_CLASSES + 2;
+        uc.nCls = U_CLASSES + nFront;
+        if (nFront) { uc.cap[0] = frontCap; uc.list[0] = uList[U_CLASSES].p; }
+        for (int c = 0; c < U_CLASSES; c++) { uc.cap[c + nFront] = (uint32_t) U_CLASS_CAP[c]; uc.list[c + nFront] = uList[c].p; }
+        uc.cnt = clsCnt;
         hipLaunchKernelGGL(k_unit_classes, dim3((unsigned) ((units + 1023) / 1024)), dim3(1024), 0, s, uc);
+        hipMemcpyAsync(uCnt, clsCnt + nFront, U_CLASSES * 4, hipMemcpyDeviceToDevice, s);
+        if (nFront) hipMemcpyAsync(uCnt + U_CLASSES, clsCnt, 4, hipMemcpyDeviceToDevice, s);
         UnitArgs ua; ua.keys = srcKeys; ua.recVal = recVal; ua.dst = dst; ua.nRec = nRec; ua.out = out; ua.n = n; ua.repShift = shiftHi; ua.hiShift = hiShift; ua.maxSub = maxSub; ua.hard.list = hardList.p; ua.hard.cnt = cnt.p + SEG_CLASSES;
         const unsigned int pad = cdm_lds_pad("CDM_LDS_PAD_UNIT");
         const unsigned int grid = (unsigned int) std::min<uint64_t>(units, (uint64_t) cuCount * 64);
         if (unitHook) {
-            for (int c = 0; c < U_CLASSES; c++) unitHook(s, grid, uList[c].p, cnt.p + SEG_CLASSES + 1 + c, ua.hard, hookUser);
+            UnitClassLists next; next.cnt = uCnt; next.handed = uCnt + U_CLASSES + 1;
+            for (int c = 0; c < U_CLASSES; c++) { next.list[c] = uList[c].p; next.cap[c] = (uint32_t) U_CLASS_CAP[c]; }
+            if (nFront) unitHook(s, grid, -1, uList[U_CLASSES].p, uCnt + U_CLASSES, next, ua.hard, hookUser);
+            for (int c = 0; c < U_CLASSES; c++) unitHook(s, grid, c, uList[c].p, uCnt + c, next, ua.hard, hookUser);
         } else {
         ua.list = uList[0].p; ua.count = cnt.p + SEG_CLASSES + 1; hipLaunchKernelGGL((k_unit_sort<U_CLASS_CAP[0], U_CLASS_NT[0]>), dim3(grid), dim3(U_CLASS_NT[0]), pad, s, ua);
         ua.list = uList[1].p; ua.count = cnt.p + SEG_CLASSES + 2; hipLaunchKernelGGL((k_unit_sort<U_CLASS_CAP[1], U_CLASS_NT[1]>), dim3(grid), dim3(U_CLASS_NT[1]), pad, s, ua);
         ua.list = uList[2].p; ua.count = cnt.p + SEG_CLASSES + 3; hipLaunchKernelGGL((k_unit_sort<U_CLASS_CAP[2], U_CLASS_NT[2]>), dim3(grid), dim3(U_CLASS_NT[2]), pad, s, ua);
         }
     }
-    SegListArgs la; la.recRep = recRep; la.dst = dst; la.nRec = nRec; la.maxWave = maxSeg; la.uEnd = maxSeg ? uEnd.p : nullptr; la.units = units;
+    SegListArgs la; la.recRep = recRep; la.dst = dst; la.nRec = nRec; la.maxWave = maxSeg; la.uEnd = maxSeg ? uEnd.p : nullptr; la.units = units; la.uShift = unitRange == 256 ? 8 : unitRange == 512 ? 9 : 10;
     la.cap[0] = 0; la.cap[1] = 0; la.cap[2] = blockCap;
     for (int c = 0; c < SEG_CLASSES; c++) la.list[c] = lists[c].p;
     la.cnt = cnt.p;
@@ -601,6 +620,8 @@
     if (hipMemcpyAsync(hc, cnt.p, NCNT * 4, hipMemcpyDeviceToHost, s) != hipSuccess || hipStreamSynchronize(s) != hipSuccess) return CDM_ERR_HIP;
     if (cdmGetenv("CDM_BUCKET_STATS")) fprintf(stderr, "segmentedSortKeys%s: n %llu, %llu records, %llu units (%u / %u / %u by size class): segments > %u: %u (<= %u, block sort), %u longer (global radix sort); %u hard units (global radix sort)\n",
                                             unitHook ? " (units aggregated)" : "", (unsigned long long) n, (unsigned long long) nRec, (unsigned long long) units, hc[SEG_CLASSES + 1], hc[SEG_CLASSES + 2], hc[SEG_CLASSES + 3], maxSeg, hc[2], blockCap, hc[3], hc[SEG_CLASSES]);
+    if (nFront && cdmGetenv("CDM_BUCKET_STATS")) fprintf(stderr, "segmentedSortKeys: unit range %d: %u units of at most %u tuples in the wave class, %u of them handed on to the size classes (counted there as well)\n",
+                                                          unitRange, hc[SEG_CLASSES + 1 + U_CLASSES], frontCap, hc[SEG_CLASSES + 2 + U_CLASSES]);
     const unsigned int nBig = hc[3] + hc[SEG_CLASSES];
     if (nBig == 0) return CDM_OK;
     if (hc[SEG_CLASSES]) hipMemcpyAsync(lists[3].p + 2 * (size_t) hc[3], hardList.p, 2 * (size_t) hc[SEG_CLASSES] * 8, hipMemcpyDeviceToDevice, s);
```
